# jammm/first_raytracer

Hardware: AMD Instinct MI355X
Metric: Mrays/sec + RMSE vs CPU ref, CornellBox 1080p 512spp, 1/2/4/8 MI355X (higher is better)
Workload: dtype f32

## Files before the change

### first_raytracer_amd/__init__.py

```python
import ctypes
import os

import numpy as np

HERE = os.path.dirname(os.path.abspath(__file__))
LIB_PATH = os.environ.get("FRT_LIB_PATH") or os.path.join(HERE, "libfrt.so")

FRT_WORLD_BVH, FRT_WORLD_LIST = 0, 1
FRT_MAT_LAMBERTIAN, FRT_MAT_DIFFUSE_LIGHT = 0, 1
FRT_PRIM_SPHERE = 1 << 30
ABI_VERSION = 9
FRT_MAT_LAMBERTIAN, FRT_MAT_DIFFUSE_LIGHT, FRT_MAT_MODIFIED_PHONG, FRT_MAT_METAL, FRT_MAT_DIELECTRIC = 0, 1, 2, 3, 4
FRT_MAT_ROUGH_CONDUCTOR = 5
FRT_DIST_GGX, FRT_DIST_BECKMANN = 0, 1
FRT_TEX_CONSTANT, FRT_TEX_CHECKER, FRT_TEX_IMAGE = 0, 1, 2
FRT_IMAGE_SRGB8, FRT_IMAGE_F32 = 0, 1
FRT_FLAG_NO_LDS_SCENE = 1
FRT_FLAG_WAVES5 = 2
FRT_FLAG_WAVES6 = 4
FRT_FLAG_WAVES4 = 8
FRT_FLAG_BVH2 = 16
FRT_FLAG_NO_OCT = 256
FRT_FLAG_FP64 = 512
FRT_FLAG_FP32 = 1024
FRT_FLAG_ENV_SAMPLING = 2048
FRT_FLAG_ROULETTE = 4096
FRT_FLAG_SOBOL = 8192
FRT_PRECISION_AUTO, FRT_PRECISION_FP32, FRT_PRECISION_FP64 = 0, 1, 2
FRT_GPU_BVH_PLOC = 0
FRT_GPU_BVH_LBVH = 1
FRT_GPU_BVH_SAH = 2
FRT_INTEGRATOR_PATH, FRT_INTEGRATOR_PSSMLT, FRT_INTEGRATOR_AO, FRT_INTEGRATOR_NORMALS = 0, 1, 2, 3
FRT_INTEGRATOR_ALBEDO, FRT_INTEGRATOR_DEPTH, FRT_INTEGRATOR_DENOISE = 4, 5, 6
FRT_INTEGRATOR_ERROR = 8

ERRORS = {0: "ok", -1: "invalid", -2: "hip", -3: "no scene", -4: "unsupported", -5: "io", -6: "no gfx950 device"}


class FrtError(RuntimeError):
    pass


class Material(ctypes.Structure):
    _fields_ = [("type", ctypes.c_int32), ("distribution", ctypes.c_int32),
                ("albedo", ctypes.c_double * 3), ("emit", ctypes.c_double * 3),
                ("specular", ctypes.c_double * 3), ("exponent", ctypes.c_double), ("ior", ctypes.c_double),
                ("alpha", ctypes.c_double), ("eta", ctypes.c_double * 3), ("k", ctypes.c_double * 3),
                ("texture", ctypes.c_int32), ("image", ctypes.c_int32), ("tex_odd", ctypes.c_double * 3),
                ("tex_scale", ctypes.c_double * 2)]

    @classmethod
    def from_spec(cls, m):
        r = cls()
        r.type = MAT_TYPES[m["type"]]
        r.distribution = DISTRIBUTIONS[m.get("distribution", "ggx").lower()]
        for k in ("albedo", "emit", "specular", "eta", "k"):
            getattr(r, k)[:] = [float(x) for x in m.get(k, (0.0, 0.0, 0.0))]
        r.exponent = float(m.get("exponent", 0.0))
        r.ior = float(m.get("ior", 0.0))
        r.alpha = float(m.get("alpha", 0.0))
        tex = m.get("checker")
        if tex is not None:
            r.texture = FRT_TEX_CHECKER
            r.tex_odd[:] = [float(x) for x in tex["odd"]]
            r.tex_scale[:] = [float(x) for x in tex["scale"]]
        if m.get("image") is not None:
            r.texture = FRT_TEX_IMAGE
            r.image = int(m["image"])
        return r


class Image(ctypes.Structure):
    _fields_ = [("nx", ctypes.c_int32), ("ny", ctypes.c_int32), ("format", ctypes.c_int32),
                ("reserved", ctypes.c_int32), ("data", ctypes.c_void_p)]


def image_array(img):
    a = np.asarray(img["data"])
    if a.ndim != 3 or a.shape[2] != 3:
        raise ValueError("image data must be (ny, nx, 3)")
    if a.dtype == np.uint8:
        return np.ascontiguousarray(a), FRT_IMAGE_SRGB8
    return np.ascontiguousarray(a, np.float32), FRT_IMAGE_F32


CORNELL_CAMERA = {"lookfrom": (0.0, 1.0, float(np.float32(3.9))), "lookat": (0.0, 1.0, 0.0), "vup": (0.0, 1.0, 0.0),
                  "vfov": 40.0, "aperture": 0.0, "focus": 10.0}
MAT_TYPES = {"lambertian": 0, "diffuse_light": 1, "modified_phong": 2, "metal": 3, "dielectric": 4,
             "rough_conductor": 5}
DISTRIBUTIONS = {"ggx": 0, "beckmann": 1}
SPHERE_WHERE = {"world": 1, "lights": 2, "both": 3}


class SceneView(ctypes.Structure):
    _fields_ = [
        ("world_kind", ctypes.c_int32),
        ("n_tris", ctypes.c_int32),
        ("tri_v", ctypes.c_void_p), ("tri_n", ctypes.c_void_p), ("tri_material", ctypes.c_void_p),
        ("tri_geometry_normal", ctypes.c_void_p), ("tri_inv_area", ctypes.c_void_p),
        ("n_spheres", ctypes.c_int32), ("sphere", ctypes.c_void_p), ("sphere_material", ctypes.c_void_p),
        ("n_materials", ctypes.c_int32), ("materials", ctypes.c_void_p),
        ("n_nodes", ctypes.c_int32), ("root", ctypes.c_int32),
        ("node_box", ctypes.c_void_p), ("node_child", ctypes.c_void_p),
        ("n_list", ctypes.c_int32), ("list", ctypes.c_void_p),
        ("n_lights", ctypes.c_int32), ("lights", ctypes.c_void_p),
        ("cam_origin", ctypes.c_double * 3), ("cam_lower_left", ctypes.c_double * 3),
        ("cam_horizontal", ctypes.c_double * 3), ("cam_vertical", ctypes.c_double * 3),
        ("cam_u", ctypes.c_double * 3), ("cam_v", ctypes.c_double * 3),
        ("cam_lens_radius", ctypes.c_double),
        ("env_color", ctypes.c_double * 3),
        ("cam_w", ctypes.c_double * 3),
        ("cam_half_height", ctypes.c_double),
        ("tri_uv", ctypes.c_void_p),
        ("n_images", ctypes.c_int32), ("images", ctypes.c_void_p),
    ]


class RenderParams(ctypes.Structure):
    _fields_ = [(n, ctypes.c_int32) for n in ("nx", "ny", "spp")] + [("seed", ctypes.c_uint32)] + [
        (n, ctypes.c_int32) for n in ("max_depth", "integrator", "tile_size", "shard_index", "shard_count",
                                      "samples_per_item", "flags", "mlt_chains", "mlt_bootstrap", "sample_offset")]

    @classmethod
    def make(cls, nx, ny, spp, seed=0, max_depth=33, tile_size=32, shard_index=0, shard_count=1,
             samples_per_item=0, flags=0, integrator=0, sample_offset=0):
        return cls(nx=nx, ny=ny, spp=spp, seed=seed, max_depth=max_depth, integrator=integrator, tile_size=tile_size,
                   shard_index=shard_index, shard_count=shard_count, samples_per_item=samples_per_item, flags=flags,
                   mlt_chains=0, mlt_bootstrap=0, sample_offset=sample_offset)

    @classmethod
    def pssmlt(cls, nx, ny, mutations_per_pixel, chains, seed=0, bootstrap=10000, shard_index=0, shard_count=1,
               flags=0):
        return cls(nx=nx, ny=ny, spp=mutations_per_pixel, seed=seed, max_depth=10, integrator=FRT_INTEGRATOR_PSSMLT,
                   tile_size=32, shard_index=shard_index, shard_count=shard_count, samples_per_item=0, flags=flags,
                   mlt_chains=chains, mlt_bootstrap=bootstrap)


class Stats(ctypes.Structure):
    _fields_ = [(n, ctypes.c_uint64) for n in ("camera_rays", "extension_rays", "shadow_rays", "samples",
                                               "pixels", "work_items")] + [
        ("kernel_ms", ctypes.c_double), ("total_ms", ctypes.c_double)] + [
        (n, ctypes.c_uint32) for n in ("scene_in_lds", "waves_cap", "stack_entries", "bvh_depth")] + [
        ("scene_bytes", ctypes.c_uint64), ("fp64", ctypes.c_uint32), ("reserved", ctypes.c_uint32)]

    @property
    def rays(self):
        return self.camera_rays + self.extension_rays + self.shadow_rays

    def as_dict(self):
        d = {n: getattr(self, n) for n, _ in self._fields_}
        d["rays"] = self.rays
        return d


class TreeCost(ctypes.Structure):
    _fields_ = [("v", ctypes.c_double), ("t", ctypes.c_double), ("j", ctypes.c_double), ("w", ctypes.c_double),
                ("depth", ctypes.c_int32), ("n_nodes", ctypes.c_int32), ("n_rays", ctypes.c_int32),
                ("applies", ctypes.c_int32)]

    def as_dict(self):
        return {k: getattr(self, k) for k, _ in self._fields_}


class ShadowTreeInfo(ctypes.Structure):
    _fields_ = [(n, ctypes.c_int32) for n in ("why", "kept_prims", "dropped_prims", "rule_a", "rule_b", "nodes_main",
                                              "nodes_added", "nodes_shared", "root", "empty", "n_rays",
                                              "root_stops_main", "root_stops_shadow", "n_nodes")] + [
        (n, ctypes.c_double) for n in ("v_main", "t_main", "v_shadow", "t_shadow")] + [
        ("segments", ctypes.c_int64), ("segment_hits", ctypes.c_int64)]

    def as_dict(self):
        return {k: getattr(self, k) for k, _ in self._fields_}


class ExitTreeInfo(ctypes.Structure):
    _fields_ = [(n, ctypes.c_int32) for n in ("why", "classes", "taken", "budget_refused", "nodes_off", "n_nodes",
                                              "nodes_added", "depth_off", "depth_on", "n_rays", "n_ext", "reserved")] + [
        (n, ctypes.c_int64) for n in ("lds_bytes", "lds_bytes_oct", "lds_cap", "lds_cap_oct")] + [
        (n, ctypes.c_double * 2) for n in ("v_all", "t_all", "j_all", "v_ext", "t_ext")]

    def as_dict(self):
        return {k: (list(getattr(self, k)) if t is ctypes.c_double * 2 else getattr(self, k)) for k, t in self._fields_}


class PlanQuery(ctypes.Structure):
    _fields_ = [(n, ctypes.c_int32) for n in ("kind", "integrator", "flags", "world_kind", "stack_needed", "has_bvh4",
                                              "depth4", "mats", "has_spec_mats", "env_image", "env_sampling",
                                              "has_f64", "precision")] + [
        ("scene_lds_bytes", ctypes.c_int64), ("scene_lds_bytes_oct", ctypes.c_int64)]


class PlanAnswer(ctypes.Structure):
    _fields_ = [(n, ctypes.c_int32) for n in ("rc", "stack", "waves", "lds_scene", "wide", "f64")] + [
        (n, ctypes.c_int64) for n in ("lds", "scene_lds", "lds_boot")] + [
        ("kernel", ctypes.c_uint64), ("kernel_boot", ctypes.c_uint64)]


class HostSceneInfo(ctypes.Structure):
    _fields_ = [(n, ctypes.c_int32) for n in ("n_tris", "n_spheres", "n_materials", "n_lights", "n_nodes",
                                              "world_kind", "n_list", "bvh_depth")] + [
        ("load_ms", ctypes.c_double), ("build_ms", ctypes.c_double)]


_lib = None

EXPORTS = ("frt_get_abi_version", "frt_create", "frt_destroy", "frt_last_error", "frt_set_precision", "frt_upload_scene",
           "frt_shard_slot_count", "frt_shard_slots", "frt_render", "frt_render_multi", "frt_render_device", "frt_trace_device",
           "frt_mlt_chain_state",
           "frt_scene_create", "frt_scene_new", "frt_scene_add_obj", "frt_scene_add_sphere", "frt_scene_set_camera",
           "frt_scene_set_env", "frt_scene_add_image", "frt_scene_finish", "frt_scene_build_bvh_gpu",
           "frt_scene_build_bvh_sah", "frt_scene_build_bvh_gpu_algo",
           "frt_scene_view_get", "frt_scene_info", "frt_scene_destroy", "frt_write_tessellated_obj",
           "frt_write_pfm", "frt_film_accumulate", "frt_tonemap_u8", "frt_write_image", "frt_selftest_path_host",
           "frt_selftest_mlt_paths_host",
           "frt_set_env_image", "frt_scene_set_env_image", "frt_scene_env_image", "frt_read_hdr",
           "frt_selftest_path_host_env")
EXPORTS_X = ("frtx_selftest_tree_refine", "frtx_selftest_trace_host", "frtx_selftest_chunk_variance",
             "frtx_selftest_plan", "frtx_selftest_shadow_tree", "frtx_render_pixels", "frtx_render_pixels_device",
             "frtx_selftest_exit_tree", "frtx_radiance_rays", "frtx_radiance_rays_device", "frtx_camera_rays_device",
             "frtx_selftest_radiance_host", "frtx_selftest_camera_rays_host")


def lib():
    global _lib
    if _lib is not None:
        return _lib
    if not os.path.exists(LIB_PATH):
        raise FrtError(f"{LIB_PATH} is missing: build it with `python -c 'import __graft_entry__ as g; g.build()'`")
    try:
        import torch
    except ImportError:
        pass
    L = ctypes.CDLL(LIB_PATH)
    vp = ctypes.c_void_p
    L.frt_get_abi_version.restype = ctypes.c_int
    if L.frt_get_abi_version() != ABI_VERSION:
        raise FrtError(f"{LIB_PATH}: ABI version {L.frt_get_abi_version()}, binding expects {ABI_VERSION}; rebuild")
    L.frt_create.argtypes = [ctypes.c_int, ctypes.POINTER(vp)]
    L.frt_destroy.argtypes = [vp]
    L.frt_last_error.argtypes = [vp]
    L.frt_last_error.restype = ctypes.c_char_p
    L.frt_set_precision.argtypes = [vp, ctypes.c_int]
    L.frt_upload_scene.argtypes = [vp, ctypes.POINTER(SceneView)]
    L.frt_shard_slot_count.argtypes = [ctypes.POINTER(RenderParams)]
    L.frt_shard_slot_count.restype = ctypes.c_int64
    L.frt_shard_slots.argtypes = [ctypes.POINTER(RenderParams), vp]
    L.frt_render.argtypes = [vp, ctypes.POINTER(RenderParams), vp, ctypes.POINTER(Stats)]
    L.frt_render_device.argtypes = [vp, ctypes.POINTER(RenderParams), vp, vp, ctypes.POINTER(Stats)]
    L.frt_trace_device.argtypes = [vp, vp, ctypes.c_int64, vp, ctypes.c_int, vp, ctypes.POINTER(Stats)]
    L.frt_mlt_chain_state.argtypes = [vp, ctypes.c_uint64, ctypes.c_uint64, vp, vp]
    L.frt_render_multi.argtypes = [ctypes.POINTER(vp), ctypes.c_int, ctypes.POINTER(RenderParams), vp,
                                   ctypes.POINTER(Stats)]
    L.frt_scene_create.argtypes = [ctypes.c_char_p, ctypes.c_char_p, ctypes.c_double, ctypes.POINTER(vp)]
    L.frt_scene_view_get.argtypes = [vp, ctypes.POINTER(SceneView)]
    L.frt_scene_info.argtypes = [vp, ctypes.POINTER(HostSceneInfo)]
    L.frt_scene_destroy.argtypes = [vp]
    L.frt_scene_destroy.restype = None
    dp = ctypes.POINTER(ctypes.c_double)
    L.frt_scene_new.argtypes = [ctypes.POINTER(vp)]
    L.frt_scene_add_obj.argtypes = [vp, ctypes.c_char_p, dp, ctypes.POINTER(Material), ctypes.c_int]
    L.frt_scene_add_sphere.argtypes = [vp, dp, ctypes.c_double, ctypes.POINTER(Material), ctypes.c_int]
    L.frt_scene_set_camera.argtypes = [vp, dp, dp, dp, ctypes.c_double, ctypes.c_double, ctypes.c_double,
                                       ctypes.c_double]
    L.frt_scene_set_env.argtypes = [vp, dp]
    L.frt_scene_add_image.argtypes = [vp, ctypes.POINTER(Image), ctypes.POINTER(ctypes.c_int)]
    L.frt_scene_finish.argtypes = [vp, ctypes.c_int]
    L.frt_scene_build_bvh_gpu.argtypes = [vp, vp, ctypes.POINTER(ctypes.c_double)]
    L.frt_scene_build_bvh_sah.argtypes = [vp]
    L.frt_scene_build_bvh_gpu_algo.argtypes = [vp, vp, ctypes.c_int, ctypes.POINTER(ctypes.c_double)]
    L.frt_write_tessellated_obj.argtypes = [ctypes.c_char_p, ctypes.c_int, ctypes.c_char_p]
    L.frt_write_pfm.argtypes = [ctypes.c_char_p, ctypes.c_int, ctypes.c_int, vp]
    L.frt_film_accumulate.argtypes = [vp, ctypes.c_int64, vp, ctypes.c_int64, ctypes.c_int64]
    L.frt_tonemap_u8.argtypes = [vp, ctypes.c_int, ctypes.c_int, vp]
    L.frt_write_image.argtypes = [ctypes.c_char_p, ctypes.c_int, ctypes.c_int, vp, ctypes.c_int]
    L.frt_selftest_path_host.argtypes = [ctypes.POINTER(SceneView), ctypes.POINTER(RenderParams), vp,
                                         ctypes.c_int, vp, ctypes.POINTER(Stats)]
    L.frt_selftest_mlt_paths_host.argtypes = [ctypes.POINTER(SceneView), ctypes.c_int, ctypes.c_int, ctypes.c_uint32,
                                              ctypes.c_int, vp]
    L.frt_set_env_image.argtypes = [vp, ctypes.POINTER(Image)]
    L.frt_scene_set_env_image.argtypes = [vp, ctypes.c_int]
    L.frt_scene_env_image.argtypes = [vp, ctypes.POINTER(Image)]
    L.frt_read_hdr.argtypes = [ctypes.c_char_p, ctypes.POINTER(ctypes.c_int32), ctypes.POINTER(ctypes.c_int32), vp]
    L.frt_selftest_path_host_env.argtypes = [ctypes.POINTER(SceneView), ctypes.POINTER(RenderParams), vp,
                                             ctypes.c_int, ctypes.POINTER(Image), vp, ctypes.POINTER(Stats)]
    L.frtx_selftest_tree_refine.argtypes = [ctypes.POINTER(SceneView), ctypes.POINTER(TreeCost), vp, vp, ctypes.c_int32]
    L.frtx_selftest_shadow_tree.argtypes = [ctypes.POINTER(SceneView), ctypes.POINTER(ShadowTreeInfo), vp, vp,
                                            ctypes.c_int32, ctypes.c_int64, ctypes.c_uint32]
    if hasattr(L, "frtx_selftest_exit_tree"):
        L.frtx_selftest_exit_tree.argtypes = [ctypes.POINTER(SceneView), ctypes.c_int32, ctypes.POINTER(ExitTreeInfo), vp,
                                              vp, vp, ctypes.c_int32, vp, vp, ctypes.c_int32]
    L.frtx_selftest_trace_host.argtypes = [ctypes.POINTER(SceneView), vp, ctypes.c_int64, vp]
    L.frtx_selftest_chunk_variance.argtypes = [vp, ctypes.c_int, ctypes.c_int64, ctypes.c_int, ctypes.c_int, vp]
    L.frtx_render_pixels.argtypes = [vp, ctypes.POINTER(RenderParams), vp, ctypes.c_int64, vp, vp, ctypes.POINTER(Stats)]
    L.frtx_render_pixels_device.argtypes = [vp, ctypes.POINTER(RenderParams), vp, ctypes.c_int64, vp, vp, vp,
                                            ctypes.POINTER(Stats)]
    if hasattr(L, "frtx_radiance_rays"):
        L.frtx_radiance_rays.argtypes = [vp, ctypes.POINTER(RenderParams), vp, ctypes.c_int64, vp, vp, ctypes.POINTER(Stats)]
        L.frtx_radiance_rays_device.argtypes = [vp, ctypes.POINTER(RenderParams), vp, ctypes.c_int64, vp, vp, vp,
                                                ctypes.POINTER(Stats)]
        L.frtx_camera_rays_device.argtypes = [vp, ctypes.POINTER(RenderParams), vp, ctypes.c_int64, vp, vp]
        L.frtx_selftest_radiance_host.argtypes = [ctypes.POINTER(SceneView), ctypes.POINTER(RenderParams), vp, ctypes.c_int64,
                                                  ctypes.POINTER(Image), vp, ctypes.POINTER(Stats)]
        L.frtx_selftest_camera_rays_host.argtypes = [ctypes.POINTER(SceneView), ctypes.POINTER(RenderParams), vp,
                                                     ctypes.c_int64, vp]
    _lib = L
    return L


def _check(rc, what, ctx=None):
    if rc != 0:
        msg = ""
        if ctx is not None:
            msg = lib().frt_last_error(ctx).decode(errors="replace")
        elif "_rays" in what or "radiance" in what:
            msg = lib().frt_last_error(None).decode(errors="replace")
        raise FrtError(f"{what} failed: {ERRORS.get(rc, rc)} {msg}")


class HostScene:

    def __init__(self, kind, obj_path, aspect):
        self.ptr = ctypes.c_void_p()
        _check(lib().frt_scene_create(kind.encode(), obj_path.encode(), float(aspect), ctypes.byref(self.ptr)),
               f"frt_scene_create({kind})")
        self.info = HostSceneInfo()
        lib().frt_scene_info(self.ptr, ctypes.byref(self.info))
        self.env = None

    def set_env(self, rgb):
        self.env = tuple(float(x) for x in rgb)

    def set_env_image(self, index):
        _check(lib().frt_scene_set_env_image(self.ptr, -1 if index is None else int(index)), "frt_scene_set_env_image")

    def env_image(self):
        img = Image()
        rc = lib().frt_scene_env_image(self.ptr, ctypes.byref(img))
        if rc < 0:
            _check(rc, "frt_scene_env_image")
        return img if rc == 1 else None

    @classmethod
    def from_spec(cls, spec, aspect):
        self = cls.__new__(cls)
        self.ptr = ctypes.c_void_p()
        self.env = None
        L = lib()
        _check(L.frt_scene_new(ctypes.byref(self.ptr)), "frt_scene_new")

        def dptr(x):
            a = np.ascontiguousarray(np.asarray(x, np.float64))
            return a, a.ctypes.data_as(ctypes.POINTER(ctypes.c_double))
        for img in spec.get("images", ()):
            a, fmt = image_array(img)
            desc = Image(a.shape[1], a.shape[0], fmt, 0, a.ctypes.data)
            idx = ctypes.c_int(-1)
            _check(L.frt_scene_add_image(self.ptr, ctypes.byref(desc), ctypes.byref(idx)), "frt_scene_add_image")
        for o in spec["objects"]:
            if "obj" in o:
                tw = dptr(o["to_world"]) if o.get("to_world") is not None else (None, None)
                bs = ctypes.byref(Material.from_spec(o["bsdf"])) if o.get("bsdf") is not None else None
                _check(L.frt_scene_add_obj(self.ptr, o["obj"].encode(), tw[1], bs, int(bool(o.get("geo", False)))),
                       f"frt_scene_add_obj({o['obj']})")
            else:
                c = dptr(o["sphere"])
                _check(L.frt_scene_add_sphere(self.ptr, c[1], float(o["radius"]),
                                              ctypes.byref(Material.from_spec(o["material"])),
                                              SPHERE_WHERE[o.get("where", "world")]), "frt_scene_add_sphere")
        cam = spec["camera"]
        f, a, u = dptr(cam["lookfrom"]), dptr(cam["lookat"]), dptr(cam.get("vup", (0, 1, 0)))
        _check(L.frt_scene_set_camera(self.ptr, f[1], a[1], u[1], float(cam["vfov"]), float(aspect),
                                      float(cam.get("aperture", 0.0)), float(cam.get("focus", 10.0))),
               "frt_scene_set_camera")
        if spec.get("env") is not None:
            e = dptr(spec["env"])
            _check(L.frt_scene_set_env(self.ptr, e[1]), "frt_scene_set_env")
        if spec.get("env_image") is not None:
            _check(L.frt_scene_set_env_image(self.ptr, int(spec["env_image"])), "frt_scene_set_env_image")
        _check(L.frt_scene_finish(self.ptr, {"bvh": 0, "list": 1}[spec.get("world", "bvh")]), "frt_scene_finish")
        self.info = HostSceneInfo()
        L.frt_scene_info(self.ptr, ctypes.byref(self.info))
        return self

    def view(self):
        v = SceneView()
        _check(lib().frt_scene_view_get(self.ptr, ctypes.byref(v)), "frt_scene_view_get")
        if self.env is not None:
            v.env_color[:] = self.env
        return v

    def arrays(self):
        v = self.view()

        def arr(ptr, n, dt, w=1):
            if n == 0 or not ptr:
                return np.zeros((0, w) if w > 1 else 0, dt)
            a = np.ctypeslib.as_array(ctypes.cast(ptr, ctypes.POINTER(np.ctypeslib.as_ctypes_type(dt))),
                                      shape=(n * w,)).copy()
            return a.reshape(n, w) if w > 1 else a
        return {
            "tri_v": arr(v.tri_v, v.n_tris, np.float64, 9),
            "tri_material": arr(v.tri_material, v.n_tris, np.int32),
            "sphere": arr(v.sphere, v.n_spheres, np.float64, 4),
            "node_box": arr(v.node_box, v.n_nodes, np.float64, 6),
            "node_child": arr(v.node_child, v.n_nodes, np.int32, 2),
            "root": v.root,
            "lights": arr(v.lights, v.n_lights, np.int32),
            "list": arr(v.list, v.n_list, np.int32),
        }

    def build_bvh_sah(self):
        _check(lib().frt_scene_build_bvh_sah(self.ptr), "frt_scene_build_bvh_sah")
        lib().frt_scene_info(self.ptr, ctypes.byref(self.info))
        return self.info.build_ms

    def build_bvh_gpu(self, ctx, algo="gsah"):
        ms = ctypes.c_double()
        a = {"ploc": FRT_GPU_BVH_PLOC, "lbvh": FRT_GPU_BVH_LBVH, "gsah": FRT_GPU_BVH_SAH}[algo]
        _check(lib().frt_scene_build_bvh_gpu_algo(self.ptr, ctx.ptr, a, ctypes.byref(ms)),
               "frt_scene_build_bvh_gpu_algo", ctx.ptr)
        lib().frt_scene_info(self.ptr, ctypes.byref(self.info))
        return ms.value

    def __del__(self):
        if getattr(self, "ptr", None):
            try:
                lib().frt_scene_destroy(self.ptr)
            except Exception:
                pass
            self.ptr = None


class Context:

    def __init__(self, device=0, precision=None):
        self.ptr = ctypes.c_void_p()
        self.device = int(device)
        _check(lib().frt_create(int(device), ctypes.byref(self.ptr)), f"frt_create(device={device})")
        if precision is not None:
            self.set_precision(precision)

    def set_precision(self, precision):
        if isinstance(precision, str):
            precision = {"auto": FRT_PRECISION_AUTO, "fp32": FRT_PRECISION_FP32, "fp64": FRT_PRECISION_FP64}[precision]
        _check(lib().frt_set_precision(self.ptr, int(precision)), "frt_set_precision", self.ptr)

    def upload(self, scene):
        view = scene.view() if isinstance(scene, HostScene) else scene
        _check(lib().frt_upload_scene(self.ptr, ctypes.byref(view)), "frt_upload_scene", self.ptr)
        img = scene.env_image() if isinstance(scene, HostScene) else None
        if img is not None:
            _check(lib().frt_set_env_image(self.ptr, ctypes.byref(img)), "frt_set_env_image", self.ptr)
            self._env_from_scene = True
        elif isinstance(scene, HostScene) and getattr(self, "_env_from_scene", False):
            _check(lib().frt_set_env_image(self.ptr, None), "frt_set_env_image", self.ptr)
            self._env_from_scene = False

    def set_env_image(self, image):
        self._env_from_scene = False
        if image is None:
            _check(lib().frt_set_env_image(self.ptr, None), "frt_set_env_image", self.ptr)
            return
        a, fmt = image_array({"data": image})
        desc = Image(a.shape[1], a.shape[0], fmt, 0, a.ctypes.data)
        _check(lib().frt_set_env_image(self.ptr, ctypes.byref(desc)), "frt_set_env_image", self.ptr)

    def render(self, params, film=None):
        if film is None:
            film = np.zeros((params.ny, params.nx, 3), np.float32)
        assert film.dtype == np.float32 and film.flags.c_contiguous and film.size == params.nx * params.ny * 3
        st = Stats()
        _check(lib().frt_render(self.ptr, ctypes.byref(params), film.ctypes.data, ctypes.byref(st)),
               "frt_render", self.ptr)
        return film, st

    def denoise(self, film, nx, ny, spp=16, seed=0, tile_size=32, flags=0):
        p = RenderParams.make(nx, ny, spp, seed=seed, tile_size=tile_size, flags=flags,
                              integrator=FRT_INTEGRATOR_DENOISE)
        return self.render(p, film=film)

    def render_error(self, params):
        p = RenderParams.from_buffer_copy(params)
        p.integrator = FRT_INTEGRATOR_ERROR
        return self.render(p)

    def render_pixels(self, params, pixels, variance=True):
        pixels = np.ascontiguousarray(pixels, dtype=np.int32).reshape(-1)
        rgb = np.zeros((len(pixels), 3), np.float32)
        V = np.zeros((len(pixels), 3), np.float32) if variance else None
        st = Stats()
        _check(lib().frtx_render_pixels(self.ptr, ctypes.byref(params), pixels.ctypes.data, len(pixels), rgb.ctypes.data,
                                        V.ctypes.data if variance else None, ctypes.byref(st)),
               "frtx_render_pixels", self.ptr)
        return rgb, V, st

    def radiance_rays(self, params, rays, variance=True):
        rays = np.ascontiguousarray(rays, dtype=np.float32).reshape(-1, 8)
        rgb = np.zeros((len(rays), 3), np.float32)
        V = np.zeros((len(rays), 3), np.float32) if variance else None
        st = Stats()
        _check(lib().frtx_radiance_rays(self.ptr, ctypes.byref(params), rays.ctypes.data, len(rays), rgb.ctypes.data,
                                        V.ctypes.data if variance else None, ctypes.byref(st)),
               "frtx_radiance_rays", self.ptr)
        return rgb, V, st

    def camera_rays(self, params, pixels):
        import torch
        pixels = np.ascontiguousarray(pixels, dtype=np.int32).reshape(-1)
        dev = torch.device("cuda", self.device)
        px = torch.from_numpy(pixels).to(dev)
        out = torch.zeros((len(pixels), 8), dtype=torch.float32, device=dev)
        _check(lib().frtx_camera_rays_device(self.ptr, ctypes.byref(params), px.data_ptr(), len(pixels), out.data_ptr(), None),
               "frtx_camera_rays_device", self.ptr)
        return out.cpu().numpy()

    def render_camera(self, params, make_rays, passes=1):
        acc, st = None, None
        for k in range(int(passes)):
            p = RenderParams.from_buffer_copy(params)
            p.sample_offset = params.sample_offset + k * params.spp
            jitter = None if passes == 1 else np.random.default_rng([int(params.seed), k]).random(2)
            rgb, _, st = self.radiance_rays(p, make_rays(jitter), variance=False)
            acc = rgb if acc is None else film_accumulate(acc, k * params.spp, rgb, params.spp)
        return acc, st

    def render_until(self, params, target, max_spp, first_spp=None, adaptive=False, switch=None):
        if adaptive:
            film, V, counts, e, ok, _ = render_until(lambda p: self.render(p), lambda p: self.render_error(p)[0],
                                                     params, target, max_spp, first_spp, adaptive=True,
                                                     render_pixels=lambda p, px: self.render_pixels(p, px), switch=switch)
            return film, V, counts, e, ok
        film, V, spp, e, ok, _ = render_until(lambda p: self.render(p), lambda p: self.render_error(p)[0],
                                              params, target, max_spp, first_spp)
        return film, V, spp, e, ok

    def render_device(self, params, dev_ptr, stream_ptr=None):
        st = Stats()
        _check(lib().frt_render_device(self.ptr, ctypes.byref(params), ctypes.c_void_p(dev_ptr),
                                       ctypes.c_void_p(stream_ptr) if stream_ptr else None, ctypes.byref(st)),
               "frt_render_device", self.ptr)
        return st

    def mlt_chain_state(self, first, n):
        u = np.zeros((max(n, 1), 92), np.float32)
        fp = np.zeros((max(n, 1), 2), np.uint32)
        _check(lib().frt_mlt_chain_state(self.ptr, int(first), int(n), u.ctypes.data, fp.ctypes.data),
               "frt_mlt_chain_state", self.ptr)
        return u[:n], fp[:n]

    def trace_device(self, rays_ptr, n, hits_ptr, flags=0, stream_ptr=None):
        st = Stats()
        _check(lib().frt_trace_device(self.ptr, ctypes.c_void_p(rays_ptr), int(n), ctypes.c_void_p(hits_ptr), int(flags),
                                      ctypes.c_void_p(stream_ptr) if stream_ptr else None, ctypes.byref(st)),
               "frt_trace_device", self.ptr)
        return st

    def close(self):
        if getattr(self, "ptr", None):
            lib().frt_destroy(self.ptr)
            self.ptr = None

    def __del__(self):
        try:
            self.close()
        except Exception:
            pass


def render_multi(contexts, params, film=None):
    if film is None:
        film = np.zeros((params.ny, params.nx, 3), np.float32)
    assert film.dtype == np.float32 and film.flags.c_contiguous and film.size == params.nx * params.ny * 3
    arr = (ctypes.c_void_p * len(contexts))(*[c.ptr for c in contexts])
    st = Stats()
    _check(lib().frt_render_multi(arr, len(contexts), ctypes.byref(params), film.ctypes.data, ctypes.byref(st)),
           "frt_render_multi", contexts[0].ptr)
    return film, st


def frame_error(film, V):
    f = np.asarray(film, np.float64)
    v = np.asarray(V, np.float64)
    return float(np.sqrt(v.sum() / v.size) / (f.sum() / f.size))


def combine_variance(a, Va, b, Vb):
    a, b = float(a), float(b)
    va, vb = np.asarray(Va, np.float64), np.asarray(Vb, np.float64)
    return (((a * a) * va + (b * b) * vb) / ((a + b) * (a + b))).astype(np.float32)


def replicate_variance(films):
    assert len(films) == 4
    r = [np.asarray(f, np.float64) for f in films]
    m = (((r[0] + r[1]) + r[2]) + r[3]) * 0.25
    v = ((((r[0] - m) ** 2 + (r[1] - m) ** 2) + (r[2] - m) ** 2) + (r[3] - m) ** 2) / 12.0
    mean = np.array(films[0], np.float32, copy=True)
    for k in range(1, 4):
        mean = film_accumulate(mean, k, films[k], 1)
    return mean, v.astype(np.float32)


ADAPTIVE_SWITCH = 0.5
ADAPTIVE_FIRST_SPP = 128


def frame_mean(film):
    f = np.asarray(film, np.float64).reshape(-1)
    return float(np.cumsum(f)[-1] / f.size)


def render_until(render, render_error, params, target, max_spp, first_spp=None, adaptive=False, render_pixels=None,
                 switch=None):
    if first_spp is None:
        first_spp = ADAPTIVE_FIRST_SPP if adaptive else 16
    first_spp, max_spp = int(first_spp), int(max_spp)
    if first_spp < 2 or first_spp & (first_spp - 1):
        raise FrtError("render_until: first_spp must be a power of two >= 2")
    if params.integrator not in (FRT_INTEGRATOR_PATH, FRT_INTEGRATOR_AO):
        raise FrtError("render_until: path and ao renders only (pssmlt has no error estimate, denoise is a filter)")
    if not target > 0:
        raise FrtError("render_until: target must be > 0")
    sobol = bool(params.flags & FRT_FLAG_SOBOL) and params.integrator == FRT_INTEGRATOR_PATH
    reps = 4 if sobol else 1
    if max_spp < reps * first_spp:
        raise FrtError("render_until: max_spp is below the first pass")
    slots = lib().frt_shard_slot_count(ctypes.byref(params))
    if slots < 0:
        raise FrtError("bad render params")
    if adaptive:
        if sobol:
            raise FrtError("render_until: adaptive with FRT_FLAG_SOBOL is refused -- V is an upper estimate under "
                           "Sobol' points and the replicates give no per-pixel error; render without the flag")
        if render_pixels is None:
            raise FrtError("render_until: adaptive needs a render_pixels callable")
        return _render_until_adaptive(render, render_error, render_pixels, params, float(target), max_spp, first_spp,
                                      slots, ADAPTIVE_SWITCH if switch is None else float(switch))
    films, V, total, passes = [None] * reps, None, 0, []
    halve = False
    while True:
        n = first_spp if total == 0 else total
        ms = 0.0
        for k in range(reps):
            p = RenderParams.from_buffer_copy(params)
            p.spp, p.sample_offset, p.seed = n, total, (params.seed + k) & 0xffffffff
            if halve:
                p.samples_per_item = n // 2
            film, st = render(p)
            if not sobol and st.work_items == slots:
                halve = True
                p.samples_per_item = n // 2
                film, st = render(p)
            ms += st.kernel_ms
            if not sobol:
                Vp = render_error(p)
                V = Vp if total == 0 else combine_variance(total, V, n, Vp)
            films[k] = film if total == 0 else film_accumulate(films[k], total, film, n)
        total += n
        if sobol:
            film, V = replicate_variance(films)
        else:
            film = films[0]
        e = frame_error(film, V)
        passes.append((reps * total, e, ms))
        if e <= target:
            return film, V, reps * total, e, True, passes
        if reps * 2 * total > max_spp:
            return film, V, reps * total, e, False, passes


def _render_until_adaptive(render, render_error, render_pixels, params, target, max_spp, first_spp, slots, switch):
    nx, ny = params.nx, params.ny
    npx = nx * ny
    halve = False

    def full_pass(n, offset):
        nonlocal halve
        p = RenderParams.from_buffer_copy(params)
        p.spp, p.sample_offset = n, offset
        if halve:
            p.samples_per_item = n // 2
        film, st = render(p)
        if st.work_items == slots:
            halve = True
            p.samples_per_item = n // 2
            film, st = render(p)
        return film, np.asarray(render_error(p), np.float32), st.kernel_ms

    def merge(film_px, V_px, cnt_px, rgb, Vp, n):
        for c in np.unique(cnt_px):
            g = cnt_px == c
            film_px[g] = film_accumulate(film_px[g], int(c), rgb[g], n)
            V_px[g] = combine_variance(int(c), V_px[g], n, Vp[g])

    film, V, ms = full_pass(first_spp, 0)
    film = np.array(film, np.float32).reshape(npx, 3)
    V = np.array(V, np.float32).reshape(npx, 3)
    counts = np.full(npx, first_spp, np.int64)
    offset = first_spp
    passes, sampled, sparse = [], npx, False
    while True:
        tau = target * frame_mean(film)
        v64 = V.astype(np.float64)
        active = np.flatnonzero(((v64[:, 0] + v64[:, 1]) + v64[:, 2]) / 3.0 > tau * tau)
        e = frame_error(film, V)
        passes.append((int(counts.sum()), e, ms, sampled, sparse))
        done = len(active) == 0
        n = 0 if done else int(counts[active].max())
        if done or 2 * n > max_spp:
            return (film.reshape(ny, nx, 3), V.reshape(ny, nx, 3), counts.astype(np.int32).reshape(ny, nx), e, done,
                    passes)
        sparse = len(active) < switch * npx
        if sparse:
            ms, before = 0.0, counts[active]
            for c in np.unique(before):
                idx = active[before == c]
                p = RenderParams.from_buffer_copy(params)
                p.spp, p.sample_offset, p.samples_per_item = int(c), offset, 0
                rgb, Vp, st = render_pixels(p, idx.astype(np.int32))
                ms += st.kernel_ms
                film[idx] = film_accumulate(film[idx], int(c), np.asarray(rgb, np.float32), int(c))
                V[idx] = combine_variance(int(c), V[idx], int(c), np.asarray(Vp, np.float32))
                counts[idx] += c
            sampled = len(active)
        else:
            rgb, Vp, ms = full_pass(n, offset)
            merge(film, V, counts, np.asarray(rgb, np.float32).reshape(npx, 3), Vp.reshape(npx, 3), n)
            counts += n
            sampled = npx
        offset += n


def selftest_chunk_variance(partial, spp, spi):
    partial = np.ascontiguousarray(partial, dtype=np.float32)
    k, n, three = partial.shape
    assert three == 3
    out = np.zeros((n, 3), np.float32)
    _check(lib().frtx_selftest_chunk_variance(partial.ctypes.data, k, n, int(spp), int(spi), out.ctypes.data),
           "frtx_selftest_chunk_variance")
    return out


def shard_slots(params):
    n = lib().frt_shard_slot_count(ctypes.byref(params))
    if n < 0:
        raise FrtError("bad render params")
    out = np.zeros(n, np.int32)
    _check(lib().frt_shard_slots(ctypes.byref(params), out.ctypes.data), "frt_shard_slots")
    return out


def selftest_path_host(scene, params, pixels, env_image=None):
    pixels = np.ascontiguousarray(pixels, dtype=np.int32)
    out = np.zeros((len(pixels), 3), np.float32)
    st = Stats()
    view = scene.view()
    if env_image is None:
        _check(lib().frt_selftest_path_host(ctypes.byref(view), ctypes.byref(params), pixels.ctypes.data, len(pixels),
                                            out.ctypes.data, ctypes.byref(st)), "frt_selftest_path_host")
        return out, st
    a, fmt = image_array({"data": env_image})
    desc = Image(a.shape[1], a.shape[0], fmt, 0, a.ctypes.data)
    _check(lib().frt_selftest_path_host_env(ctypes.byref(view), ctypes.byref(params), pixels.ctypes.data, len(pixels),
                                            ctypes.byref(desc), out.ctypes.data, ctypes.byref(st)),
           "frt_selftest_path_host_env")
    return out, st


def ray_records(origins, directions, t_max=None, streams=None):
    o, d = np.broadcast_arrays(np.asarray(origins, np.float32).reshape(-1, 3), np.asarray(directions, np.float32).reshape(-1, 3))
    rec = np.zeros((len(d), 8), np.float32)
    rec[:, 0:3] = o
    rec[:, 3] = np.finfo(np.float32).max if t_max is None else t_max
    rec[:, 4:7] = d
    ids = np.arange(len(d), dtype=np.uint32) if streams is None else np.asarray(streams, np.uint32).reshape(-1)
    rec.view(np.uint32)[:, 7] = ids
    return rec


def selftest_radiance_host(scene, params, rays, env_image=None):
    rays = np.ascontiguousarray(rays, dtype=np.float32).reshape(-1, 8)
    out = np.zeros((len(rays), 3), np.float32)
    st = Stats()
    view = scene.view()
    desc = None
    if env_image is not None:
        a, fmt = image_array({"data": env_image})
        desc = ctypes.byref(Image(a.shape[1], a.shape[0], fmt, 0, a.ctypes.data))
    _check(lib().frtx_selftest_radiance_host(ctypes.byref(view), ctypes.byref(params), rays.ctypes.data, len(rays), desc,
                                             out.ctypes.data, ctypes.byref(st)), "frtx_selftest_radiance_host")
    return out, st


def selftest_camera_rays_host(scene, params, pixels):
    pixels = np.ascontiguousarray(pixels, dtype=np.int32).reshape(-1)
    out = np.zeros((len(pixels), 8), np.float32)
    view = scene.view()
    _check(lib().frtx_selftest_camera_rays_host(ctypes.byref(view), ctypes.byref(params), pixels.ctypes.data, len(pixels),
                                                out.ctypes.data), "frtx_selftest_camera_rays_host")
    return out


def selftest_tree_refine(scene):
    view = scene.view()
    cap = max(1, view.n_tris + view.n_spheres)
    nodes = [np.zeros((cap, 16), np.float32) for _ in range(2)]
    out = (TreeCost * 2)()
    _check(lib().frtx_selftest_tree_refine(ctypes.byref(view), out, nodes[0].ctypes.data, nodes[1].ctypes.data, cap),
           "frtx_selftest_tree_refine")
    return tuple((out[k].as_dict(), nodes[k][:out[k].n_nodes].copy()) for k in range(2))


def selftest_shadow_tree(scene, segments=0, seed=1):
    view = scene.view()
    cap = max(2 * int(view.n_nodes), 1) + 4
    nodes = np.zeros((cap, 16), np.float32)
    dropped = np.zeros(max(int(view.n_tris), 1), np.uint8)
    out = ShadowTreeInfo()
    _check(lib().frtx_selftest_shadow_tree(ctypes.byref(view), ctypes.byref(out), dropped.ctypes.data, nodes.ctypes.data,
                                           cap, int(segments), int(seed)), "frtx_selftest_shadow_tree")
    return out.as_dict(), dropped[:int(view.n_tris)].copy(), nodes[:out.n_nodes].copy()


EXIT_WHY = ("ran", "off", "material", "not_resident", "too_large", "nothing", "budget")


def selftest_exit_tree(scene, mode=1):
    view = scene.view()
    cap = max(4 * int(view.n_nodes), 1) + 16
    nodes = np.zeros((2, cap, 16), np.float32)
    roots = np.zeros(max(int(view.n_tris), 1), np.int32)
    taken = np.zeros((64, 6), np.int32)
    view_of = np.zeros(max(int(view.n_tris), 1), np.int32)
    out = ExitTreeInfo()
    _check(lib().frtx_selftest_exit_tree(ctypes.byref(view), int(mode), ctypes.byref(out), roots.ctypes.data,
                                         view_of.ctypes.data, taken.ctypes.data, len(taken), nodes[0].ctypes.data, nodes[1].ctypes.data, cap),
           "frtx_selftest_exit_tree")
    info = out.as_dict()
    info["why_name"] = EXIT_WHY[out.why]
    info["view_of"] = view_of[:int(view.n_tris)].copy()
    return (info, roots[:int(view.n_tris)].copy(), taken[:min(out.taken, len(taken))].copy(),
            nodes[0, :out.nodes_off].copy(), nodes[1, :out.n_nodes].copy())


def selftest_trace_host(scene, rays):
    rays = np.ascontiguousarray(rays, dtype=np.float32).reshape(-1, 8)
    hits = np.zeros((len(rays), 4), np.float32)
    view = scene.view()
    _check(lib().frtx_selftest_trace_host(ctypes.byref(view), rays.ctypes.data, len(rays), hits.ctypes.data),
           "frtx_selftest_trace_host")
    return hits


_handles = None


def kernel_handles():
    global _handles
    if _handles is None:
        import re
        import subprocess
        out = subprocess.run(["nm", "--defined-only", LIB_PATH], capture_output=True, text=True, check=True).stdout
        syms = [l.split() for l in out.splitlines()]
        stub = re.compile(r"(\d+)__device_stub__")
        kernels = {stub.sub(lambda m: str(int(m.group(1)) - 15), f[2]) for f in syms if len(f) == 3 and stub.search(f[2])}
        _handles = {int(f[0], 16): f[2] for f in syms if len(f) == 3 and f[2] in kernels}
    return _handles


def selftest_plan(**query):
    f = lib().frtx_selftest_plan
    f.argtypes = [ctypes.POINTER(PlanQuery), ctypes.POINTER(PlanAnswer)]
    a = PlanAnswer()
    _check(f(ctypes.byref(PlanQuery(**query)), ctypes.byref(a)), "frtx_selftest_plan")
    d = {n: getattr(a, n) for n, _ in a._fields_}
    for k in ("kernel", "kernel_boot"):
        d[k] = kernel_handles().get(d[k]) if d[k] else None
    return d


def selftest_mlt_paths_host(scene, nx, ny, seed, n):
    out = np.zeros((n, 6), np.float32)
    view = scene.view()
    _check(lib().frt_selftest_mlt_paths_host(ctypes.byref(view), nx, ny, seed, n, out.ctypes.data),
           "frt_selftest_mlt_paths_host")
    return out


def read_hdr(path):
    nx, ny = ctypes.c_int32(0), ctypes.c_int32(0)
    _check(lib().frt_read_hdr(os.fsencode(path), ctypes.byref(nx), ctypes.byref(ny), None), f"frt_read_hdr({path})")
    out = np.zeros((ny.value, nx.value, 3), np.float32)
    _check(lib().frt_read_hdr(os.fsencode(path), ctypes.byref(nx), ctypes.byref(ny), out.ctypes.data),
           f"frt_read_hdr({path})")
    return out


def write_pfm(path, film):
    film = np.ascontiguousarray(film, dtype=np.float32)
    ny, nx = film.shape[0], film.shape[1]
    _check(lib().frt_write_pfm(path.encode(), nx, ny, film.ctypes.data), "frt_write_pfm")


def film_accumulate(acc, acc_spp, film, spp):
    acc = np.ascontiguousarray(acc, dtype=np.float32)
    film = np.ascontiguousarray(film, dtype=np.float32)
    _check(lib().frt_film_accumulate(acc.ctypes.data, int(acc_spp), film.ctypes.data, int(spp), film.size),
           "frt_film_accumulate")
    return acc


def tonemap_u8(film):
    film = np.ascontiguousarray(film, dtype=np.float32)
    ny, nx = film.shape[0], film.shape[1]
    out = np.zeros((ny, nx, 3), np.uint8)
    _check(lib().frt_tonemap_u8(film.ctypes.data, nx, ny, out.ctypes.data), "frt_tonemap_u8")
    return out


IMAGE_FORMATS = {"png": 0, "bmp": 1, "jpg": 2}


def write_image(path, rgb_u8, fmt="png"):
    rgb_u8 = np.ascontiguousarray(rgb_u8, dtype=np.uint8)
    ny, nx = rgb_u8.shape[0], rgb_u8.shape[1]
    _check(lib().frt_write_image(path.encode(), nx, ny, rgb_u8.ctypes.data, IMAGE_FORMATS[fmt]), "frt_write_image")


def work_granule(integrator, spp, n_slots, lanes, spi_req=0):
    L = lib()
    f = L.frt_internal_work_granule
    f.argtypes = [ctypes.c_int, ctypes.c_int, ctypes.c_int64, ctypes.c_int64, ctypes.c_int,
                  ctypes.POINTER(ctypes.c_int), ctypes.POINTER(ctypes.c_int)]
    spi, k = ctypes.c_int(0), ctypes.c_int(0)
    _check(f(integrator, spp, n_slots, lanes, spi_req, ctypes.byref(spi), ctypes.byref(k)), "work_granule")
    return spi.value, k.value


def write_tessellated_obj(src_obj, k, dst_obj):
    _check(lib().frt_write_tessellated_obj(src_obj.encode(), int(k), dst_obj.encode()), "frt_write_tessellated_obj")
```

### first_raytracer_amd/csrc/frt_flatten.hip

```cpp
#include "frt_flatten.hpp"

#include <algorithm>
#include <cfloat>
#include <cmath>
#include <cstdlib>
#include <functional>

#include "frt_kernels.hpp"
#include "frt_tree_passes.hpp"

using namespace frt;

static inline float round_down(double x)
{
    float f = (float)x;
    if ((double)f > x) f = std::nextafter(f, -INFINITY);
    return f;
}
static inline float round_up(double x)
{
    float f = (float)x;
    if ((double)f < x) f = std::nextafter(f, INFINITY);
    return f;
}
// ... 183 lines not shown
        out.push_back(make_float4((float)c[0], (float)c[1], (float)c[2], 0.0f));
    }
}
int env_texels_of(const frt_image *img, std::vector<float4> &out, std::string &err)
{
    if (img->nx <= 0 || img->ny <= 0) { err = "environment image: nx and ny must be positive"; return FRT_E_INVALID; }
    if (!img->data) { err = "environment image: null data"; return FRT_E_INVALID; }
    if (img->format != FRT_IMAGE_SRGB8 && img->format != FRT_IMAGE_F32) {
        err = "environment image: format must be FRT_IMAGE_SRGB8 or FRT_IMAGE_F32";
        return FRT_E_INVALID;
    }
    if ((size_t)img->nx * img->ny > (size_t)INT32_MAX) { err = "environment image larger than 2^31 texels"; return FRT_E_UNSUPPORTED; }
    out.clear();
    out.reserve((size_t)img->nx * img->ny);
    append_texels(*img, out);
    for (size_t q = 0; q < out.size(); ++q) {
        const float v[3] = {out[q].x, out[q].y, out[q].z};
        for (int ch = 0; ch < 3; ++ch)
            if (!(v[ch] >= 0.0f && v[ch] <= FLT_MAX)) {
                err = "environment image: texel (" + std::to_string(q % img->nx) + ", " + std::to_string(q / img->nx) +
                      ") is negative or not finite";
                return FRT_E_INVALID;
            }
    }
    return FRT_OK;
}

static void fill_octants(FlatScene &F)
{
    for (int o = 0; o < 8 && !F.nodes_oct.empty(); ++o)
        for (size_t i = 0; i < F.nodes.size() / 4; ++i) {
            const float4 *n = &F.nodes[4 * i];
            const float b0[6] = {n[0].x, n[0].y, n[0].z, n[0].w, n[1].x, n[1].y};
            const float b1[6] = {n[1].z, n[1].w, n[2].x, n[2].y, n[2].z, n[2].w};
            float q[12];
            for (int a = 0; a < 3; ++a) {
                const bool neg = (o >> a) & 1;
                q[a] = neg ? b0[3 + a] : b0[a];
                q[3 + a] = neg ? b0[a] : b0[3 + a];
                q[6 + a] = neg ? b1[3 + a] : b1[a];
                q[9 + a] = neg ? b1[a] : b1[3 + a];
            }
            float4 *d = &F.nodes_oct[(size_t)o * F.nodes.size() + 4 * i];
            d[0] = make_float4(q[0], q[1], q[2], q[3]);
            d[1] = make_float4(q[4], q[5], q[6], q[7]);
            d[2] = make_float4(q[8], q[9], q[10], q[11]);
            d[3] = n[3];
        }
}

int flatten_scene(const frt_scene_view *sv, FlatScene &F, std::string &err, bool f64, int refine, int shadow, int exit)
{
    auto fail = [&](int code, const std::string &m) { err = m; return code; };
    const int nt = sv->n_tris, ns = sv->n_spheres, nm = sv->n_materials;
    if (nt < 0 || ns < 0 || nm <= 0 || !sv->materials || (nt > 0 && (!sv->tri_v || !sv->tri_material || !sv->tri_inv_area)))
        return fail(FRT_E_INVALID, "scene view: missing triangle arrays or materials");
    if (ns > 0 && (!sv->sphere || !sv->sphere_material)) return fail(FRT_E_INVALID, "scene view: missing sphere arrays");
    for (int i = 0; i < nm; ++i) {
        const int t = sv->materials[i].type;
        if (t != FRT_MAT_LAMBERTIAN && t != FRT_MAT_DIFFUSE_LIGHT && t != FRT_MAT_MODIFIED_PHONG &&
            t != FRT_MAT_METAL && t != FRT_MAT_DIELECTRIC && t != FRT_MAT_ROUGH_CONDUCTOR)
            return fail(FRT_E_UNSUPPORTED, "material type " + std::to_string(t) + " is not supported");
        const int tex = sv->materials[i].texture;
        if (tex != FRT_TEX_CONSTANT && tex != FRT_TEX_CHECKER && tex != FRT_TEX_IMAGE)
            return fail(FRT_E_INVALID, "material texture must be FRT_TEX_CONSTANT, FRT_TEX_CHECKER or FRT_TEX_IMAGE");
        if (tex != FRT_TEX_CONSTANT && (t == FRT_MAT_DIFFUSE_LIGHT || t == FRT_MAT_METAL))
            return fail(FRT_E_UNSUPPORTED, "checker / image textures apply to lambertian / modified_phong / dielectric / "
                                           "rough_conductor colours");
        if (tex == FRT_TEX_IMAGE) {
            const int k = sv->materials[i].image;
            if (k < 0 || k >= sv->n_images || !sv->images)
                return fail(FRT_E_INVALID, "material image index out of range");
            const frt_image &im = sv->images[k];
            if (im.nx <= 0 || im.ny <= 0 || !im.data || (im.format != FRT_IMAGE_SRGB8 && im.format != FRT_IMAGE_F32))
                return fail(FRT_E_INVALID, "scene view: bad image");
        }
        if (t == FRT_MAT_ROUGH_CONDUCTOR &&
            (!(sv->materials[i].alpha > 0.0) || (sv->materials[i].distribution != FRT_DIST_GGX &&
                                                  sv->materials[i].distribution != FRT_DIST_BECKMANN)))
            return fail(FRT_E_INVALID, "rough_conductor needs alpha > 0 and a GGX / Beckmann distribution");
    }
    auto valid_ref = [&](int ref) {
        if (ref < 0) return false;
        if (ref & FRT_PRIM_SPHERE) return (ref & ~FRT_PRIM_SPHERE) < ns;
        return ref < nt;
    };
    auto prim_box = [&](int ref, double *lo, double *hi) {
        if (ref & FRT_PRIM_SPHERE) {
            const double *q = &sv->sphere[4 * (ref & ~FRT_PRIM_SPHERE)];
            for (int k = 0; k < 3; ++k) { lo[k] = q[k] - q[3]; hi[k] = q[k] + q[3]; }
        } else {
            const double *v = &sv->tri_v[9 * ref];
            for (int k = 0; k < 3; ++k) {
                lo[k] = std::min(std::min(v[k], v[3 + k]), v[6 + k]);
                hi[k] = std::max(std::max(v[k], v[3 + k]), v[6 + k]);
            }
        }
    };
    std::vector<int> tri_order;
    std::vector<int> tri_dev(nt, -1);
    DevScene &S = F.meta;
    S = DevScene{};
    if (sv->world_kind == FRT_WORLD_BVH) {
        const int nn = sv->n_nodes;
        if (nn < 0 || (nn > 0 && (!sv->node_box || !sv->node_child)))
            return fail(FRT_E_INVALID, "scene view: missing BVH arrays");
        if (sv->root >= nn || (sv->root >= 0 && nn == 0)) return fail(FRT_E_INVALID, "scene view: bad root");
        double rlo[3], rhi[3];
        if (sv->root < 0) {
            if (!valid_ref(~sv->root)) return fail(FRT_E_INVALID, "scene view: bad root prim");
            prim_box(~sv->root, rlo, rhi);
        } else {
            for (int k = 0; k < 3; ++k) { rlo[k] = sv->node_box[6 * sv->root + k]; rhi[k] = sv->node_box[6 * sv->root + 3 + k]; }
        }
        double scale = 1.0;
        for (int k = 0; k < 3; ++k) scale = std::max(scale, std::max(std::fabs(rlo[k]), std::fabs(rhi[k])));
        const double pad = 4e-6 * scale;
        auto padded = [&](const double *lo, const double *hi, float *flo, float *fhi) {
            for (int k = 0; k < 3; ++k) { flo[k] = round_down(lo[k] - pad); fhi[k] = round_up(hi[k] + pad); }
        };
        padded(rlo, rhi, S.root_lo, S.root_hi);
        S.ao_tmax = (float)((rhi[1] - rlo[1]) * 0.50f);
        std::vector<int> new_id(std::max(nn, 1), -1), order;
        order.reserve(nn);
        std::vector<std::pair<int, int>> st;
        st.push_back({sv->root, 1});
        while (!st.empty()) {
            const auto [x, lvl] = st.back();
            st.pop_back();
            if (x >= 0) {
                if (x >= nn || new_id[x] >= 0) return fail(FRT_E_INVALID, "scene view: BVH is not a tree");
                new_id[x] = (int)order.size();
                order.push_back(x);
                F.depth = std::max(F.depth, lvl);
                st.push_back({sv->node_child[2 * x + 1], lvl + 1});
                st.push_back({sv->node_child[2 * x], lvl + 1});
            } else {
                const int ref = ~x;
                if (!valid_ref(ref)) return fail(FRT_E_INVALID, "scene view: bad leaf prim");
                if (!(ref & FRT_PRIM_SPHERE)) {
                    if (tri_dev[ref] >= 0) return fail(FRT_E_INVALID, "scene view: triangle in two leaves");
                    tri_dev[ref] = (int)tri_order.size();
                    tri_order.push_back(ref);
                }
            }
        }
        F.nodes.resize(4 * order.size());
        for (size_t i = 0; i < order.size(); ++i) {
            const int x = order[i];
            float cb[2][6];
            int cref[2];
            for (int side = 0; side < 2; ++side) {
                const int ch = sv->node_child[2 * x + side];
                double lo[3], hi[3];
                if (ch >= 0) {
                    for (int k = 0; k < 3; ++k) { lo[k] = sv->node_box[6 * ch + k]; hi[k] = sv->node_box[6 * ch + 3 + k]; }
                    cref[side] = new_id[ch];
                } else {
                    const int ref = ~ch;
                    prim_box(ref, lo, hi);
                    cref[side] = ~((ref & FRT_PRIM_SPHERE) ? ref : tri_dev[ref]);
                }
                padded(lo, hi, &cb[side][0], &cb[side][3]);
            }
            F.nodes[4 * i + 0] = make_float4(cb[0][0], cb[0][1], cb[0][2], cb[0][3]);
            F.nodes[4 * i + 1] = make_float4(cb[0][4], cb[0][5], cb[1][0], cb[1][1]);
            F.nodes[4 * i + 2] = make_float4(cb[1][2], cb[1][3], cb[1][4], cb[1][5]);
            F.nodes[4 * i + 3] = make_float4(i2f(cref[0]), i2f(cref[1]), 0.0f, 0.0f);
        }
        if (nt >= kLeafIndexLimit) return fail(FRT_E_INVALID, "scene view: too many triangles");
        const int forced = leaf_size_override();
        if (forced) {
            collapse_leaves(F, forced);
        } else {
            const std::vector<float4> binary = F.nodes;
            const int depth = F.depth;
            collapse_leaves(F, kLeafSmallScene);
            if (!lds_planar_fits(lds_planar_bytes(F.nodes.size() / 4, 5 * (size_t)nt + 2 * (size_t)nm)) || F.depth >= kLdsMaxDepth) {
                F.nodes = binary;
                F.depth = depth;
                collapse_leaves(F, kLeafDefault);
            }
        }
        for (int i = 0; i < nt; ++i)
            if (tri_dev[i] < 0) { tri_dev[i] = (int)tri_order.size(); tri_order.push_back(i); }
    } else if (sv->world_kind == FRT_WORLD_LIST) {
        S.ao_spheres_only = 1;
        if (sv->n_list < 0 || (sv->n_list > 0 && !sv->list)) return fail(FRT_E_INVALID, "scene view: bad list");
        for (int i = 0; i < nt; ++i) { tri_dev[i] = i; tri_order.push_back(i); }
        for (int i = 0; i < sv->n_list; ++i)
            if (!valid_ref(sv->list[i])) return fail(FRT_E_INVALID, "scene view: bad list entry");
    } else {
        return fail(FRT_E_INVALID, "scene view: unknown world kind");
    }
    auto dev_ref = [&](int ref) { return (ref & FRT_PRIM_SPHERE) ? ref : tri_dev[ref]; };
    F.tri_view = tri_order;

    bool any_smooth = false;
    for (int i = 0; i < nt; ++i)
        if (sv->tri_geometry_normal && !sv->tri_geometry_normal[i]) any_smooth = true;
    if (any_smooth && !sv->tri_n) return fail(FRT_E_INVALID, "scene view: smooth triangles without normals");
    F.tris.resize(3 * (size_t)nt);
    F.tshade.resize(2 * (size_t)nt);
    if (any_smooth) F.tnorm.resize(3 * (size_t)nt);
    if (f64) {
        F.tris64.resize(3 * (size_t)nt);
        F.tshade64.resize(nt);
        if (any_smooth) F.tnorm64.resize(3 * (size_t)nt);
    }
    for (int d = 0; d < nt; ++d) {
        const int i = tri_order[d];
        const double *v = &sv->tri_v[9 * i];
        const double e1[3] = {v[3] - v[0], v[4] - v[1], v[5] - v[2]};
        const double e2[3] = {v[6] - v[0], v[7] - v[1], v[8] - v[2]};
        double ng[3] = {e1[1] * e2[2] - e1[2] * e2[1], e1[2] * e2[0] - e1[0] * e2[2], e1[0] * e2[1] - e1[1] * e2[0]};
        const double l = std::sqrt(ng[0] * ng[0] + ng[1] * ng[1] + ng[2] * ng[2]);
        for (int k = 0; k < 3; ++k) ng[k] = ng[k] / l;
        F.tris[3 * d + 0] = make_float4((float)v[0], (float)v[1], (float)v[2], 0.0f);
        F.tris[3 * d + 1] = make_float4((float)e1[0], (float)e1[1], (float)e1[2], 0.0f);
        F.tris[3 * d + 2] = make_float4((float)e2[0], (float)e2[1], (float)e2[2], 0.0f);
        const int mat = sv->tri_material[i];
        if (mat < 0 || mat >= nm) return fail(FRT_E_INVALID, "scene view: bad triangle material");
        const int geo = sv->tri_geometry_normal ? (sv->tri_geometry_normal[i] ? 1 : 0) : 1;
        F.tshade[2 * d + 0] = make_float4((float)ng[0], (float)ng[1], (float)ng[2], (float)sv->tri_inv_area[i]);
        F.tshade[2 * d + 1] = make_float4(i2f(mat), i2f(geo), 0.0f, 0.0f);
        if (any_smooth)
            for (int k = 0; k < 3; ++k)
                F.tnorm[3 * d + k] = make_float4((float)sv->tri_n[9 * i + 3 * k], (float)sv->tri_n[9 * i + 3 * k + 1],
                                                 (float)sv->tri_n[9 * i + 3 * k + 2], 0.0f);
        if (f64) {
            F.tris64[3 * d + 0] = make_double4(v[0], v[1], v[2], 0.0);
            F.tris64[3 * d + 1] = make_double4(e1[0], e1[1], e1[2], 0.0);
            F.tris64[3 * d + 2] = make_double4(e2[0], e2[1], e2[2], 0.0);
            F.tshade64[d] = make_double4(ng[0], ng[1], ng[2], sv->tri_inv_area[i]);
            if (any_smooth)
                for (int k = 0; k < 3; ++k)
                    F.tnorm64[3 * d + k] = make_double4(sv->tri_n[9 * i + 3 * k], sv->tri_n[9 * i + 3 * k + 1],
                                                        sv->tri_n[9 * i + 3 * k + 2], 0.0);
        }
    }
    bool any_tex = false;
    for (int i = 0; i < nm; ++i) any_tex |= sv->materials[i].texture != FRT_TEX_CONSTANT;
    if (any_tex) {
        F.tuv.assign(2 * (size_t)std::max(nt, 1), make_float4(0.0f, 0.0f, 0.0f, 0.0f));
        if (sv->tri_uv)
            for (int d = 0; d < nt; ++d) {
                const double *q = &sv->tri_uv[6 * tri_order[d]];
                F.tuv[2 * d] = make_float4((float)q[0], (float)q[1], (float)q[2], (float)q[3]);
                F.tuv[2 * d + 1] = make_float4((float)q[4], (float)q[5], 0.0f, 0.0f);
            }
    }
    F.spheres.resize(ns);
    F.smat.resize(ns);
    if (f64) F.spheres64.resize(ns);
    for (int k = 0; k < ns; ++k) {
        const double *q = &sv->sphere[4 * k];
        F.spheres[k] = make_float4((float)q[0], (float)q[1], (float)q[2], (float)q[3]);
        if (f64) F.spheres64[k] = make_double4(q[0], q[1], q[2], q[3]);
        F.smat[k] = sv->sphere_material[k];
        if (F.smat[k] < 0 || F.smat[k] >= nm) return fail(FRT_E_INVALID, "scene view: bad sphere material");
    }
    std::vector<int> image_off(std::max(sv->n_images, 0), -1);
    for (int i = 0; i < nm; ++i) {
        if (sv->materials[i].texture != FRT_TEX_IMAGE) continue;
        const int k = sv->materials[i].image;
        if (image_off[k] >= 0) continue;
        const frt_image &im = sv->images[k];
        const size_t n = (size_t)im.nx * im.ny;
        if (F.texels.size() + n > (size_t)INT32_MAX) return fail(FRT_E_UNSUPPORTED, "images larger than 2^31 texels");
        image_off[k] = (int)F.texels.size();
        append_texels(im, F.texels);
    }
    F.mats.assign(kMatStride * (size_t)nm, make_float4(0.0f, 0.0f, 0.0f, 0.0f));
    for (int i = 0; i < nm; ++i) {
        const frt_material &m = sv->materials[i];
        float4 *d = &F.mats[kMatStride * i];
        auto f4 = [](const double *v, float w) { return make_float4((float)v[0], (float)v[1], (float)v[2], w); };
        d[0] = f4(m.type == FRT_MAT_ROUGH_CONDUCTOR ? m.eta : m.albedo, i2f(m.type));
        if (m.type == FRT_MAT_DIFFUSE_LIGHT) d[1] = f4(m.emit, 0.0f);
        else d[1] = f4(m.specular, (float)(m.type == FRT_MAT_MODIFIED_PHONG ? m.exponent
                                           : m.type == FRT_MAT_DIELECTRIC ? m.ior : m.alpha));
        d[2] = f4(m.k, i2f(m.distribution));
        d[3] = f4(m.tex_odd, i2f(m.texture));
        d[4] = make_float4((float)m.tex_scale[0], (float)m.tex_scale[1], 0.0f, 0.0f);
        if (m.texture == FRT_TEX_IMAGE)
            d[4] = make_float4(i2f(sv->images[m.image].nx), i2f(sv->images[m.image].ny), i2f(image_off[m.image]), 0.0f);
    }
    if (sv->n_lights < 0 || (sv->n_lights > 0 && !sv->lights)) return fail(FRT_E_INVALID, "scene view: bad lights");
    F.lights.resize(sv->n_lights);
    for (int i = 0; i < sv->n_lights; ++i) {
        if (!valid_ref(sv->lights[i])) return fail(FRT_E_INVALID, "scene view: bad light");
        F.lights[i] = dev_ref(sv->lights[i]);
    }
    F.list.resize(sv->world_kind == FRT_WORLD_LIST ? sv->n_list : 0);
    for (size_t i = 0; i < F.list.size(); ++i) F.list[i] = dev_ref(sv->list[i]);

    if (sv->world_kind == FRT_WORLD_BVH && F.depth < kLdsMaxDepth &&
        lds_octant_fits(lds_octant_bytes(F.nodes.size() / 4, lds_rest(F))))
        F.nodes_oct.resize(8 * F.nodes.size());
    S.root = (sv->world_kind == FRT_WORLD_BVH) ? ((sv->root >= 0) ? 0 : ~dev_ref(~sv->root)) : 0;
    S.sroot = S.root;
    auto derive_trees = [&]() {
        fill_octants(F);
        F.has4 = sv->world_kind == FRT_WORLD_BVH && build_bvh4(F, S.root);
        if (!F.has4) F.nodes4.clear();
        S.root4 = F.has4 ? F.root4 : S.root;
        S.n_nodes4 = (int)(F.nodes4.size() / kNode4Parts);
    };
    derive_trees();
    S.n_lights = sv->n_lights;
    S.n_list = (int)F.list.size();
    S.n_nodes = (int)(F.nodes.size() / 4);
    S.n_tris = nt;
    S.n_mats = nm;
    S.n_nodes4 = (int)(F.nodes4.size() / kNode4Parts);
    S.node_es = 4; S.node_ps = 1;
    S.node4_es = kNode4Parts; S.node4_ps = 1;
    S.tri_es = 3; S.tri_ps = 1;
    S.sh_es = 2; S.sh_ps = 1;
    S.world_kind = sv->world_kind;
    auto f3d = [](const double *x) { return mk3((float)x[0], (float)x[1], (float)x[2]); };
    S.cam_o = f3d(sv->cam_origin); S.cam_llc = f3d(sv->cam_lower_left);
    S.cam_h = f3d(sv->cam_horizontal); S.cam_v = f3d(sv->cam_vertical);
    S.cam_u = f3d(sv->cam_u); S.cam_vv = f3d(sv->cam_v);
    S.lens_r = (float)sv->cam_lens_radius;
    S.cam_w = f3d(sv->cam_w);
    S.cam_half_height = (float)sv->cam_half_height;
    S.env = f3d(sv->env_color);
    auto d3d = [](const double *x) { return d3{x[0], x[1], x[2]}; };
    S.cam64_o = d3d(sv->cam_origin); S.cam64_llc = d3d(sv->cam_lower_left);
    S.cam64_h = d3d(sv->cam_horizontal); S.cam64_v = d3d(sv->cam_vertical);
    S.cam64_u = d3d(sv->cam_u); S.cam64_vv = d3d(sv->cam_v);
    S.lens_r64 = sv->cam_lens_radius;
    bool again = refine_tree(F, refine);
    again |= shadow_tree(sv, F, shadow);
    again |= exit_tree(sv, F, exit);
    if (again) derive_trees();
    S.n_nodes = (int)(F.nodes.size() / 4);
    return FRT_OK;
}

DevScene host_scene(const FlatScene &F)
{
    DevScene S = F.meta;
    S.nodes = F.nodes.data(); S.nodes4 = F.nodes4.data(); S.nodes_oct = F.nodes_oct.data();
    S.tris = F.tris.data(); S.tshade = F.tshade.data(); S.tnorm = F.tnorm.data();
    S.tuv = F.tuv.data(); S.texels = F.texels.data();
    S.spheres = F.spheres.data(); S.sphere_mat = F.smat.data(); S.mats = F.mats.data();
    S.lights = F.lights.data(); S.list = F.list.data(); S.tri_view = F.tri_view.data();
    S.tris64 = F.tris64.data(); S.tshade64 = F.tshade64.data(); S.tnorm64 = F.tnorm64.data();
    S.spheres64 = F.spheres64.data();
    return S;
}
```

### first_raytracer_amd/csrc/frt_flatten.hpp

```cpp
#pragma once
#include <string>
#include <vector>

#include "frt.h"
#include "frt_device.hpp"
#include "frt_path.hpp"

using frt::DevScene;

#pragma GCC visibility push(hidden)
struct FlatScene {
    std::vector<float4> nodes, tris, tshade, tnorm, spheres, mats, tuv;
    std::vector<float4> texels;
    std::vector<uint4> nodes4;
    std::vector<float4> nodes_oct;
    std::vector<double4> tris64, tshade64, tnorm64, spheres64;
    bool has4 = false;
    int root4 = 0, depth4 = 0;
    std::vector<int> smat, lights, list;
    std::vector<int> tri_view;
    DevScene meta{};
    int depth = 0;
    enum { kShadowRan = 0, kShadowOff, kShadowNoLights, kShadowTooLarge, kShadowMaterial, kShadowNotResident,
           kShadowNothing, kShadowBudget };
    struct {
        int why = kShadowOff;
        std::vector<uint8_t> dropped;
        int n_dropped = 0, rule_a = 0, rule_b = 0, nodes_main = 0, added = 0, shared = 0;
        bool empty = false;
    } shadow;
    enum { kExitRan = 0, kExitOff, kExitMaterial, kExitNotResident, kExitTooLarge, kExitNothing, kExitBudget };
    struct ExitClass { int sub, root, members, dropped, added, shared; double gain; };
    struct {
        int why = kExitOff;
        int classes = 0;
        std::vector<ExitClass> taken;
        std::vector<int> root;
        int nodes_before = 0, added = 0;
        bool budget_refused = false;
    } exit;
};

int flatten_scene(const frt_scene_view *sv, FlatScene &F, std::string &err, bool f64, int refine = -1, int shadow = -1,
                  int exit = -1);
int env_texels_of(const frt_image *img, std::vector<float4> &out, std::string &err);
frt::DevScene host_scene(const FlatScene &F);
#pragma GCC visibility pop
```

### first_raytracer_amd/csrc/frt_selftest.hip

```cpp
#include <algorithm>
#include <cstring>
#include <string>
#include <vector>

#include "frt_ctx.hpp"
#include "frt_flatten.hpp"
#include "frt_rays.hpp"
#include "frt_tree_passes.hpp"
#include "host/envdist.hpp"

using namespace frt;

constexpr int kSelftestStack = 8;

template <typename R, int MATS = kMatsAll>
static void selftest_pixels(const DevScene &S, const FlatScene &F, const frt_render_params *p, const int32_t *pixels,
                            int npix, bool wide, std::vector<int> &stack, float *out_rgb, uint64_t cnt[3],
                            const float *rays = nullptr)
{
    uint32_t n_ext = 0, n_sh = 0;
    for (int i = 0; i < npix; ++i) {
        const int pix = rays ? 0 : pixels[i];
        const int px = pix % p->nx, py = pix / p->nx;
        float4 ray[2];
        if (rays) memcpy(ray, rays + 8 * (size_t)i, sizeof(ray));
        V3<R> acc = zero3<R>();
        for (int smp = 0; smp < p->spp; ++smp) {
            PathState<R> P;
            if (rays) ray_begin<MATS>(P, ray[0], ray[1], p->seed, (uint32_t)(smp + p->sample_offset));
            else path_begin<MATS>(P, S, px, py, p->nx, p->ny, p->seed, (uint32_t)pix, (uint32_t)(smp + p->sample_offset));
            ++cnt[0];
            for (;;) {
                Hit<R> h;
                const bool occl = p->integrator != FRT_INTEGRATOR_AO && light_shadow_ray(P);
                const int xroot = p->integrator == FRT_INTEGRATOR_PATH && !P.shadow ? exit_root(P) : 0;
                if (S.world_kind == FRT_WORLD_LIST) {
                    h = trace<FRT_WORLD_LIST, 1>(S, P.ro, P.rd, P.rtmax, P.shadow, stack.data());
                } else if constexpr (!kIsF64<R>) {
                    h = wide ? trace<kWorldBvh4, 1, kSelftestStack>(S, P.ro, P.rd, P.rtmax, P.shadow, stack.data())
                        : xroot ? trace_bvh_from<1>(S, xroot, P.ro, P.rd, P.rtmax, stack.data())
                             : trace<FRT_WORLD_BVH, 1>(S, P.ro, P.rd, P.rtmax, P.shadow, stack.data(), occl);
                } else {
                    h = xroot ? trace_bvh_from<1>(S, xroot, P.ro, P.rd, P.rtmax, stack.data())
                              : trace<FRT_WORLD_BVH, 1>(S, P.ro, P.rd, P.rtmax, P.shadow, stack.data(), occl);
                }
                n_ext = n_sh = 0;
                const bool done = p->integrator == FRT_INTEGRATOR_AO ? ao_shade<MATS>(P, S, h, n_sh)
                                  : p->integrator == FRT_INTEGRATOR_NORMALS ? normals_shade<MATS>(P, S, h)
                                  : p->integrator == FRT_INTEGRATOR_ALBEDO ? albedo_shade(P, S, h)
                                  : p->integrator == FRT_INTEGRATOR_DEPTH ? depth_shade(P, S, h)
                                  : path_shade<MATS, true>(P, S, h, p->max_depth, n_ext, n_sh);
                cnt[1] += n_ext; cnt[2] += n_sh;
                if (done) break;
            }
            acc = acc + P.L;
        }
        if (p->integrator == FRT_INTEGRATOR_ALBEDO || p->integrator == FRT_INTEGRATOR_DEPTH) {
            const R n = (R)p->spp;
            out_rgb[3 * i] = (float)(acc.x / n); out_rgb[3 * i + 1] = (float)(acc.y / n); out_rgb[3 * i + 2] = (float)(acc.z / n);
            if (p->integrator == FRT_INTEGRATOR_DEPTH)
                out_rgb[3 * i + 1] = depth_moment_floor(out_rgb[3 * i], out_rgb[3 * i + 1], out_rgb[3 * i + 2]);
            continue;
        }
        if (rays) {
            const R n = (R)p->spp;
            out_rgb[3 * i] = (float)(acc.x / n); out_rgb[3 * i + 1] = (float)(acc.y / n); out_rgb[3 * i + 2] = (float)(acc.z / n);
            continue;
        }
        const R k = R(1) / (R)p->spp;
        out_rgb[3 * i] = (float)(acc.x * k); out_rgb[3 * i + 1] = (float)(acc.y * k); out_rgb[3 * i + 2] = (float)(acc.z * k);
    }
}

extern "C" int frt_selftest_path_host(const frt_scene_view *sv, const frt_render_params *p, const int32_t *pixels,
                                      int npix, float *out_rgb, frt_stats *st)
{
    return frt_selftest_path_host_env(sv, p, pixels, npix, nullptr, out_rgb, st);
}
static int selftest_replay(const frt_scene_view *sv, const frt_render_params *p, const int32_t *pixels, const float *rays,
                           int npix, const frt_image *env, float *out_rgb, frt_stats *st);
extern "C" int frt_selftest_path_host_env(const frt_scene_view *sv, const frt_render_params *p, const int32_t *pixels,
                                          int npix, const frt_image *env, float *out_rgb, frt_stats *st)
{
    if (!sv || !p || !pixels || !out_rgb || npix < 0 || p->spp <= 0 || p->nx <= 0 || p->ny <= 0) return FRT_E_INVALID;
    for (int i = 0; i < npix; ++i)
        if (pixels[i] < 0 || pixels[i] >= p->nx * p->ny) return FRT_E_INVALID;
    return selftest_replay(sv, p, pixels, nullptr, npix, env, out_rgb, st);
}
static int selftest_replay(const frt_scene_view *sv, const frt_render_params *p, const int32_t *pixels, const float *rays,
                           int npix, const frt_image *env, float *out_rgb, frt_stats *st)
{
    if (p->integrator == FRT_INTEGRATOR_DENOISE) return FRT_E_INVALID;
    if (p->integrator == FRT_INTEGRATOR_ERROR) return FRT_E_INVALID;
    const bool feature = p->integrator == FRT_INTEGRATOR_ALBEDO || p->integrator == FRT_INTEGRATOR_DEPTH;
    if (feature) env = nullptr;
    const bool f64 = (p->flags & FRT_FLAG_FP64) != 0 && !feature;
    FlatScene F;
    std::string err;
    const int rc = flatten_scene(sv, F, err, f64);
    if (rc != FRT_OK) return rc;
    if (p->integrator == FRT_INTEGRATOR_AO)
        for (int i = 0; i < sv->n_materials; ++i)
            if (sv->materials[i].type == FRT_MAT_METAL) return FRT_E_UNSUPPORTED;
    DevScene S = host_scene(F);
    std::vector<float4> env_tex;
    bool env_sampling = false;
    if (env) {
        const int erc = env_texels_of(env, env_tex, err);
        if (erc != FRT_OK) return erc;
        if ((p->flags & FRT_FLAG_ENV_SAMPLING) && p->integrator != FRT_INTEGRATOR_AO &&
            p->integrator != FRT_INTEGRATOR_NORMALS) {
            std::vector<float> tab;
            env_sampling = env_tables_of(&env_tex[0].x, env->nx, env->ny, tab);
            const size_t n = env_tex.size();
            env_tex.resize(n + tab.size() / 4);
            memcpy(reinterpret_cast<float *>(env_tex.data() + n), tab.data(), tab.size() * sizeof(float));
        }
        S.env_texels = env_tex.data(); S.env_nx = env->nx; S.env_ny = env->ny;
    }
    std::vector<int> stack(std::max(F.depth + 1, kSelftestStack));
    const bool wide = !f64 && S.world_kind == FRT_WORLD_BVH && F.has4 && !(p->flags & FRT_FLAG_BVH2) &&
                      bvh4_stack_fits(F.depth4, kSelftestStack);
    uint64_t cnt[3] = {0, 0, 0};
    constexpr int kEnvAll = kMatsAll | kMatsEnv;
    constexpr int kEnvNee = kEnvAll | kMatsEnvNee;
    const bool path = p->integrator == FRT_INTEGRATOR_PATH;
    const bool roulette = (p->flags & FRT_FLAG_ROULETTE) && path, sobol = (p->flags & FRT_FLAG_SOBOL) && path;
    auto run_set = [&](auto extra) {
        constexpr int X = decltype(extra)::value;
        auto run = [&](auto mats) {
            constexpr int M = decltype(mats)::value;
            if (f64) selftest_pixels<double, M | X>(S, F, p, pixels, npix, wide, stack, out_rgb, cnt, rays);
            else selftest_pixels<float, M | X>(S, F, p, pixels, npix, wide, stack, out_rgb, cnt, rays);
        };
        if (env_sampling) run(std::integral_constant<int, kEnvNee>{});
        else if (env) run(std::integral_constant<int, kEnvAll>{});
        else run(std::integral_constant<int, kMatsAll>{});
    };
    if (sobol && roulette) run_set(std::integral_constant<int, kMatsSobol | kMatsRoulette>{});
    else if (sobol) run_set(std::integral_constant<int, kMatsSobol>{});
    else if (roulette) run_set(std::integral_constant<int, kMatsRoulette>{});
    else run_set(std::integral_constant<int, 0>{});
    if (st) {
        memset(st, 0, sizeof(*st));
        st->camera_rays = cnt[0]; st->extension_rays = cnt[1]; st->shadow_rays = cnt[2];
        st->samples = cnt[0]; st->pixels = (uint64_t)npix;
        st->stack_entries = wide ? (uint32_t)kSelftestStack : (uint32_t)stack.size();
        st->bvh_depth = (uint32_t)(wide ? F.depth4 : F.depth);
        st->fp64 = f64 ? 1u : 0u;
    }
    return FRT_OK;
}

extern "C" int frtx_selftest_radiance_host(const frt_scene_view *sv, const frt_render_params *p, const float *rays, int64_t n,
                                           const frt_image *env, float *out_rgb, frt_stats *st)
{
    auto fail = [](int code, const std::string &m) { frt::null_ctx_err() = m; return code; };
    if (!sv || !p || n < 0 || n > INT32_MAX || (n > 0 && (!rays || !out_rgb))) return fail(FRT_E_INVALID, "radiance_rays: bad arguments");
    const int k = p->integrator;
    if (k == FRT_INTEGRATOR_NORMALS || k == FRT_INTEGRATOR_ALBEDO || k == FRT_INTEGRATOR_DEPTH)
        return fail(FRT_E_UNSUPPORTED, "radiance_rays: path and ao only (normals, albedo and depth have no sparse kernel)");
    if (k != FRT_INTEGRATOR_PATH && k != FRT_INTEGRATOR_AO)
        return fail(FRT_E_INVALID, "radiance_rays: path and ao only (pssmlt is no per-pixel estimator; denoise and error are "
                                   "films of a whole frame)");
    if (p->shard_count != 1) return fail(FRT_E_INVALID, "radiance_rays: shard_count must be 1 (split the list instead)");
    if (p->spp <= 0 || p->sample_offset < 0) return fail(FRT_E_INVALID, "bad render params");
    std::string why;
    if (frt::rays_first_bad(rays, n, why) >= 0) return fail(FRT_E_INVALID, "radiance_rays: " + why);
    if (st) memset(st, 0, sizeof(*st));
    if (n == 0) return FRT_OK;
    frt_render_params q = *p;
    q.nx = q.ny = 1;
    return selftest_replay(sv, &q, nullptr, rays, (int)n, env, out_rgb, st);
}

extern "C" int frtx_selftest_camera_rays_host(const frt_scene_view *sv, const frt_render_params *p, const int32_t *pixels,
                                              int64_t npix, float *rays_out)
{
    if (!sv || !p || npix < 0 || (npix > 0 && (!pixels || !rays_out)) || p->nx <= 0 || p->ny <= 0 || p->sample_offset < 0 ||
        (int64_t)p->nx * p->ny > (int64_t)INT32_MAX)
        return FRT_E_INVALID;
    for (int64_t i = 0; i < npix; ++i)
        if (pixels[i] < 0 || pixels[i] >= p->nx * p->ny) return FRT_E_INVALID;
    FlatScene F;
    std::string err;
    const int rc = flatten_scene(sv, F, err, false);
    if (rc != FRT_OK) return rc;
    const DevScene S = host_scene(F);
    for (int64_t i = 0; i < npix; ++i) {
        const int pix = pixels[i];
        PathState<float> P;
        if (p->flags & FRT_FLAG_SOBOL)
            path_begin<kMatsSobol>(P, S, pix % p->nx, pix / p->nx, p->nx, p->ny, p->seed, (uint32_t)pix, (uint32_t)p->sample_offset);
        else
            path_begin<kMatsNone>(P, S, pix % p->nx, pix / p->nx, p->nx, p->ny, p->seed, (uint32_t)pix, (uint32_t)p->sample_offset);
        const float rec[8] = {P.ro.x, P.ro.y, P.ro.z, P.rtmax, P.rd.x, P.rd.y, P.rd.z, i2f(pix)};
        memcpy(rays_out + 8 * i, rec, sizeof(rec));
    }
    return FRT_OK;
}

extern "C" int frt_selftest_mlt_paths_host(const frt_scene_view *sv, int nx, int ny, uint32_t seed, int n,
                                           float *out6)
{
    if (!sv || !out6 || n < 0 || nx <= 0 || ny <= 0) return FRT_E_INVALID;
    FlatScene F;
    std::string err;
    const int rc = flatten_scene(sv, F, err, false);
    if (rc != FRT_OK) return rc;
    const DevScene S = host_scene(F);
    std::vector<int> stack(std::max(F.depth + 1, 1));
    for (int i = 0; i < n; ++i) {
        PrndSource src{nullptr, 0, 0, rng_key(seed ^ kMltBootSalt, (uint32_t)i, 0u), 0u, true, 0.0f, 0.0f};
        MltPath M;
        mlt_begin(M, S, src, nx, ny);
        uint32_t ne = 0, ns = 0;
        for (;;) {
            if (mlt_beyond(M)) { M.P.L = M.P.L + M.P.beta * env_of<float>(S); break; }
            const Hit<float> h = (S.world_kind == FRT_WORLD_LIST)
                              ? trace<FRT_WORLD_LIST, 1>(S, M.P.ro, M.P.rd, M.P.rtmax, M.P.shadow, stack.data())
                              : trace<FRT_WORLD_BVH, 1>(S, M.P.ro, M.P.rd, M.P.rtmax, M.P.shadow, stack.data(), M.P.shadow);
            if (mlt_shade(M, S, h, src, ne, ns)) break;
        }
        const f3 L = M.P.L;
        float *o = &out6[6 * (size_t)i];
        o[0] = M.x; o[1] = M.y; o[2] = L.x; o[3] = L.y; o[4] = L.z; o[5] = fmaxf(fmaxf(L.x, L.y), L.z);
    }
    return FRT_OK;
}

extern "C" int frtx_selftest_tree_refine(const frt_scene_view *sv, frt_tree_cost out[2], float *nodes_off,
                                        float *nodes_on, int32_t max_nodes)
{
    if (!sv || !out) return FRT_E_INVALID;
    float *dst[2] = {nodes_off, nodes_on};
    for (int on = 0; on < 2; ++on) {
        FlatScene F;
        std::string err;
        const int rc = flatten_scene(sv, F, err, false, on, 0, 0);
        if (rc != FRT_OK) return rc;
        TreeCost c;
        const bool applies = tree_cost_host(F, c);
        const int nn = (int)(F.nodes.size() / 4);
        out[on] = frt_tree_cost{c.V, c.T, c.J, c.w, c.depth, nn, c.n_rays, applies ? 1 : 0};
        if (dst[on]) {
            if (nn > max_nodes) return FRT_E_INVALID;
            memcpy(dst[on], F.nodes.data(), F.nodes.size() * sizeof(float4));
        }
    }
    return FRT_OK;
}

extern "C" int frtx_selftest_shadow_tree(const frt_scene_view *sv, frt_shadow_tree_info *out, uint8_t *dropped,
                                         float *nodes, int32_t max_nodes, int64_t segments, uint32_t seed)
{
    if (!sv || !out || segments < 0) return FRT_E_INVALID;
    FlatScene F;
    std::string err;
    const int rc = flatten_scene(sv, F, err, false, -1, 1, 0);
    if (rc != FRT_OK) return rc;
    const auto &I = F.shadow;
    memset(out, 0, sizeof(*out));
    out->why = I.why;
    out->n_nodes = (int)(F.nodes.size() / 4);
    out->nodes_main = I.nodes_main;
    out->root = F.meta.sroot;
    if (nodes) {
        if (out->n_nodes > max_nodes) return FRT_E_INVALID;
        memcpy(nodes, F.nodes.data(), F.nodes.size() * sizeof(float4));
    }
    if (dropped) memset(dropped, 0, (size_t)std::max(sv->n_tris, 0));
    if (I.why != FlatScene::kShadowRan) return FRT_OK;
    out->dropped_prims = I.n_dropped;
    out->kept_prims = sv->n_tris + sv->n_spheres - I.n_dropped;
    out->rule_a = I.rule_a; out->rule_b = I.rule_b;
    out->nodes_added = I.added; out->nodes_shared = I.shared; out->empty = I.empty ? 1 : 0;
    if (dropped)
        for (int d = 0; d < sv->n_tris; ++d) dropped[F.tri_view[d]] = I.dropped[d];
    ShadowCost c;
    shadow_cost_host(F, c);
    out->n_rays = c.n_rays;
    out->v_main = c.V[0]; out->t_main = c.T[0]; out->v_shadow = c.V[1]; out->t_shadow = c.T[1];
    out->root_stops_main = c.stops[0]; out->root_stops_shadow = c.stops[1];
    if (segments > 0) {
        std::vector<float> org;
        shadow_origins_host(F, org);
        const DevScene S = host_scene(F);
        const int64_t no = (int64_t)(org.size() / 3);
        for (int64_t i = 0; i < segments && no > 0 && S.n_lights > 0; ++i) {
            const RngKey key = rng_key(seed, (uint32_t)i, (uint32_t)(i >> 32));
            const float *q = &org[3 * (size_t)(i % no)];
            const f3 o = mk3(q[0], q[1], q[2]);
            int idx = (int)(rng_u(key, 0) * (float)S.n_lights);
            if (idx == S.n_lights) idx -= 1;
            f3 ln;
            int lmat;
            const f3 d = prim_sample(S, S.lights[idx], o, rng_u(key, 1), rng_u(key, 2), ln, lmat);
            ++out->segments;
            for (int t = 0; t < S.n_tris; ++t) {
                if (!I.dropped[t]) continue;
                float u, v;
                if (prim_t(S, t, o, d, bvh_tmin(o), 1.0f - Cst<float>::shadow_eps, u, v) > 0.0f) ++out->segment_hits;
            }
        }
    }
    return FRT_OK;
}

extern "C" int frtx_selftest_exit_tree(const frt_scene_view *sv, int32_t mode, frt_exit_tree_info *out, int32_t *roots,
                                       int32_t *view_of, int32_t *taken, int32_t max_taken, float *nodes_off,
                                       float *nodes_on, int32_t max_nodes)
{
    if (!sv || !out || mode < -1 || mode > 1 || max_taken < 0) return FRT_E_INVALID;
    memset(out, 0, sizeof(*out));
    FlatScene F0, F;
    std::string err;
    int rc = flatten_scene(sv, F0, err, false, -1, -1, 0);
    if (rc == FRT_OK) rc = flatten_scene(sv, F, err, false, -1, -1, mode);
    if (rc != FRT_OK) return rc;
    const auto &I = F.exit;
    out->why = I.why;
    out->classes = I.classes;
    out->taken = (int32_t)I.taken.size();
    out->nodes_off = (int32_t)(F0.nodes.size() / 4);
    out->n_nodes = (int32_t)(F.nodes.size() / 4);
    out->nodes_added = I.added;
    out->budget_refused = I.budget_refused ? 1 : 0;
    out->depth_off = F0.depth; out->depth_on = F.depth;
    out->lds_bytes = (int64_t)lds_planar_bytes(out->n_nodes, lds_rest(F));
    out->lds_bytes_oct = F.nodes_oct.empty() ? 0 : (int64_t)lds_octant_bytes(out->n_nodes, lds_rest(F));
    out->lds_cap = (int64_t)kLdsSceneBytes; out->lds_cap_oct = (int64_t)kLdsOctBytes;
    if (out->nodes_off > max_nodes || out->n_nodes > max_nodes) return FRT_E_INVALID;
    if (nodes_off) memcpy(nodes_off, F0.nodes.data(), F0.nodes.size() * sizeof(float4));
    if (nodes_on) memcpy(nodes_on, F.nodes.data(), F.nodes.size() * sizeof(float4));
    if (roots)
        for (int d = 0; d < sv->n_tris; ++d) {
            const int r = f2i(F.tshade[2 * (size_t)d + 1].z);
            if (r != (d < (int)I.root.size() ? I.root[d] : 0)) return FRT_E_UNSUPPORTED;
            roots[F.tri_view[d]] = r;
        }
    if (view_of)
        for (int d = 0; d < sv->n_tris; ++d) view_of[d] = F.tri_view[d];
    if (taken)
        for (int k = 0; k < out->taken && k < max_taken; ++k) {
            const auto &c = I.taken[k];
            const int32_t rec[6] = {c.sub, c.root, c.members, c.dropped, c.added, c.shared};
            memcpy(taken + 6 * k, rec, sizeof(rec));
        }
    ExitCost c;
    if (exit_cost_host(F, c)) {
        out->n_rays = c.n_rays; out->n_ext = c.n_ext;
        for (int on = 0; on < 2; ++on) {
            out->v_all[on] = c.V_all[on]; out->t_all[on] = c.T_all[on]; out->j_all[on] = c.J_all[on];
            out->v_ext[on] = c.V_ext[on]; out->t_ext[on] = c.T_ext[on];
        }
    }
    return FRT_OK;
}

extern "C" int frtx_selftest_trace_host(const frt_scene_view *sv, const float *rays, int64_t n, float *hits)
{
    if (!sv || n < 0 || (n > 0 && (!rays || !hits))) return FRT_E_INVALID;
    FlatScene F;
    std::string err;
    const int rc = flatten_scene(sv, F, err, false);
    if (rc != FRT_OK) return rc;
    const DevScene S = host_scene(F);
    std::vector<int> stack(std::max(F.depth + 1, 1));
    for (int64_t i = 0; i < n; ++i) {
        const float *q = rays + 8 * i;
        const f3 o = mk3(q[0], q[1], q[2]), d = mk3(q[4], q[5], q[6]);
        const bool anyhit = (f2i(q[7]) & 1) != 0;
        const Hit<float> h = S.world_kind == FRT_WORLD_LIST ? trace<FRT_WORLD_LIST, 1>(S, o, d, q[3], anyhit, stack.data())
                                                            : trace<FRT_WORLD_BVH, 1>(S, o, d, q[3], anyhit, stack.data());
        const int ref = (h.prim < 0 || (h.prim & FRT_PRIM_SPHERE)) ? h.prim : F.tri_view[h.prim];
        float *r = hits + 4 * i;
        r[0] = h.t; r[1] = h.u; r[2] = h.v;
        const float refbits = i2f(ref);
        memcpy(&r[3], &refbits, sizeof(float));
    }
    return FRT_OK;
}
```

### first_raytracer_amd/csrc/frt_tree_passes.hip

```cpp
#include "frt_tree_passes.hpp"

#include <algorithm>
#include <cstdlib>
#include <cstring>
#include <functional>
#include <unordered_map>

#include "frt_kernels.hpp"
#include "host/exit_tree.hpp"
#include "host/shadow_tree.hpp"
#include "host/tree_refine.hpp"

using namespace frt;

static bool knob(const char *name)
{
    const char *e = std::getenv(name);
    return !(e && std::atoi(e) == 0);
}
static bool pass_on(int mode, const char *name) { return mode < 0 ? knob(name) : mode != 0; }

static bool lambertian_only(const frt_scene_view *sv)
{
    for (int i = 0; i < sv->n_materials; ++i)
        if (sv->materials[i].type != FRT_MAT_LAMBERTIAN && sv->materials[i].type != FRT_MAT_DIFFUSE_LIGHT) return false;
    return true;
}

static bool tree_in_lds(const FlatScene &F)
{
    if (F.meta.world_kind != FRT_WORLD_BVH || F.meta.root < 0 || F.depth >= kLdsMaxDepth) return false;
    return lds_planar_fits(lds_planar_bytes(F.nodes.size() / 4, lds_rest(F))) || !F.nodes_oct.empty();
}

constexpr size_t kLdsGranule = 1280, kLdsCuBytes = 160 * 1024;
static int lds_blocks_per_cu(const FlatScene &F, size_t scene_bytes)
{
    const size_t block = lds_block_bytes(F.depth < 8 ? 8 : 16, scene_bytes);
    return (int)(kLdsCuBytes / ((block + kLdsGranule - 1) / kLdsGranule * kLdsGranule));
}
static bool keeps_plan(const FlatScene &F, int nn0, int nn1, bool same_blocks)
{
    const size_t rest = lds_rest(F);
    const size_t p0 = lds_planar_bytes(nn0, rest), p1 = lds_planar_bytes(nn1, rest);
    const size_t o0 = lds_octant_bytes(nn0, rest), o1 = lds_octant_bytes(nn1, rest);
    const bool lds0 = lds_planar_fits(p0), oct0 = !F.nodes_oct.empty();
    if (lds0 != lds_planar_fits(p1) || oct0 != lds_octant_fits(o1)) return false;
    if (!same_blocks) return true;
    if (lds0 && lds_blocks_per_cu(F, p1) != lds_blocks_per_cu(F, p0)) return false;
    return !oct0 || lds_blocks_per_cu(F, o1) == lds_blocks_per_cu(F, o0);
}

static std::vector<float> node_floats(const std::vector<float4> &nodes)
{
    std::vector<float> v(4 * nodes.size());
    memcpy(v.data(), nodes.data(), sizeof(float4) * nodes.size());
    return v;
}
static std::vector<float4> node_records(const std::vector<float> &v)
{
    std::vector<float4> nodes(v.size() / 4);
    memcpy(nodes.data(), v.data(), sizeof(float) * v.size());
    return nodes;
}
static void adopt_nodes(FlatScene &F, const std::vector<float> &v)
{
    F.nodes = node_records(v);
    if (!F.nodes_oct.empty()) F.nodes_oct.resize(8 * F.nodes.size());
}

struct RefineLeaf { float box[6]; int ref; };

struct TreeView {
    frt_refine::Topology t;
    std::vector<RefineLeaf> leaves;
    std::unordered_map<int, int> leaf_of;

    explicit TreeView(const std::vector<float4> &nodes)
    {
        const int nn = (int)(nodes.size() / 4);
        t.child.assign(2 * (size_t)nn, 0);
        for (int i = 0; i < nn; ++i) {
            const float4 *n = &nodes[4 * i];
            const float b[2][6] = {{n[0].x, n[0].y, n[0].z, n[0].w, n[1].x, n[1].y}, {n[1].z, n[1].w, n[2].x, n[2].y, n[2].z, n[2].w}};
            for (int side = 0; side < 2; ++side) {
                const int c = f2i(side ? n[3].y : n[3].x);
                if (c >= 0) { t.child[2 * i + side] = ~c; continue; }
                const auto [it, fresh] = leaf_of.emplace(c, (int)leaves.size());
                if (fresh) {
                    RefineLeaf l;
                    for (int k = 0; k < 6; ++k) l.box[k] = b[side][k];
                    l.ref = c;
                    leaves.push_back(l);
                }
                t.child[2 * i + side] = it->second;
            }
        }
        t.n_leaves = (int)leaves.size();
        t.root = t.n_leaves;
        for (int &c : t.child)
            if (c < 0) c = t.n_leaves + ~c;
    }
    int slot(int ref) const { return ref >= 0 ? t.n_leaves + ref : leaf_of.at(ref); }
    std::vector<int> leaves_under(int s) const
    {
        std::vector<int> under, st{s};
        while (!st.empty()) {
            const int x = st.back();
            st.pop_back();
            if (x < t.n_leaves) { under.push_back(x); continue; }
            st.push_back(t.child[2 * (x - t.n_leaves)]);
            st.push_back(t.child[2 * (x - t.n_leaves) + 1]);
        }
        return under;
    }
    bool same_leaves(const TreeView &o) const
    {
        return leaves.size() == o.leaves.size() &&
               std::equal(leaves.begin(), leaves.end(), o.leaves.begin(),
                          [](const RefineLeaf &a, const RefineLeaf &b) { return a.ref == b.ref; });
    }
};

constexpr double kRefineW = 1.8;
constexpr int kRefineFitFrame = 24, kRefineValFrame = 40;
constexpr uint32_t kRefineFitSeed = 0x7ee5eed1u, kRefineValSeed = 0x7ee5eed2u;
constexpr int kRefineMaxDepth = 33;
constexpr int kRefineMaxEvals = 700;

struct Replay {
    frt_refine::RaySet R;
    std::vector<uint8_t> occl;
    std::vector<int> from;
    std::vector<float> origins;
};
static Replay sample_rays(const FlatScene &F, const std::vector<RefineLeaf> &leaves, int frame, uint32_t seed)
{
    const DevScene S = host_scene(F);
    struct Ray { f3 o, d; float tmax; bool shadow, occl; int from; };
    std::vector<Ray> rays;
    std::vector<int> stack(std::max(F.depth + 1, 1));
    for (int pix = 0; pix < frame * frame; ++pix) {
        PathState<float> P;
        path_begin<kMatsAll>(P, S, pix % frame, pix / frame, frame, frame, seed, (uint32_t)pix, 0u);
        int last = -1;
        for (;;) {
            rays.push_back(Ray{P.ro, P.rd, P.rtmax, P.shadow, light_shadow_ray(P),
                               (P.shadow || last < 0 || (last & FRT_PRIM_SPHERE)) ? -1 : last});
            const Hit<float> h = trace<FRT_WORLD_BVH, 1>(S, P.ro, P.rd, P.rtmax, P.shadow, stack.data(), light_shadow_ray(P));
            if (!P.shadow) last = h.prim;
            uint32_t n_ext = 0, n_sh = 0;
            if (path_shade<kMatsAll>(P, S, h, kRefineMaxDepth, n_ext, n_sh)) break;
        }
    }
    const int n = (int)rays.size(), nl = (int)leaves.size();
    Replay out;
    frt_refine::RaySet &R = out.R;
    R.n = n;
    R.n_leaves = nl;
    R.prim_first.assign(nl + 1, 0);
    for (int l = 0; l < nl; ++l) {
        const int lref = ~leaves[l].ref;
        const bool sph = (lref & FRT_PRIM_SPHERE) != 0;
        const int first = sph ? lref : (lref & kLeafIndexMask), count = sph ? 1 : (lref >> kLeafCountShift) + 1;
        for (int k = 0; k < count; ++k) R.prim_ref.push_back(first + k);
        R.prim_first[l + 1] = (int)R.prim_ref.size();
    }
    R.n_prims = (int)R.prim_ref.size();
    R.tmin.resize(n); R.tmax.resize(n); R.anyhit.resize(n); R.live.resize(n);
    out.occl.assign(n, 0);
    out.from.assign(n, -1);
    R.slab.resize((size_t)nl * n * 6);
    R.prim_t.resize((size_t)n * R.n_prims);
    int stride = (int)(0.618 * n) | 1;
    auto gcd = [](int a, int b) { while (b) { const int c = a % b; a = b; b = c; } return a; };
    while (n > 1 && gcd(stride, n) != 1) stride += 2;
    for (int i = 0; i < n; ++i) {
        const Ray &q = rays[(int)(((int64_t)i * stride) % std::max(n, 1))];
        Trav<float> T;
        R.live[i] = trav_begin(T, S, S.root, q.o, q.d, q.tmax) ? 1 : 0;
        R.tmin[i] = T.tmin;
        R.tmax[i] = q.tmax;
        R.anyhit[i] = q.shadow ? 1 : 0;
        out.occl[i] = q.occl ? 1 : 0;
        out.from[i] = q.from;
        if (q.occl) out.origins.insert(out.origins.end(), {q.o.x, q.o.y, q.o.z});
        const float inv[3] = {T.sr.invd.x, T.sr.invd.y, T.sr.invd.z}, oi[3] = {T.sr.oinv.x, T.sr.oinv.y, T.sr.oinv.z};
        for (int l = 0; l < nl; ++l) {
            float *s = &R.slab[((size_t)i * nl + l) * 6];
            for (int a = 0; a < 3; ++a) {
                const bool neg = inv[a] < 0.0f;
                s[a] = vfma(leaves[l].box[neg ? 3 + a : a], inv[a], oi[a]);
                s[3 + a] = -vfma(leaves[l].box[neg ? a : 3 + a], inv[a], oi[a]);
            }
        }
        for (int k = 0; k < R.n_prims; ++k) {
            float u, v;
            R.prim_t[(size_t)i * R.n_prims + k] = prim_t(S, R.prim_ref[k], q.o, q.d, T.tmin, q.tmax, u, v);
        }
    }
    return out;
}


static void write_topology(FlatScene &F, const frt_refine::Topology &t, const std::vector<RefineLeaf> &leaves)
{
    const int L = t.n_leaves, nn = L - 1;
    std::vector<float> box(6 * (size_t)(L + nn));
    std::function<void(int)> bound = [&](int s) {
        float *b = &box[6 * (size_t)s];
        if (s < L) { for (int k = 0; k < 6; ++k) b[k] = leaves[s].box[k]; return; }
        const int c0 = t.child[2 * (s - L)], c1 = t.child[2 * (s - L) + 1];
        bound(c0);
        bound(c1);
        for (int k = 0; k < 3; ++k) {
            b[k] = std::min(box[6 * (size_t)c0 + k], box[6 * (size_t)c1 + k]);
            b[3 + k] = std::max(box[6 * (size_t)c0 + 3 + k], box[6 * (size_t)c1 + 3 + k]);
        }
    };
    bound(t.root);
    std::vector<float4> out(4 * (size_t)nn);
    int next = 0;
    std::function<int(int)> emit = [&](int s) {
        if (s < L) return leaves[s].ref;
        const int me = next++;
        const int c[2] = {t.child[2 * (s - L)], t.child[2 * (s - L) + 1]};
        const float *a = &box[6 * (size_t)c[0]], *b = &box[6 * (size_t)c[1]];
        out[4 * me + 0] = make_float4(a[0], a[1], a[2], a[3]);
        out[4 * me + 1] = make_float4(a[4], a[5], b[0], b[1]);
        out[4 * me + 2] = make_float4(b[2], b[3], b[4], b[5]);
        const int r0 = emit(c[0]), r1 = emit(c[1]);
        out[4 * me + 3] = make_float4(i2f(r0), i2f(r1), 0.0f, 0.0f);
        return me;
    };
    emit(t.root);
    F.nodes.swap(out);
}

bool tree_cost_host(const FlatScene &F, TreeCost &out)
{
    out = TreeCost{};
    out.w = kRefineW;
    if (!tree_in_lds(F) || F.nodes.empty()) return false;
    const TreeView v(F.nodes);
    const Replay val = sample_rays(F, v.leaves, kRefineValFrame, kRefineValSeed);
    const frt_refine::Cost c = frt_refine::tree_cost(v.t, val.R);
    out.V = c.V; out.T = c.T; out.J = frt_refine::cost_j(c, kRefineW);
    out.depth = v.t.depth();
    out.n_rays = val.R.n;
    return true;
}

bool refine_tree(FlatScene &F, int mode)
{
    const int nn = (int)(F.nodes.size() / 4);
    if (!pass_on(mode, "FRT_TREE_REFINE") || !tree_in_lds(F) || nn < 3) return false;
    const TreeView v(F.nodes);
    if (v.t.n_leaves != nn + 1) return false;
    frt_refine::Topology t = v.t;
    const Replay fit = sample_rays(F, v.leaves, kRefineFitFrame, kRefineFitSeed);
    if (frt_refine::refine(t, fit.R, kRefineW, v.t.depth(), kRefineMaxEvals) == 0) return false;
    const Replay val = sample_rays(F, v.leaves, kRefineValFrame, kRefineValSeed);
    const double j0 = frt_refine::cost_j(frt_refine::tree_cost(v.t, val.R), kRefineW);
    const double j1 = frt_refine::cost_j(frt_refine::tree_cost(t, val.R), kRefineW);
    if (!(j1 < j0)) return false;
    write_topology(F, t, v.leaves);
    return true;
}


struct ProofGeometry {
    std::vector<double> tv, tn;
    std::vector<uint8_t> smooth;
    frt_shadow::Geometry g;
};
static void proof_geometry(const frt_scene_view *sv, const FlatScene &F, ProofGeometry &pg)
{
    const int nt = sv->n_tris;
    pg.tv.resize(9 * (size_t)nt);
    pg.smooth.assign(nt, 0);
    bool any_smooth = false;
    for (int d = 0; d < nt; ++d) {
        const int i = F.tri_view[d];
        std::copy(&sv->tri_v[9 * (size_t)i], &sv->tri_v[9 * (size_t)i] + 9, &pg.tv[9 * (size_t)d]);
        pg.smooth[d] = sv->tri_geometry_normal && !sv->tri_geometry_normal[i];
        any_smooth |= pg.smooth[d] != 0;
    }
    if (any_smooth) {
        pg.tn.resize(9 * (size_t)nt);
        for (int d = 0; d < nt; ++d)
            std::copy(&sv->tri_n[9 * (size_t)F.tri_view[d]], &sv->tri_n[9 * (size_t)F.tri_view[d]] + 9, &pg.tn[9 * (size_t)d]);
    }
    frt_shadow::Geometry &g = pg.g;
    g.n_tris = nt; g.n_spheres = sv->n_spheres;
    g.tri_v = pg.tv.data(); g.tri_n = any_smooth ? pg.tn.data() : nullptr; g.tri_smooth = pg.smooth.data();
    g.sphere = sv->sphere;
    g.lights = F.lights.data(); g.n_lights = (int)F.lights.size(); g.sphere_bit = FRT_PRIM_SPHERE;
    for (int k = 0; k < 3; ++k) { g.cam_o[k] = sv->cam_origin[k]; g.cam_u[k] = sv->cam_u[k]; g.cam_v[k] = sv->cam_v[k]; }
    g.lens_r = sv->cam_lens_radius;
    g.eps = (double)Cst<float>::eps;
}

bool shadow_tree(const frt_scene_view *sv, FlatScene &F, int mode)
{
    if (!pass_on(mode, "FRT_SHADOW_TREE")) return false;
    auto &I = F.shadow;
    DevScene &S = F.meta;
    auto why = [&](int w) { I.why = w; return w == FlatScene::kShadowRan; };
    I.nodes_main = (int)(F.nodes.size() / 4);
    if (sv->n_lights <= 0) return why(FlatScene::kShadowNoLights);
    if (!lambertian_only(sv)) return why(FlatScene::kShadowMaterial);
    if (!tree_in_lds(F) || F.nodes.empty()) return why(FlatScene::kShadowNotResident);
    ProofGeometry pg;
    proof_geometry(sv, F, pg);
    frt_shadow::Classified c;
    frt_shadow::classify(pg.g, c);
    if (c.why != frt_shadow::kRan)
        return why(c.why == frt_shadow::kNoLights ? FlatScene::kShadowNoLights : FlatScene::kShadowTooLarge);
    int n_dropped = 0;
    for (int d = 0; d < sv->n_tris; ++d) n_dropped += c.dropped[d];
    if (n_dropped == 0) return why(FlatScene::kShadowNothing);
    std::vector<float> nodes = node_floats(F.nodes);
    frt_shadow::Tree t;
    frt_shadow::build(nodes, S.root, c.dropped, FRT_PRIM_SPHERE, kLeafCountShift, t);
    if (t.dropped_leaves == 0) return why(FlatScene::kShadowNothing);
    if (!keeps_plan(F, I.nodes_main, (int)(nodes.size() / 16), false)) return why(FlatScene::kShadowBudget);
    adopt_nodes(F, nodes);
    S.sroot = t.empty ? kSentinel : t.root;
    I.dropped = c.dropped;
    I.n_dropped = n_dropped; I.rule_a = c.n_rule_a; I.rule_b = c.n_rule_b;
    I.added = t.added; I.shared = t.shared; I.empty = t.empty;
    return why(FlatScene::kShadowRan);
}

bool shadow_cost_host(const FlatScene &F, ShadowCost &out)
{
    out = ShadowCost{};
    if (F.shadow.why != FlatScene::kShadowRan) return false;
    const TreeView v(F.nodes);
    Replay val = sample_rays(F, v.leaves, kRefineValFrame, kRefineValSeed);
    frt_refine::RaySet &R = val.R;
    const std::vector<uint8_t> &occl = val.occl;
    int n_occl = 0;
    for (int i = 0; i < R.n; ++i) n_occl += occl[i];
    out.n_rays = n_occl;
    if (n_occl == 0) return true;
    auto price = [&](int which) {
        const frt_refine::Cost c = frt_refine::tree_cost(v.t, R);
        out.V[which] = c.V * R.n / n_occl;
        out.T[which] = c.T * R.n / n_occl;
    };
    for (int i = 0; i < R.n; ++i) {
        R.live[i] = R.live[i] && occl[i];
        if (occl[i] && !R.live[i]) ++out.stops[0];
    }
    price(0);
    if (F.shadow.empty) {
        out.stops[1] = n_occl;
        return true;
    }
    const int sroot = v.slot(F.meta.sroot);
    const std::vector<int> under = v.leaves_under(sroot);
    auto misses_box = [&](int i) {
        float u[6];
        for (int k = 0; k < 6; ++k) u[k] = __builtin_inff();
        for (int l : under)
            for (int k = 0; k < 6; ++k) u[k] = std::min(u[k], R.slab[((size_t)i * R.n_leaves + l) * 6 + k]);
        const float tn = std::max(std::max(u[0], u[1]), std::max(u[2], Cst<float>::eps));
        const float tf = std::min(std::min(-u[3], -u[4]), std::min(-u[5], R.tmax[i]));
        return !(tn <= tf);
    };
    R.root.assign(R.n, sroot);
    for (int i = 0; i < R.n; ++i) {
        R.live[i] = occl[i];
        if (occl[i] && misses_box(i)) ++out.stops[1];
    }
    price(1);
    return true;
}

void shadow_origins_host(const FlatScene &F, std::vector<float> &origins)
{
    origins.clear();
    if (F.meta.world_kind != FRT_WORLD_BVH || F.nodes.empty()) return;
    origins = sample_rays(F, TreeView(F.nodes).leaves, kRefineValFrame, kRefineValSeed).origins;
}

constexpr int kExitMaxRoot = 1 << 10;

bool exit_tree(const frt_scene_view *sv, FlatScene &F, int mode)
{
    if (!pass_on(mode, "FRT_EXIT_TREE")) return false;
    auto &I = F.exit;
    DevScene &S = F.meta;
    auto why = [&](int w) { I.why = w; return w == FlatScene::kExitRan; };
    I.nodes_before = (int)(F.nodes.size() / 4);
    I.root.assign((size_t)std::max(sv->n_tris, 0), 0);
    if (!lambertian_only(sv)) return why(FlatScene::kExitMaterial);
    if (!tree_in_lds(F) || F.nodes.empty() || S.root != 0) return why(FlatScene::kExitNotResident);
    ProofGeometry pg;
    proof_geometry(sv, F, pg);
    frt_exit::Hidden hid;
    frt_exit::classify(pg.g, hid);
    if (hid.why != frt_exit::kRan) return why(FlatScene::kExitTooLarge);
    std::vector<float> nodes = node_floats(F.nodes);
    std::vector<frt_exit::Class> cls;
    frt_exit::classes(nodes, S.root, FRT_PRIM_SPHERE, kLeafCountShift, hid, cls);
    I.classes = (int)cls.size();
    if (cls.empty()) return why(FlatScene::kExitNothing);

    const TreeView v0(F.nodes);
    Replay fit = sample_rays(F, v0.leaves, kRefineFitFrame, kRefineFitSeed);
    frt_refine::RaySet &R = fit.R;
    const std::vector<uint8_t> live0 = R.live;

    struct Cand { int cls, added; double gain; };
    std::vector<Cand> cand;
    for (int c = 0; c < (int)cls.size(); ++c) {
        std::vector<float> trial = nodes;
        frt_shadow::Tree t;
        frt_shadow::build(trial, S.root, cls[c].dropped, FRT_PRIM_SPHERE, kLeafCountShift, t);
        if (t.empty || t.root <= 0 || t.root >= kExitMaxRoot || t.dropped_leaves == 0) continue;
        const TreeView v(node_records(trial));
        if (!v.same_leaves(v0)) continue;
        bool any = false;
        for (int i = 0; i < R.n; ++i) {
            const int from = fit.from[i];
            const bool mine = from >= 0 && std::binary_search(cls[c].members.begin(), cls[c].members.end(), from);
            R.live[i] = live0[i] && mine;
            any |= R.live[i] != 0;
        }
        if (!any) continue;
        R.root.clear();
        const double j0 = frt_refine::cost_j(frt_refine::tree_cost(v.t, R), kRefineW);
        R.root.assign(R.n, v.slot(t.root));
        const double j1 = frt_refine::cost_j(frt_refine::tree_cost(v.t, R), kRefineW);
        if (j1 < j0) cand.push_back(Cand{c, t.added, j0 - j1});
    }
    if (cand.empty()) return why(FlatScene::kExitNothing);
    std::stable_sort(cand.begin(), cand.end(), [](const Cand &a, const Cand &b) {
        if ((a.added == 0) != (b.added == 0)) return a.added == 0;
        const double ra = a.gain / std::max(a.added, 1), rb = b.gain / std::max(b.added, 1);
        if (ra != rb) return ra > rb;
        return a.gain > b.gain;
    });
    bool refused = false;
    for (const Cand &k : cand) {
        const frt_exit::Class &c = cls[k.cls];
        std::vector<float> next = nodes;
        frt_shadow::Tree t;
        frt_shadow::build(next, S.root, c.dropped, FRT_PRIM_SPHERE, kLeafCountShift, t);
        if (!keeps_plan(F, I.nodes_before, (int)(next.size() / 16), true) || t.root >= kExitMaxRoot) { refused = true; continue; }
        nodes.swap(next);
        for (int d : c.members) I.root[d] = t.root;
        I.taken.push_back({c.sub, t.root, (int)c.members.size(), c.n_dropped, t.added, t.shared, k.gain});
        I.added += t.added;
    }
    if (I.taken.empty()) return why(refused ? FlatScene::kExitBudget : FlatScene::kExitNothing);
    I.budget_refused = refused;
    adopt_nodes(F, nodes);
    for (size_t d = 0; d < I.root.size(); ++d)
        if (I.root[d]) F.tshade[2 * d + 1].z = i2f(I.root[d]);
    return why(FlatScene::kExitRan);
}

bool exit_cost_host(const FlatScene &F, ExitCost &out)
{
    out = ExitCost{};
    if (!tree_in_lds(F) || F.nodes.empty()) return false;
    const TreeView v(F.nodes);
    Replay val = sample_rays(F, v.leaves, kRefineValFrame, kRefineValSeed);
    frt_refine::RaySet &R = val.R;
    const std::vector<uint8_t> &occl = val.occl;
    const std::vector<int> &from = val.from;
    const DevScene &S = F.meta;
    const std::vector<uint8_t> live0 = R.live;
    out.n_rays = R.n;
    for (int i = 0; i < R.n; ++i) out.n_ext += from[i] >= 0;
    for (int on = 0; on < 2; ++on) {
        R.root.assign(R.n, v.t.root);
        R.live = live0;
        for (int i = 0; i < R.n; ++i) {
            if (occl[i] && S.sroot != S.root) {
                if (S.sroot == kSentinel) R.live[i] = 0;
                else { R.root[i] = v.slot(S.sroot); R.live[i] = 1; }
            } else if (on && from[i] >= 0 && from[i] < (int)F.exit.root.size() && F.exit.root[from[i]]) {
                R.root[i] = v.slot(F.exit.root[from[i]]);
            }
        }
        const frt_refine::Cost all = frt_refine::tree_cost(v.t, R);
        out.V_all[on] = all.V; out.T_all[on] = all.T; out.J_all[on] = frt_refine::cost_j(all, kRefineW);
        for (int i = 0; i < R.n; ++i) R.live[i] = R.live[i] && from[i] >= 0;
        const frt_refine::Cost ext = frt_refine::tree_cost(v.t, R);
        if (out.n_ext > 0) { out.V_ext[on] = ext.V * R.n / out.n_ext; out.T_ext[on] = ext.T * R.n / out.n_ext; }
    }
    return true;
}
```

### first_raytracer_amd/csrc/frt_tree_passes.hpp

```cpp
#pragma once
#include "frt_flatten.hpp"

#pragma GCC visibility push(hidden)
bool refine_tree(FlatScene &F, int mode);
bool shadow_tree(const frt_scene_view *sv, FlatScene &F, int mode);
bool exit_tree(const frt_scene_view *sv, FlatScene &F, int mode);

struct ExitCost {
    double V_all[2] = {0, 0}, T_all[2] = {0, 0}, J_all[2] = {0, 0}, V_ext[2] = {0, 0}, T_ext[2] = {0, 0};
    int n_rays = 0, n_ext = 0;
};
bool exit_cost_host(const FlatScene &F, ExitCost &out);
struct ShadowCost { double V[2] = {0, 0}, T[2] = {0, 0}; int n_rays = 0, stops[2] = {0, 0}; };
bool shadow_cost_host(const FlatScene &F, ShadowCost &out);
void shadow_origins_host(const FlatScene &F, std::vector<float> &origins);
struct TreeCost { double V = 0.0, T = 0.0, J = 0.0, w = 0.0; int depth = 0, n_rays = 0; };
bool tree_cost_host(const FlatScene &F, TreeCost &out);
#pragma GCC visibility pop
```

### first_raytracer_amd/csrc/host/shadow_tree.cpp

```cpp
#include "shadow_tree.hpp"

#include <algorithm>
#include <cmath>

namespace frt_shadow {
namespace {

constexpr double kU = 1.0 / 16777216.0;
constexpr double kNoise = 32.0, kOnPlane = 8.0, kMaxAspect = 8.0;

struct V { double x, y, z; };
inline V sub(V a, V b) { return V{a.x - b.x, a.y - b.y, a.z - b.z}; }
inline double dot(V a, V b) { return a.x * b.x + a.y * b.y + a.z * b.z; }
inline V cross(V a, V b) { return V{a.y * b.z - a.z * b.y, a.z * b.x - a.x * b.z, a.x * b.y - a.y * b.x}; }
inline double len(V a) { return std::sqrt(dot(a, a)); }
inline V at(const double *p) { return V{p[0], p[1], p[2]}; }

}

void classify(const Geometry &g, Classified &out)
{
    out = Classified{};
    out.dropped.assign((size_t)std::max(g.n_tris, 0), 0);
    if (g.n_lights <= 0) { out.why = kNoLights; return; }
    double lo[3] = {1e300, 1e300, 1e300}, hi[3] = {-1e300, -1e300, -1e300};
    auto grow = [&](const double *p, double r) {
        for (int k = 0; k < 3; ++k) { lo[k] = std::min(lo[k], p[k] - r); hi[k] = std::max(hi[k], p[k] + r); }
    };
    for (int i = 0; i < 3 * g.n_tris; ++i) grow(&g.tri_v[3 * i], 0.0);
    for (int i = 0; i < g.n_spheres; ++i) grow(&g.sphere[4 * i], g.sphere[4 * i + 3]);
    grow(g.cam_o, std::fabs(g.lens_r));
    double M = 0.0, Dm = 0.0;
    for (int k = 0; k < 3; ++k) {
        M = std::max(M, std::max(std::fabs(lo[k]), std::fabs(hi[k])));
        Dm += (hi[k] - lo[k]) * (hi[k] - lo[k]);
    }
    Dm = std::sqrt(Dm);
    if (!(kNoise * kU * Dm <= 0.25 * g.eps) || !(M < 1e30)) { out.why = kTooLarge; return; }
    const double tol = kOnPlane * kU * M;
    const double lens = std::fabs(g.lens_r);

    std::vector<V> ng((size_t)g.n_tris);
    std::vector<uint8_t> flat((size_t)g.n_tris, 0);
    for (int i = 0; i < g.n_tris; ++i) {
        const double *v = &g.tri_v[9 * i];
        const V c = cross(sub(at(v + 3), at(v)), sub(at(v + 6), at(v)));
        const double l = len(c);
        if (l > 0.0) ng[i] = V{c.x / l, c.y / l, c.z / l};
        else { ng[i] = V{0, 0, 0}; flat[i] = 1; }
    }
    auto smooth = [&](int i) { return g.tri_smooth && g.tri_smooth[i]; };
    auto light_is_sphere = [&](int ref) { return (ref & g.sphere_bit) != 0; };

    for (int p = 0; p < g.n_tris; ++p) {
        if (flat[p]) continue;
        const double *pv = &g.tri_v[9 * p];
        const V v0 = at(pv), e1 = sub(at(pv + 3), v0), e2 = sub(at(pv + 6), v0), m = ng[p];
        const double rho = len(e1) * len(e2) / len(cross(e1, e2));
        if (!(rho <= kMaxAspect)) continue;
        const double E = kNoise * kU * rho * Dm, D = 4.0 * E / g.eps;
        auto s = [&](const double *x) { return dot(m, sub(at(x), v0)); };

        bool rule_b = false;
        for (int k = 0; k < 3 && !rule_b; ++k) {
            const double c = pv[k];
            bool ok = pv[3 + k] == c && pv[6 + k] == c;
            for (int l = 0; l < g.n_lights && ok; ++l) {
                const int ref = g.lights[l];
                if (light_is_sphere(ref)) { ok = false; break; }
                const double *lv = &g.tri_v[9 * ref];
                ok = lv[k] == c && lv[3 + k] == c && lv[6 + k] == c;
            }
            rule_b = ok;
        }
        if (rule_b) { out.dropped[p] = 1; ++out.n_rule_b; continue; }

        for (int side = 1; side >= -1 && !out.dropped[p]; side -= 2) {
            const double sg = (double)side;
            bool ok = true;
            for (int i = 0; i < 3 * g.n_tris && ok; ++i) ok = sg * s(&g.tri_v[3 * i]) >= -tol;
            for (int i = 0; i < g.n_spheres && ok; ++i) ok = sg * s(&g.sphere[4 * i]) - g.sphere[4 * i + 3] >= -tol;
            if (ok) {
                const double a = dot(m, at(g.cam_u)), b = dot(m, at(g.cam_v));
                ok = sg * s(g.cam_o) - lens * std::sqrt(a * a + b * b) >= -tol;
            }
            for (int q = 0; q < g.n_tris && ok; ++q) {
                const double *qv = &g.tri_v[9 * q];
                bool leans;
                if (smooth(q)) {
                    leans = false;
                    for (int j = 0; j < 3; ++j) leans |= !(sg * dot(m, at(&g.tri_n[9 * q + 3 * j])) >= 0.0);
                } else {
                    leans = flat[q] || !(-sg * dot(m, ng[q]) * g.eps <= E);
                }
                if (leans) ok = std::min(std::min(sg * s(qv), sg * s(qv + 3)), sg * s(qv + 6)) >= 2.0 * g.eps;
            }
            for (int i = 0; i < g.n_spheres && ok; ++i)
                ok = sg * s(&g.sphere[4 * i]) - g.sphere[4 * i + 3] >= 2.0 * g.eps;
            for (int l = 0; l < g.n_lights && ok; ++l) {
                const int ref = g.lights[l];
                if (light_is_sphere(ref)) {
                    const double *q = &g.sphere[4 * (ref & ~g.sphere_bit)];
                    ok = sg * s(q) - q[3] >= D;
                } else {
                    const double *lv = &g.tri_v[9 * ref];
                    ok = std::min(std::min(sg * s(lv), sg * s(lv + 3)), sg * s(lv + 6)) >= D;
                }
            }
            if (ok) { out.dropped[p] = 1; ++out.n_rule_a; }
        }
    }
}

void build(std::vector<float> &nodes, int main_root, const std::vector<uint8_t> &dropped, int sphere_bit,
           int count_shift, Tree &out)
{
    out = Tree{};
    auto ref_of = [&](int i, int side) {
        int r;
        const float f = nodes[16 * (size_t)i + 12 + side];
        static_assert(sizeof(r) == sizeof(f), "refs are stored as int bits");
        std::copy(reinterpret_cast<const char *>(&f), reinterpret_cast<const char *>(&f) + sizeof(f), reinterpret_cast<char *>(&r));
        return r;
    };
    auto leaf_kept = [&](int lref) {
        if (lref & sphere_bit) return true;
        const int first = lref & ((1 << count_shift) - 1), count = (lref >> count_shift) + 1;
        for (int k = 0; k < count; ++k)
            if (first + k >= (int)dropped.size() || !dropped[first + k]) return true;
        return false;
    };
    struct Sub { bool empty, same; int ref; float box[6]; int n_nodes; };
    struct Rec {
        std::vector<float> &nodes;
        decltype(ref_of) &ref;
        decltype(leaf_kept) &kept;
        Tree &out;
        Sub visit(int r, const float *box)
        {
            Sub s{};
            for (int k = 0; k < 6; ++k) s.box[k] = box[k];
            s.ref = r;
            if (r < 0) {
                s.same = true;
                s.empty = !kept(~r);
                ++(s.empty ? out.dropped_leaves : out.kept_leaves);
                return s;
            }
            float b0[6], b1[6];
            for (int k = 0; k < 6; ++k) { b0[k] = nodes[16 * (size_t)r + k]; b1[k] = nodes[16 * (size_t)r + 6 + k]; }
            const Sub a = visit(ref(r, 0), b0), b = visit(ref(r, 1), b1);
            if (a.empty && b.empty) { s.empty = true; return s; }
            if (a.empty || b.empty) { Sub c = a.empty ? b : a; c.same = false; return c; }
            if (a.same && b.same) { s.same = true; s.n_nodes = 1 + a.n_nodes + b.n_nodes; return s; }
            out.shared += a.n_nodes + b.n_nodes;
            s.ref = (int)(nodes.size() / 16);
            float rec[16] = {0};
            for (int k = 0; k < 6; ++k) { rec[k] = a.box[k]; rec[6 + k] = b.box[k]; }
            const int refs[2] = {a.ref, b.ref};
            std::copy(reinterpret_cast<const char *>(refs), reinterpret_cast<const char *>(refs) + sizeof(refs),
                      reinterpret_cast<char *>(&rec[12]));
            nodes.insert(nodes.end(), rec, rec + 16);
            ++out.added;
            for (int k = 0; k < 3; ++k) { s.box[k] = std::min(a.box[k], b.box[k]); s.box[3 + k] = std::max(a.box[3 + k], b.box[3 + k]); }
            return s;
        }
    } rec{nodes, ref_of, leaf_kept, out};
    const float no_box[6] = {0, 0, 0, 0, 0, 0};
    const Sub r = rec.visit(main_root, no_box);
    out.shared += r.n_nodes;
    out.empty = r.empty;
    out.root = r.empty ? main_root : r.ref;
}

}
```

### first_raytracer_amd/csrc/host/shadow_tree.hpp

```cpp
#pragma once
#include <cstdint>
#include <vector>

namespace frt_shadow {

struct Geometry {
    int n_tris = 0, n_spheres = 0;
    const double *tri_v = nullptr;
    const double *tri_n = nullptr;
    const uint8_t *tri_smooth = nullptr;
    const double *sphere = nullptr;
    const int *lights = nullptr;
    int n_lights = 0, sphere_bit = 0;
    double cam_o[3] = {0, 0, 0}, cam_u[3] = {0, 0, 0}, cam_v[3] = {0, 0, 0}, lens_r = 0.0;
    double eps = 0.0;
};

enum Why { kRan = 0, kNoLights, kTooLarge };
struct Classified {
    int why = kRan;
    std::vector<uint8_t> dropped;
    int n_rule_a = 0, n_rule_b = 0;
};
void classify(const Geometry &g, Classified &out);

struct Tree {
    int root = 0;
    bool empty = false;
    int added = 0, shared = 0;
    int kept_leaves = 0, dropped_leaves = 0;
};
void build(std::vector<float> &nodes, int main_root, const std::vector<uint8_t> &dropped, int sphere_bit,
           int count_shift, Tree &out);

}
```

### first_raytracer_amd/csrc/host/tree_refine.cpp

```cpp
#include "tree_refine.hpp"

#include <algorithm>
#include <cstddef>
#include <cstring>
#include <utility>
#include <vector>

#include "frt.h"

namespace frt_refine {
namespace {

constexpr int kMaxLevels = 64;
constexpr int kChunks = 16;
constexpr double kSlack = 0.002;

struct Tables {
    int n_slots = 0;
    std::vector<float> tab;
};

inline void unite(const float *a, const float *b, float *out)
{
    for (int k = 0; k < 6; ++k) out[k] = std::min(a[k], b[k]);
}

void count_rays(const Topology &t, const RaySet &R, const Tables &tb, const int *dirty, int n_dirty, const int *local_of,
                int r0, int r1, uint64_t &V, uint64_t &T)
{
    const int L = t.n_leaves;
    const int *child = t.child.data();
    float loc[2 * kMaxLevels][6];
    for (int r = r0; r < r1; ++r) {
        if (!R.live[r]) continue;
        const float *base = &tb.tab[(size_t)r * tb.n_slots * 6];
        auto rec = [&](int s) { return n_dirty > 0 && local_of[s] >= 0 ? loc[local_of[s]] : base + 6 * s; };
        for (int k = 0; k < n_dirty; ++k) {
            const int j = dirty[k] - L;
            unite(rec(child[2 * j]), rec(child[2 * j + 1]), loc[k]);
        }
        const float tmin = R.tmin[r];
        const bool any = R.anyhit[r] != 0;
        const float *pt = &R.prim_t[(size_t)r * R.n_prims];
        float tb_ = R.tmax[r];
        int hp = -1, sp = 0, node = R.root.empty() ? t.root : R.root[r];
        int stk[kMaxLevels];
        for (;;) {
            while (node >= L) {
                ++V;
                const int c0 = child[2 * (node - L)], c1 = child[2 * (node - L) + 1];
                const float *a = rec(c0), *b = rec(c1);
                const float t0 = std::max(std::max(a[0], a[1]), std::max(a[2], tmin));
                const float f0 = std::min(std::min(-a[3], -a[4]), std::min(-a[5], tb_));
                const float t1 = std::max(std::max(b[0], b[1]), std::max(b[2], tmin));
                const float f1 = std::min(std::min(-b[3], -b[4]), std::min(-b[5], tb_));
                const bool h0 = t0 <= f0, h1 = t1 <= f1;
                if (h0 && h1) {
                    const bool first0 = t0 <= t1;
                    stk[sp++] = first0 ? c1 : c0;
                    node = first0 ? c0 : c1;
                } else if (h0) {
                    node = c0;
                } else if (h1) {
                    node = c1;
                } else {
                    node = sp > 0 ? stk[--sp] : -1;
                }
            }
            if (node < 0) break;
            bool done = false;
            for (int k = R.prim_first[node]; k < R.prim_first[node + 1]; ++k) {
                ++T;
                const float th = pt[k];
                const int ref = R.prim_ref[k];
                const bool sph = (ref & FRT_PRIM_SPHERE) != 0;
                if (th > 0.0f && th <= tb_ && (th < tb_ || (sph ? hp >= 0 : ref < hp))) {
                    tb_ = th;
                    hp = ref;
                    if (any) { done = true; break; }
                }
            }
            if (done || sp == 0) break;
            node = stk[--sp];
        }
    }
}

void build_tables(const Topology &t, const RaySet &R, Tables &tb)
{
    const int L = t.n_leaves, nI = (int)(t.child.size() / 2);
    tb.n_slots = L + nI;
    tb.tab.resize((size_t)R.n * tb.n_slots * 6);
    std::vector<int> order, roots{t.root};
    roots.insert(roots.end(), R.root.begin(), R.root.end());
    std::sort(roots.begin(), roots.end());
    roots.erase(std::unique(roots.begin(), roots.end()), roots.end());
    std::vector<char> seen(tb.n_slots, 0);
    std::vector<std::pair<int, bool>> st;
    for (int root : roots) st.push_back({root, false});
    while (!st.empty()) {
        const auto [s, done] = st.back();
        st.pop_back();
        if (s < L) continue;
        if (done) { order.push_back(s); continue; }
        if (seen[s]) continue;
        seen[s] = 1;
        st.push_back({s, true});
        st.push_back({t.child[2 * (s - L)], false});
        st.push_back({t.child[2 * (s - L) + 1], false});
    }
    for (int r = 0; r < R.n; ++r) {
        float *base = &tb.tab[(size_t)r * tb.n_slots * 6];
        memcpy(base, &R.slab[(size_t)r * L * 6], sizeof(float) * 6 * L);
        for (size_t k = 0; k < order.size(); ++k) {
            const int s = order[k], j = s - L;
            unite(base + 6 * t.child[2 * j], base + 6 * t.child[2 * j + 1], base + 6 * s);
        }
    }
}

}

int Topology::depth() const
{
    int d = 0, sp = 0;
    int st[2 * kMaxLevels][2];
    st[sp][0] = root; st[sp++][1] = 1;
    while (sp > 0) {
        const int s = st[--sp][0], lvl = st[sp][1];
        if (s < n_leaves) continue;
        d = std::max(d, lvl);
        if (lvl >= kMaxLevels) return lvl;
        st[sp][0] = child[2 * (s - n_leaves)]; st[sp++][1] = lvl + 1;
        st[sp][0] = child[2 * (s - n_leaves) + 1]; st[sp++][1] = lvl + 1;
    }
    return d;
}

Cost tree_cost(const Topology &t, const RaySet &R)
{
    Tables tb;
    build_tables(t, R, tb);
    uint64_t V = 0, T = 0;
    count_rays(t, R, tb, nullptr, 0, nullptr, 0, R.n, V, T);
    Cost c;
    if (R.n > 0) { c.V = (double)V / R.n; c.T = (double)T / R.n; }
    return c;
}

int refine(Topology &t, const RaySet &R, double w, int max_depth, int max_evals)
{
    const int L = t.n_leaves, nI = L - 1, nS = L + nI;
    if (nI < 2 || R.n <= 0 || max_depth >= kMaxLevels) return 0;
    Tables tb;
    std::vector<int> parent(nS, -1), local_of(nS, -1);
    int bound[kChunks + 1];
    for (int c = 0; c <= kChunks; ++c) bound[c] = (int)((int64_t)R.n * c / kChunks);
    double prefix[kChunks + 1] = {0.0};
    auto keep_tree = [&]() {
        std::fill(parent.begin(), parent.end(), -1);
        for (int j = 0; j < nI; ++j) { parent[t.child[2 * j]] = L + j; parent[t.child[2 * j + 1]] = L + j; }
        build_tables(t, R, tb);
        uint64_t V = 0, T = 0;
        for (int c = 0; c < kChunks; ++c) {
            count_rays(t, R, tb, nullptr, 0, nullptr, bound[c], bound[c + 1], V, T);
            prefix[c + 1] = (double)V + w * (double)T;
        }
    };
    keep_tree();
    auto in_subtree = [&](int x, int s) {
        for (; x >= 0; x = parent[x]) if (x == s) return true;
        return false;
    };
    auto side_of = [&](int par, int c) { return 2 * (par - L) + (t.child[2 * (par - L)] == c ? 0 : 1); };
    auto move = [&](int s, int x) {
        const int p = parent[s];
        const int q = t.child[side_of(p, s) ^ 1];
        const int g = parent[p];
        if (g < 0) t.root = q;
        else t.child[side_of(g, p)] = q;
        parent[q] = g;
        const int xp = parent[x];
        if (xp < 0) t.root = p;
        else t.child[side_of(xp, x)] = p;
        parent[p] = xp;
        t.child[2 * (p - L)] = x;
        t.child[2 * (p - L) + 1] = s;
        parent[x] = p;
        parent[s] = p;
        return g;
    };
    int evals = 0, kept = 0;
    bool improved = true;
    while (improved && evals < max_evals) {
        improved = false;
        for (int s = 0; s < nS && evals < max_evals; ++s) {
            if (parent[s] < 0) continue;
            int best_x = -1;
            double best_j = prefix[kChunks];
            const Topology keep = t;
            const std::vector<int> keep_parent = parent;
            const int p = parent[s], q = t.child[side_of(p, s) ^ 1];
            for (int x = 0; x < nS && evals < max_evals; ++x) {
                if (x == p || x == q || in_subtree(x, s)) continue;
                const int g = move(s, x);
                if (t.depth() <= max_depth) {
                    ++evals;
                    std::pair<int, int> dl[2 * kMaxLevels];
                    int nd = 0;
                    for (int start : {p, g})
                        for (int y = start; y >= 0; y = parent[y]) {
                            int lvl = 0;
                            for (int z = y; z >= 0; z = parent[z]) ++lvl;
                            dl[nd++] = {-lvl, y};
                        }
                    std::sort(dl, dl + nd);
                    nd = (int)(std::unique(dl, dl + nd) - dl);
                    int dirty[2 * kMaxLevels];
                    for (int k = 0; k < nd; ++k) { dirty[k] = dl[k].second; local_of[dirty[k]] = k; }
                    uint64_t V = 0, T = 0;
                    const double slack = kSlack * prefix[kChunks];
                    double j = 0.0;
                    bool ok = true;
                    for (int c = 0; c < kChunks && ok; ++c) {
                        count_rays(t, R, tb, dirty, nd, local_of.data(), bound[c], bound[c + 1], V, T);
                        j = (double)V + w * (double)T;
                        ok = j <= prefix[c + 1] + slack;
                    }
                    for (int k = 0; k < nd; ++k) local_of[dirty[k]] = -1;
                    if (ok && j < best_j) { best_j = j; best_x = x; }
                }
                t = keep;
                parent = keep_parent;
            }
            if (best_x < 0) continue;
            move(s, best_x);
            keep_tree();
            ++kept;
            improved = true;
        }
    }
    return kept;
}

}
```

### first_raytracer_amd/csrc/host/tree_refine.hpp

```cpp
#pragma once
#include <cstdint>
#include <vector>

namespace frt_refine {

struct RaySet {
    int n = 0, n_leaves = 0, n_prims = 0;
    std::vector<float> tmin, tmax;
    std::vector<uint8_t> anyhit, live;
    std::vector<float> slab;
    std::vector<int> prim_first;
    std::vector<int> prim_ref;
    std::vector<float> prim_t;
    std::vector<int> root;
};

struct Topology {
    int n_leaves = 0, root = 0;
    std::vector<int> child;
    int depth() const;
};

struct Cost { double V = 0.0, T = 0.0; };
inline double cost_j(const Cost &c, double w) { return c.V + w * c.T; }

Cost tree_cost(const Topology &t, const RaySet &rays);

int refine(Topology &t, const RaySet &fit, double w, int max_depth, int max_evals);

}
```

### include/frt.h

```cpp
#ifndef FRT_H
#define FRT_H

#include <stdint.h>

#ifdef __cplusplus
extern "C" {
#endif

#define FRT_ABI_VERSION 9

enum {
    FRT_OK = 0,
    FRT_E_INVALID = -1,
    FRT_E_HIP = -2,
    FRT_E_NO_SCENE = -3,
    FRT_E_UNSUPPORTED = -4,
    FRT_E_IO = -5,
    FRT_E_NO_DEVICE = -6
};

enum { FRT_WORLD_BVH = 0, FRT_WORLD_LIST = 1 };
enum { FRT_MAT_LAMBERTIAN = 0,
       FRT_MAT_DIFFUSE_LIGHT = 1,
       FRT_MAT_MODIFIED_PHONG = 2,
       FRT_MAT_METAL = 3,
       FRT_MAT_DIELECTRIC = 4,
       FRT_MAT_ROUGH_CONDUCTOR = 5 };
enum { FRT_DIST_GGX = 0, FRT_DIST_BECKMANN = 1 };
enum { FRT_INTEGRATOR_PATH = 0,
       FRT_INTEGRATOR_PSSMLT = 1,
       FRT_INTEGRATOR_AO = 2,
       FRT_INTEGRATOR_NORMALS = 3,
       FRT_INTEGRATOR_ALBEDO = 4,
       FRT_INTEGRATOR_DEPTH = 5,
       FRT_INTEGRATOR_DENOISE = 6,
       FRT_INTEGRATOR_ERROR = 8      };
enum { FRT_FLAG_NO_LDS_SCENE = 1,
       FRT_FLAG_WAVES5 = 2,
       FRT_FLAG_WAVES6 = 4,
       FRT_FLAG_WAVES4 = 8,
       FRT_FLAG_BVH2 = 16,
       FRT_FLAG_NO_OCT = 256,
       FRT_FLAG_FP64 = 512,
       FRT_FLAG_FP32 = 1024,
       FRT_FLAG_ENV_SAMPLING = 2048,
       FRT_FLAG_ROULETTE = 4096,
       FRT_FLAG_SOBOL = 8192 };




enum { FRT_PRECISION_AUTO = 0, FRT_PRECISION_FP32 = 1, FRT_PRECISION_FP64 = 2 };

#define FRT_PRIM_SPHERE (1 << 30)

typedef struct frt_material {
    int32_t type;
    int32_t distribution;
    double albedo[3];
    double emit[3];
    double specular[3];
    double exponent;
    double ior;
    double alpha;
    double eta[3], k[3];
    int32_t texture;
    int32_t image;
    double tex_odd[3];
    double tex_scale[2];
} frt_material;
enum { FRT_TEX_CONSTANT = 0, FRT_TEX_CHECKER = 1, FRT_TEX_IMAGE = 2 };

enum { FRT_IMAGE_SRGB8 = 0, FRT_IMAGE_F32 = 1 };
typedef struct frt_image {
    int32_t nx, ny;
    int32_t format;
    int32_t reserved;
    const void *data;
} frt_image;

typedef struct frt_scene_view {
    int32_t world_kind;
    int32_t n_tris;
    const double *tri_v;
    const double *tri_n;
    const int32_t *tri_material;
    const uint8_t *tri_geometry_normal;
    const double *tri_inv_area;
    int32_t n_spheres;
    const double *sphere;
    const int32_t *sphere_material;
    int32_t n_materials;
    const frt_material *materials;
    int32_t n_nodes;
    int32_t root;
    const double *node_box;
    const int32_t *node_child;
    int32_t n_list;
    const int32_t *list;
    int32_t n_lights;
    const int32_t *lights;
    double cam_origin[3], cam_lower_left[3], cam_horizontal[3], cam_vertical[3];
    double cam_u[3], cam_v[3];
    double cam_lens_radius;
    double env_color[3];
    double cam_w[3];
    double cam_half_height;
    const double *tri_uv;
    int32_t n_images;
    const frt_image *images;
} frt_scene_view;

typedef struct frt_render_params {
    int32_t nx, ny;
    int32_t spp;
    uint32_t seed;
    int32_t max_depth;
    int32_t integrator;
    int32_t tile_size;
    int32_t shard_index;
    int32_t shard_count;
    int32_t samples_per_item;
    int32_t flags;
    int32_t mlt_chains;
    int32_t mlt_bootstrap;
    int32_t sample_offset;
} frt_render_params;

typedef struct frt_stats {
    uint64_t camera_rays;
    uint64_t extension_rays;
    uint64_t shadow_rays;
    uint64_t samples;
    uint64_t pixels;
    uint64_t work_items;
    double kernel_ms;
    double total_ms;
    uint32_t scene_in_lds;
    uint32_t waves_cap;
    uint32_t stack_entries;
    uint32_t bvh_depth;
    uint64_t scene_bytes;
    uint32_t fp64;
    uint32_t reserved;
} frt_stats;

int frt_get_abi_version(void);

typedef struct frt_ctx frt_ctx;
int frt_create(int hip_device, frt_ctx **out);
int frt_destroy(frt_ctx *ctx);
const char *frt_last_error(const frt_ctx *ctx);
int frt_set_precision(frt_ctx *ctx, int precision);

int frt_set_env_image(frt_ctx *ctx, const frt_image *img);

int frt_upload_scene(frt_ctx *ctx, const frt_scene_view *scene);

int64_t frt_shard_slot_count(const frt_render_params *p);
int frt_shard_slots(const frt_render_params *p, int32_t *slot_pixel);

int frt_render(frt_ctx *ctx, const frt_render_params *p, float *film_rgb, frt_stats *st);

int frt_render_multi(frt_ctx **ctxs, int n, const frt_render_params *p, float *film_rgb, frt_stats *st);

int frt_render_device(frt_ctx *ctx, const frt_render_params *p, float *slots_rgb, void *hip_stream,
                      frt_stats *st);

int frt_mlt_chain_state(frt_ctx *ctx, uint64_t first, uint64_t n, float *u_out, uint32_t *fp_out);

int frt_trace_device(frt_ctx *ctx, const float *rays, int64_t n, float *hits, int flags, void *hip_stream,
                     frt_stats *st);

typedef struct frt_host_scene frt_host_scene;
typedef struct frt_host_scene_info {
    int32_t n_tris, n_spheres, n_materials, n_lights, n_nodes, world_kind, n_list, bvh_depth;
    double load_ms, build_ms;
} frt_host_scene_info;
int frt_scene_create(const char *kind, const char *obj_path, double aspect, frt_host_scene **out);
int frt_scene_view_get(const frt_host_scene *s, frt_scene_view *view);

enum { FRT_SPHERE_WORLD = 1, FRT_SPHERE_LIGHTS = 2, FRT_SPHERE_BOTH = 3 };
int frt_scene_new(frt_host_scene **out);
int frt_scene_add_obj(frt_host_scene *s, const char *obj_path, const double *to_world16, const frt_material *bsdf,
                      int use_geometry_normals);
int frt_scene_add_sphere(frt_host_scene *s, const double *center, double radius, const frt_material *m, int where);
int frt_scene_set_camera(frt_host_scene *s, const double *lookfrom, const double *lookat, const double *vup,
                         double vfov, double aspect, double aperture, double focus_dist);
int frt_scene_set_env(frt_host_scene *s, const double *rgb);
int frt_scene_add_image(frt_host_scene *s, const frt_image *img, int *index);
int frt_scene_set_env_image(frt_host_scene *s, int index);
int frt_scene_env_image(const frt_host_scene *s, frt_image *out);
int frt_scene_finish(frt_host_scene *s, int world_kind);
enum { FRT_GPU_BVH_PLOC = 0, FRT_GPU_BVH_LBVH = 1, FRT_GPU_BVH_SAH = 2 };
int frt_scene_build_bvh_gpu(frt_host_scene *s, frt_ctx *ctx, double *device_ms);
int frt_scene_build_bvh_gpu_algo(frt_host_scene *s, frt_ctx *ctx, int algo, double *device_ms);
int frt_scene_build_bvh_sah(frt_host_scene *s);
int frt_scene_info(const frt_host_scene *s, frt_host_scene_info *info);
void frt_scene_destroy(frt_host_scene *s);

int frt_write_tessellated_obj(const char *src_obj, int k, const char *dst_obj);

int frt_read_hdr(const char *path, int32_t *nx, int32_t *ny, float *rgb);

int frt_write_pfm(const char *path, int nx, int ny, const float *rgb);

int frt_film_accumulate(float *acc, int64_t acc_spp, const float *pass, int64_t pass_spp, int64_t n);
int frt_tonemap_u8(const float *rgb, int nx, int ny, uint8_t *out_u8);
enum { FRT_IMAGE_PNG = 0, FRT_IMAGE_BMP = 1, FRT_IMAGE_JPG = 2 };
int frt_write_image(const char *path, int nx, int ny, const uint8_t *rgb_u8, int format);

int frt_selftest_path_host(const frt_scene_view *scene, const frt_render_params *p, const int32_t *pixels,
                           int npix, float *out_rgb, frt_stats *st);
int frt_selftest_path_host_env(const frt_scene_view *scene, const frt_render_params *p, const int32_t *pixels,
                               int npix, const frt_image *env, float *out_rgb, frt_stats *st);
int frt_selftest_mlt_paths_host(const frt_scene_view *scene, int nx, int ny, uint32_t seed, int n, float *out6);
typedef struct frt_tree_cost {
    double v, t, j, w;
    int32_t depth, n_nodes, n_rays, applies;
} frt_tree_cost;
int frtx_selftest_tree_refine(const frt_scene_view *scene, frt_tree_cost out[2], float *nodes_off, float *nodes_on,
                             int32_t max_nodes);
typedef struct frt_shadow_tree_info {
    int32_t why, kept_prims, dropped_prims, rule_a, rule_b;
    int32_t nodes_main, nodes_added, nodes_shared, root, empty;
    int32_t n_rays, root_stops_main, root_stops_shadow, n_nodes;
    double v_main, t_main, v_shadow, t_shadow;
    int64_t segments, segment_hits;
} frt_shadow_tree_info;
int frtx_selftest_shadow_tree(const frt_scene_view *scene, frt_shadow_tree_info *out, uint8_t *dropped, float *nodes,
                              int32_t max_nodes, int64_t segments, uint32_t seed);
typedef struct frt_exit_tree_info {
    int32_t why, classes, taken, budget_refused;
    int32_t nodes_off, n_nodes, nodes_added, depth_off, depth_on, n_rays, n_ext, reserved;
    int64_t lds_bytes, lds_bytes_oct, lds_cap, lds_cap_oct;
    double v_all[2], t_all[2], j_all[2], v_ext[2], t_ext[2];
} frt_exit_tree_info;
int frtx_selftest_exit_tree(const frt_scene_view *scene, int32_t mode, frt_exit_tree_info *out, int32_t *roots,
                            int32_t *view_of, int32_t *taken, int32_t max_taken, float *nodes_off, float *nodes_on,
                            int32_t max_nodes);
int frtx_selftest_trace_host(const frt_scene_view *scene, const float *rays, int64_t n, float *hits);
int frtx_selftest_chunk_variance(const float *partial, int n_chunks, int64_t n_slots, int spp, int spi, float *out);
typedef struct frt_plan_query {
    int32_t kind, integrator, flags;
    int32_t world_kind, stack_needed, has_bvh4, depth4;
    int32_t mats, has_spec_mats, env_image, env_sampling, has_f64, precision;
    int64_t scene_lds_bytes, scene_lds_bytes_oct;
} frt_plan_query;
typedef struct frt_plan_answer {
    int32_t rc, stack, waves, lds_scene, wide, f64;
    int64_t lds, scene_lds;
    int64_t lds_boot;
    uint64_t kernel, kernel_boot;
} frt_plan_answer;
int frtx_selftest_plan(const frt_plan_query *q, frt_plan_answer *a);
int frtx_render_pixels(frt_ctx *ctx, const frt_render_params *p, const int32_t *pixels, int64_t npix,
                       float *out_rgb, float *out_var, frt_stats *st);
int frtx_render_pixels_device(frt_ctx *ctx, const frt_render_params *p, const int32_t *pixels, int64_t npix,
                              float *out_rgb, float *out_var, void *hip_stream, frt_stats *st);
int frtx_radiance_rays(frt_ctx *ctx, const frt_render_params *p, const float *rays, int64_t n,
                       float *out_rgb, float *out_var, frt_stats *st);
int frtx_radiance_rays_device(frt_ctx *ctx, const frt_render_params *p, const float *rays, int64_t n,
                              float *out_rgb, float *out_var, void *hip_stream, frt_stats *st);
int frtx_camera_rays_device(frt_ctx *ctx, const frt_render_params *p, const int32_t *pixels, int64_t npix,
                            float *rays_out, void *hip_stream);
int frtx_selftest_radiance_host(const frt_scene_view *scene, const frt_render_params *p, const float *rays, int64_t n,
                                const frt_image *env, float *out_rgb, frt_stats *st);
int frtx_selftest_camera_rays_host(const frt_scene_view *scene, const frt_render_params *p, const int32_t *pixels,
                                   int64_t npix, float *rays_out);

#ifdef __cplusplus
}
#endif
#endif
```

Before: 41010.

## Jointly plan main, shadow and exit BVH trees with a priced host search

Replaces the standalone tree-refine pass with a joint tree planner that prices the main, shadow and exit trees together using replayed sample paths, and adds a wave-level SIMD traversal simulator to estimate divergent per-wave cost. The main-tree topology used for BVH4 derivation can now differ from the binary tree that carries the appended subtrees. The aim is to pick tree shapes that cut traversal node and leaf visits per wave in the LDS-resident scene. It adds host preprocessing time and more complex tree-construction logic, and the planner is on by default unless FRT_TREE_PLAN=0.

```diff
diff --git a/first_raytracer_amd/__init__.py b/first_raytracer_amd/__init__.py
--- a/first_raytracer_amd/__init__.py
+++ b/first_raytracer_amd/__init__.py
@@ -183,6 +183,19 @@
         return {k: (list(getattr(self, k)) if t is ctypes.c_double * 2 else getattr(self, k)) for k, t in self._fields_}
 
 
+class TreePlanInfo(ctypes.Structure):
+    _fields_ = [(n, ctypes.c_int32) for n in ("mode", "priced", "searched", "accepted", "evals", "kept", "priced_sroot",
+                                              "built_sroot", "priced_appended", "built_appended", "priced_served",
+                                              "built_served", "shadow_added", "nodes_main", "n_nodes", "depth_in",
+                                              "depth")] + [("n_kind", ctypes.c_int32 * 4), ("reserved", ctypes.c_int32)] + [
+        (n, ctypes.c_double) for n in ("j_parent", "j_plan", "j_main_in", "j_main")] + [
+        (n, ctypes.c_double * 4) for n in ("v", "t", "j")] + [("pass_seconds", ctypes.c_double)]
+
+    def as_dict(self):
+        return {k: (getattr(self, k) if isinstance(getattr(self, k), (int, float)) else list(getattr(self, k)))
+                for k, _ in self._fields_}
+
+
 class PlanQuery(ctypes.Structure):
     _fields_ = [(n, ctypes.c_int32) for n in ("kind", "integrator", "flags", "world_kind", "stack_needed", "has_bvh4",
                                               "depth4", "mats", "has_spec_mats", "env_image", "env_sampling",
@@ -218,7 +231,7 @@
 EXPORTS_X = ("frtx_selftest_tree_refine", "frtx_selftest_trace_host", "frtx_selftest_chunk_variance",
              "frtx_selftest_plan", "frtx_selftest_shadow_tree", "frtx_render_pixels", "frtx_render_pixels_device",
              "frtx_selftest_exit_tree", "frtx_radiance_rays", "frtx_radiance_rays_device", "frtx_camera_rays_device",
-             "frtx_selftest_radiance_host", "frtx_selftest_camera_rays_host")
+             "frtx_selftest_radiance_host", "frtx_selftest_camera_rays_host", "frtx_selftest_tree_plan", "frtx_selftest_wave_model")
 
 
 def lib():
@@ -303,6 +316,10 @@
                                                   ctypes.POINTER(Image), vp, ctypes.POINTER(Stats)]
         L.frtx_selftest_camera_rays_host.argtypes = [ctypes.POINTER(SceneView), ctypes.POINTER(RenderParams), vp,
                                                      ctypes.c_int64, vp]
+    if hasattr(L, "frtx_selftest_wave_model"):
+        L.frtx_selftest_wave_model.argtypes = [ctypes.POINTER(SceneView), ctypes.POINTER(ctypes.c_double)]
+    if hasattr(L, "frtx_selftest_tree_plan"):
+        L.frtx_selftest_tree_plan.argtypes = [ctypes.POINTER(SceneView), ctypes.POINTER(TreePlanInfo), vp, vp, vp, ctypes.c_int32]
     _lib = L
     return L
 
@@ -843,6 +860,28 @@
             nodes[0, :out.nodes_off].copy(), nodes[1, :out.n_nodes].copy())
 
 
+def selftest_tree_plan(scene):
+    view = scene.view()
+    cap = max(4 * int(view.n_nodes), 1) + 16
+    nodes = np.zeros((cap, 16), np.float32)
+    roots = np.zeros((2, max(int(view.n_tris), 1)), np.int32)
+    out = TreePlanInfo()
+    _check(lib().frtx_selftest_tree_plan(ctypes.byref(view), ctypes.byref(out), roots[0].ctypes.data, roots[1].ctypes.data,
+                                         nodes.ctypes.data, cap), "frtx_selftest_tree_plan")
+    n = int(view.n_tris)
+    return out.as_dict(), roots[0, :n].copy(), roots[1, :n].copy(), nodes[:out.n_nodes].copy()
+
+
+WAVE_MODEL_FIELDS = ("node_trips", "leaf_trips", "step_trips", "shade_trips", "node_util", "leaf_util", "step_util", "cost", "rays")
+
+
+def selftest_wave_model(scene):
+    out = (ctypes.c_double * 9)()
+    view = scene.view()
+    _check(lib().frtx_selftest_wave_model(ctypes.byref(view), out), "frtx_selftest_wave_model")
+    return dict(zip(WAVE_MODEL_FIELDS, out))
+
+
 def selftest_trace_host(scene, rays):
     rays = np.ascontiguousarray(rays, dtype=np.float32).reshape(-1, 8)
     hits = np.zeros((len(rays), 4), np.float32)
diff --git a/first_raytracer_amd/csrc/frt_flatten.hip b/first_raytracer_amd/csrc/frt_flatten.hip
--- a/first_raytracer_amd/csrc/frt_flatten.hip
+++ b/first_raytracer_amd/csrc/frt_flatten.hip
@@ -509,7 +509,9 @@
     S.sroot = S.root;
     auto derive_trees = [&]() {
         fill_octants(F);
+        if (!F.plan.main_root_nodes.empty()) F.nodes.swap(F.plan.main_root_nodes);
         F.has4 = sv->world_kind == FRT_WORLD_BVH && build_bvh4(F, S.root);
+        if (!F.plan.main_root_nodes.empty()) F.nodes.swap(F.plan.main_root_nodes);
         if (!F.has4) F.nodes4.clear();
         S.root4 = F.has4 ? F.root4 : S.root;
         S.n_nodes4 = (int)(F.nodes4.size() / kNode4Parts);
@@ -539,7 +541,7 @@
     S.cam64_h = d3d(sv->cam_horizontal); S.cam64_v = d3d(sv->cam_vertical);
     S.cam64_u = d3d(sv->cam_u); S.cam64_vv = d3d(sv->cam_v);
     S.lens_r64 = sv->cam_lens_radius;
-    bool again = refine_tree(F, refine);
+    bool again = refine_tree(sv, F, refine);
     again |= shadow_tree(sv, F, shadow);
     again |= exit_tree(sv, F, exit);
     if (again) derive_trees();
diff --git a/first_raytracer_amd/csrc/frt_flatten.hpp b/first_raytracer_amd/csrc/frt_flatten.hpp
--- a/first_raytracer_amd/csrc/frt_flatten.hpp
+++ b/first_raytracer_amd/csrc/frt_flatten.hpp
@@ -39,6 +39,16 @@
         int nodes_before = 0, added = 0;
         bool budget_refused = false;
     } exit;
+    struct {
+        int mode = 0;
+        bool priced = false, searched = false, accepted = false;
+        int evals = 0, kept = 0;
+        double j_parent = 0.0, j_plan = 0.0;
+        double j_main_in = 0.0, j_main = 0.0;
+        int sroot = 0, appended = 0, served = 0;
+        std::vector<int> exit_root;
+        std::vector<float4> main_root_nodes;
+    } plan;
 };
 
 int flatten_scene(const frt_scene_view *sv, FlatScene &F, std::string &err, bool f64, int refine = -1, int shadow = -1,
diff --git a/first_raytracer_amd/csrc/frt_selftest.hip b/first_raytracer_amd/csrc/frt_selftest.hip
--- a/first_raytracer_amd/csrc/frt_selftest.hip
+++ b/first_raytracer_amd/csrc/frt_selftest.hip
@@ -1,4 +1,5 @@
 #include <algorithm>
+#include <chrono>
 #include <cstring>
 #include <string>
 #include <vector>
@@ -358,6 +359,64 @@
     return FRT_OK;
 }
 
+extern "C" int frtx_selftest_tree_plan(const frt_scene_view *sv, frt_tree_plan_info *out, int32_t *roots_priced,
+                                       int32_t *roots_built, float *nodes, int32_t max_nodes)
+{
+    if (!sv || !out) return FRT_E_INVALID;
+    memset(out, 0, sizeof(*out));
+    using clk = std::chrono::steady_clock;
+    FlatScene F0, F;
+    std::string err;
+    const auto t0 = clk::now();
+    int rc = flatten_scene(sv, F0, err, false, 0, 0, 0);
+    const auto t1 = clk::now();
+    if (rc == FRT_OK) rc = flatten_scene(sv, F, err, false);
+    const auto t2 = clk::now();
+    if (rc != FRT_OK) return rc;
+    out->pass_seconds = std::chrono::duration<double>(t2 - t1).count() - std::chrono::duration<double>(t1 - t0).count();
+    const auto &I = F.plan;
+    out->mode = I.mode; out->priced = I.priced; out->searched = I.searched; out->accepted = I.accepted;
+    out->evals = I.evals; out->kept = I.kept;
+    out->j_parent = I.j_parent; out->j_plan = I.j_plan; out->j_main_in = I.j_main_in; out->j_main = I.j_main;
+    out->n_nodes = (int32_t)(F.nodes.size() / 4);
+    out->nodes_main = (int32_t)(F0.nodes.size() / 4);
+    out->priced_sroot = I.sroot; out->built_sroot = F.meta.sroot;
+    out->priced_appended = I.appended; out->built_appended = out->n_nodes - out->nodes_main;
+    out->priced_served = I.served;
+    out->shadow_added = F.shadow.why == FlatScene::kShadowRan ? F.shadow.added : 0;
+    out->depth_in = F0.depth;
+    for (int d = 0; d < sv->n_tris; ++d) {
+        const int b = d < (int)F.exit.root.size() ? F.exit.root[d] : 0, p = d < (int)I.exit_root.size() ? I.exit_root[d] : 0;
+        out->built_served += b != 0;
+        if (roots_built) roots_built[F.tri_view[d]] = b;
+        if (roots_priced) roots_priced[F.tri_view[d]] = p;
+    }
+    if (nodes) {
+        if (out->n_nodes > max_nodes) return FRT_E_INVALID;
+        memcpy(nodes, F.nodes.data(), F.nodes.size() * sizeof(float4));
+    }
+    PlanCost c;
+    if (plan_cost_host(F, c)) {
+        out->depth = c.depth;
+        for (int k = 0; k < 4; ++k) { out->v[k] = c.V[k]; out->t[k] = c.T[k]; out->j[k] = c.J[k]; out->n_kind[k] = c.n[k]; }
+    }
+    return FRT_OK;
+}
+
+extern "C" int frtx_selftest_wave_model(const frt_scene_view *sv, double *out)
+{
+    if (!sv || !out) return FRT_E_INVALID;
+    FlatScene F;
+    std::string err;
+    const int rc = flatten_scene(sv, F, err, false);
+    if (rc != FRT_OK) return rc;
+    WaveCost c;
+    if (!wave_cost_host(F, c)) return FRT_E_UNSUPPORTED;
+    const double v[9] = {c.node_trips, c.leaf_trips, c.step_trips, c.shade_trips, c.node_util, c.leaf_util, c.step_util, c.cost, c.rays};
+    memcpy(out, v, sizeof(v));
+    return FRT_OK;
+}
+
 extern "C" int frtx_selftest_trace_host(const frt_scene_view *sv, const float *rays, int64_t n, float *hits)
 {
     if (!sv || n < 0 || (n > 0 && (!rays || !hits))) return FRT_E_INVALID;
diff --git a/first_raytracer_amd/csrc/frt_tree_passes.hip b/first_raytracer_amd/csrc/frt_tree_passes.hip
--- a/first_raytracer_amd/csrc/frt_tree_passes.hip
+++ b/first_raytracer_amd/csrc/frt_tree_passes.hip
@@ -4,12 +4,15 @@
 #include <cstdlib>
 #include <cstring>
 #include <functional>
+#include <limits>
 #include <unordered_map>
 
 #include "frt_kernels.hpp"
 #include "host/exit_tree.hpp"
 #include "host/shadow_tree.hpp"
+#include "host/tree_plan.hpp"
 #include "host/tree_refine.hpp"
+#include "host/wave_model.hpp"
 
 using namespace frt;
 
@@ -19,6 +22,11 @@
     return !(e && std::atoi(e) == 0);
 }
 static bool pass_on(int mode, const char *name) { return mode < 0 ? knob(name) : mode != 0; }
+static int plan_mode()
+{
+    const char *e = std::getenv("FRT_TREE_PLAN");
+    return (e && std::atoi(e) == 0) ? 0 : 1;
+}
 
 static bool lambertian_only(const frt_scene_view *sv)
 {
@@ -75,9 +83,14 @@
     frt_refine::Topology t;
     std::vector<RefineLeaf> leaves;
     std::unordered_map<int, int> leaf_of;
-
-    explicit TreeView(const std::vector<float4> &nodes)
+    bool foreign = false;
+
+    explicit TreeView(const std::vector<float4> &nodes, const std::vector<RefineLeaf> *numbering = nullptr)
     {
+        if (numbering) {
+            leaves = *numbering;
+            for (size_t l = 0; l < leaves.size(); ++l) leaf_of.emplace(leaves[l].ref, (int)l);
+        }
         const int nn = (int)(nodes.size() / 4);
         t.child.assign(2 * (size_t)nn, 0);
         for (int i = 0; i < nn; ++i) {
@@ -88,6 +101,7 @@
                 if (c >= 0) { t.child[2 * i + side] = ~c; continue; }
                 const auto [it, fresh] = leaf_of.emplace(c, (int)leaves.size());
                 if (fresh) {
+                    foreign |= numbering != nullptr;
                     RefineLeaf l;
                     for (int k = 0; k < 6; ++k) l.box[k] = b[side][k];
                     l.ref = c;
@@ -133,16 +147,21 @@
     std::vector<uint8_t> occl;
     std::vector<int> from;
     std::vector<float> origins;
+    std::vector<int> path_first;
+    std::vector<int> path_ray;
 };
-static Replay sample_rays(const FlatScene &F, const std::vector<RefineLeaf> &leaves, int frame, uint32_t seed)
+static Replay sample_rays(const FlatScene &F, const std::vector<RefineLeaf> &leaves, int frame, uint32_t seed, int spp = 1)
 {
     const DevScene S = host_scene(F);
     struct Ray { f3 o, d; float tmax; bool shadow, occl; int from; };
     std::vector<Ray> rays;
     std::vector<int> stack(std::max(F.depth + 1, 1));
-    for (int pix = 0; pix < frame * frame; ++pix) {
+    std::vector<int> path_first;
+    for (int path = 0; path < frame * frame * spp; ++path) {
+        const int pix = path / spp;
+        path_first.push_back((int)rays.size());
         PathState<float> P;
-        path_begin<kMatsAll>(P, S, pix % frame, pix / frame, frame, frame, seed, (uint32_t)pix, 0u);
+        path_begin<kMatsAll>(P, S, pix % frame, pix / frame, frame, frame, seed, (uint32_t)pix, (uint32_t)(path % spp));
         int last = -1;
         for (;;) {
             rays.push_back(Ray{P.ro, P.rd, P.rtmax, P.shadow, light_shadow_ray(P),
@@ -153,8 +172,11 @@
             if (path_shade<kMatsAll>(P, S, h, kRefineMaxDepth, n_ext, n_sh)) break;
         }
     }
+    path_first.push_back((int)rays.size());
     const int n = (int)rays.size(), nl = (int)leaves.size();
     Replay out;
+    out.path_first.swap(path_first);
+    out.path_ray.assign(n, 0);
     frt_refine::RaySet &R = out.R;
     R.n = n;
     R.n_leaves = nl;
@@ -177,6 +199,7 @@
     while (n > 1 && gcd(stride, n) != 1) stride += 2;
     for (int i = 0; i < n; ++i) {
         const Ray &q = rays[(int)(((int64_t)i * stride) % std::max(n, 1))];
+        out.path_ray[(int)(((int64_t)i * stride) % std::max(n, 1))] = i;
         Trav<float> T;
         R.live[i] = trav_begin(T, S, S.root, q.o, q.d, q.tmax) ? 1 : 0;
         R.tmin[i] = T.tmin;
@@ -203,7 +226,7 @@
 }
 
 
-static void write_topology(FlatScene &F, const frt_refine::Topology &t, const std::vector<RefineLeaf> &leaves)
+static std::vector<float4> topology_nodes(const frt_refine::Topology &t, const std::vector<RefineLeaf> &leaves)
 {
     const int L = t.n_leaves, nn = L - 1;
     std::vector<float> box(6 * (size_t)(L + nn));
@@ -234,7 +257,7 @@
         return me;
     };
     emit(t.root);
-    F.nodes.swap(out);
+    return out;
 }
 
 bool tree_cost_host(const FlatScene &F, TreeCost &out)
@@ -251,23 +274,6 @@
     return true;
 }
 
-bool refine_tree(FlatScene &F, int mode)
-{
-    const int nn = (int)(F.nodes.size() / 4);
-    if (!pass_on(mode, "FRT_TREE_REFINE") || !tree_in_lds(F) || nn < 3) return false;
-    const TreeView v(F.nodes);
-    if (v.t.n_leaves != nn + 1) return false;
-    frt_refine::Topology t = v.t;
-    const Replay fit = sample_rays(F, v.leaves, kRefineFitFrame, kRefineFitSeed);
-    if (frt_refine::refine(t, fit.R, kRefineW, v.t.depth(), kRefineMaxEvals) == 0) return false;
-    const Replay val = sample_rays(F, v.leaves, kRefineValFrame, kRefineValSeed);
-    const double j0 = frt_refine::cost_j(frt_refine::tree_cost(v.t, val.R), kRefineW);
-    const double j1 = frt_refine::cost_j(frt_refine::tree_cost(t, val.R), kRefineW);
-    if (!(j1 < j0)) return false;
-    write_topology(F, t, v.leaves);
-    return true;
-}
-
 
 struct ProofGeometry {
     std::vector<double> tv, tn;
@@ -301,36 +307,58 @@
     g.eps = (double)Cst<float>::eps;
 }
 
+struct ShadowProof {
+    int why = FlatScene::kShadowOff;
+    frt_shadow::Classified c;
+    int n_dropped = 0;
+};
+static void shadow_proof(const frt_scene_view *sv, const FlatScene &F, int mode, ShadowProof &P)
+{
+    P = ShadowProof{};
+    if (!pass_on(mode, "FRT_SHADOW_TREE")) return;
+    if (sv->n_lights <= 0) { P.why = FlatScene::kShadowNoLights; return; }
+    if (!lambertian_only(sv)) { P.why = FlatScene::kShadowMaterial; return; }
+    if (!tree_in_lds(F) || F.nodes.empty()) { P.why = FlatScene::kShadowNotResident; return; }
+    ProofGeometry pg;
+    proof_geometry(sv, F, pg);
+    frt_shadow::classify(pg.g, P.c);
+    if (P.c.why != frt_shadow::kRan) {
+        P.why = P.c.why == frt_shadow::kNoLights ? FlatScene::kShadowNoLights : FlatScene::kShadowTooLarge;
+        return;
+    }
+    for (int d = 0; d < sv->n_tris; ++d) P.n_dropped += P.c.dropped[d];
+    P.why = P.n_dropped == 0 ? FlatScene::kShadowNothing : FlatScene::kShadowRan;
+}
+static int shadow_derive(const FlatScene &F, std::vector<float> &nodes, const ShadowProof &P, frt_shadow::Tree &t)
+{
+    if (P.why != FlatScene::kShadowRan) return P.why;
+    const int nn_main = (int)(nodes.size() / 16);
+    std::vector<float> next = nodes;
+    frt_shadow::build(next, F.meta.root, P.c.dropped, FRT_PRIM_SPHERE, kLeafCountShift, t);
+    if (t.dropped_leaves == 0) return FlatScene::kShadowNothing;
+    if (!keeps_plan(F, nn_main, (int)(next.size() / 16), false)) return FlatScene::kShadowBudget;
+    nodes.swap(next);
+    return FlatScene::kShadowRan;
+}
+
 bool shadow_tree(const frt_scene_view *sv, FlatScene &F, int mode)
 {
-    if (!pass_on(mode, "FRT_SHADOW_TREE")) return false;
     auto &I = F.shadow;
     DevScene &S = F.meta;
-    auto why = [&](int w) { I.why = w; return w == FlatScene::kShadowRan; };
+    ShadowProof P;
+    shadow_proof(sv, F, mode, P);
+    if (P.why == FlatScene::kShadowOff) return false;
     I.nodes_main = (int)(F.nodes.size() / 4);
-    if (sv->n_lights <= 0) return why(FlatScene::kShadowNoLights);
-    if (!lambertian_only(sv)) return why(FlatScene::kShadowMaterial);
-    if (!tree_in_lds(F) || F.nodes.empty()) return why(FlatScene::kShadowNotResident);
-    ProofGeometry pg;
-    proof_geometry(sv, F, pg);
-    frt_shadow::Classified c;
-    frt_shadow::classify(pg.g, c);
-    if (c.why != frt_shadow::kRan)
-        return why(c.why == frt_shadow::kNoLights ? FlatScene::kShadowNoLights : FlatScene::kShadowTooLarge);
-    int n_dropped = 0;
-    for (int d = 0; d < sv->n_tris; ++d) n_dropped += c.dropped[d];
-    if (n_dropped == 0) return why(FlatScene::kShadowNothing);
     std::vector<float> nodes = node_floats(F.nodes);
     frt_shadow::Tree t;
-    frt_shadow::build(nodes, S.root, c.dropped, FRT_PRIM_SPHERE, kLeafCountShift, t);
-    if (t.dropped_leaves == 0) return why(FlatScene::kShadowNothing);
-    if (!keeps_plan(F, I.nodes_main, (int)(nodes.size() / 16), false)) return why(FlatScene::kShadowBudget);
+    I.why = shadow_derive(F, nodes, P, t);
+    if (I.why != FlatScene::kShadowRan) return false;
     adopt_nodes(F, nodes);
     S.sroot = t.empty ? kSentinel : t.root;
-    I.dropped = c.dropped;
-    I.n_dropped = n_dropped; I.rule_a = c.n_rule_a; I.rule_b = c.n_rule_b;
+    I.dropped = P.c.dropped;
+    I.n_dropped = P.n_dropped; I.rule_a = P.c.n_rule_a; I.rule_b = P.c.n_rule_b;
     I.added = t.added; I.shared = t.shared; I.empty = t.empty;
-    return why(FlatScene::kShadowRan);
+    return true;
 }
 
 bool shadow_cost_host(const FlatScene &F, ShadowCost &out)
@@ -388,80 +416,134 @@
 
 constexpr int kExitMaxRoot = 1 << 10;
 
-bool exit_tree(const frt_scene_view *sv, FlatScene &F, int mode)
-{
-    if (!pass_on(mode, "FRT_EXIT_TREE")) return false;
-    auto &I = F.exit;
-    DevScene &S = F.meta;
-    auto why = [&](int w) { I.why = w; return w == FlatScene::kExitRan; };
-    I.nodes_before = (int)(F.nodes.size() / 4);
-    I.root.assign((size_t)std::max(sv->n_tris, 0), 0);
-    if (!lambertian_only(sv)) return why(FlatScene::kExitMaterial);
-    if (!tree_in_lds(F) || F.nodes.empty() || S.root != 0) return why(FlatScene::kExitNotResident);
+struct ExitProof {
+    int why = FlatScene::kExitOff;
+    frt_exit::Hidden hid;
+};
+static void exit_proof(const frt_scene_view *sv, const FlatScene &F, int mode, ExitProof &P)
+{
+    P = ExitProof{};
+    if (!pass_on(mode, "FRT_EXIT_TREE")) return;
+    if (!lambertian_only(sv)) { P.why = FlatScene::kExitMaterial; return; }
+    if (!tree_in_lds(F) || F.nodes.empty() || F.meta.root != 0) { P.why = FlatScene::kExitNotResident; return; }
     ProofGeometry pg;
     proof_geometry(sv, F, pg);
-    frt_exit::Hidden hid;
-    frt_exit::classify(pg.g, hid);
-    if (hid.why != frt_exit::kRan) return why(FlatScene::kExitTooLarge);
-    std::vector<float> nodes = node_floats(F.nodes);
+    frt_exit::classify(pg.g, P.hid);
+    P.why = P.hid.why != frt_exit::kRan ? FlatScene::kExitTooLarge : FlatScene::kExitRan;
+}
+
+struct ExitChoice {
+    int classes = 0, added = 0;
+    bool refused = false;
+    std::vector<FlatScene::ExitClass> taken;
+    std::vector<int> root;
+};
+static int exit_derive(const FlatScene &F, std::vector<float> &nodes, const ExitProof &P, const std::vector<RefineLeaf> &leaves,
+                       Replay &fit, int share_from, bool share, ExitChoice &out)
+{
+    out = ExitChoice{};
+    out.root.assign((size_t)P.hid.n, 0);
+    if (P.why != FlatScene::kExitRan) return P.why;
+    const int root = F.meta.root, nodes_before = (int)(nodes.size() / 16), from_node = share ? share_from : -1;
     std::vector<frt_exit::Class> cls;
-    frt_exit::classes(nodes, S.root, FRT_PRIM_SPHERE, kLeafCountShift, hid, cls);
-    I.classes = (int)cls.size();
-    if (cls.empty()) return why(FlatScene::kExitNothing);
-
-    const TreeView v0(F.nodes);
-    Replay fit = sample_rays(F, v0.leaves, kRefineFitFrame, kRefineFitSeed);
+    frt_exit::classes(nodes, root, FRT_PRIM_SPHERE, kLeafCountShift, P.hid, cls);
+    out.classes = (int)cls.size();
+    if (cls.empty()) return FlatScene::kExitNothing;
+
     frt_refine::RaySet &R = fit.R;
     const std::vector<uint8_t> live0 = R.live;
-
+    const std::vector<int> root0 = R.root;
+    std::vector<int> class_of((size_t)P.hid.n, -1);
+    for (int c = 0; c < (int)cls.size(); ++c)
+        for (int d : cls[c].members) class_of[d] = c;
+    std::vector<std::vector<int>> rays_of(cls.size());
+    for (int i = 0; i < R.n; ++i) {
+        const int from = fit.from[i];
+        if (live0[i] && from >= 0 && from < P.hid.n && class_of[from] >= 0) rays_of[class_of[from]].push_back(i);
+    }
     struct Cand { int cls, added; double gain; };
     std::vector<Cand> cand;
     for (int c = 0; c < (int)cls.size(); ++c) {
+        if (rays_of[c].empty()) continue;
         std::vector<float> trial = nodes;
         frt_shadow::Tree t;
-        frt_shadow::build(trial, S.root, cls[c].dropped, FRT_PRIM_SPHERE, kLeafCountShift, t);
+        frt_shadow::build(trial, root, cls[c].dropped, FRT_PRIM_SPHERE, kLeafCountShift, t, from_node);
         if (t.empty || t.root <= 0 || t.root >= kExitMaxRoot || t.dropped_leaves == 0) continue;
-        const TreeView v(node_records(trial));
-        if (!v.same_leaves(v0)) continue;
-        bool any = false;
-        for (int i = 0; i < R.n; ++i) {
-            const int from = fit.from[i];
-            const bool mine = from >= 0 && std::binary_search(cls[c].members.begin(), cls[c].members.end(), from);
-            R.live[i] = live0[i] && mine;
-            any |= R.live[i] != 0;
-        }
-        if (!any) continue;
+        const TreeView v(node_records(trial), &leaves);
+        if (v.foreign) continue;
+        std::fill(R.live.begin(), R.live.end(), 0);
+        for (int i : rays_of[c]) R.live[i] = 1;
         R.root.clear();
         const double j0 = frt_refine::cost_j(frt_refine::tree_cost(v.t, R), kRefineW);
         R.root.assign(R.n, v.slot(t.root));
         const double j1 = frt_refine::cost_j(frt_refine::tree_cost(v.t, R), kRefineW);
         if (j1 < j0) cand.push_back(Cand{c, t.added, j0 - j1});
     }
-    if (cand.empty()) return why(FlatScene::kExitNothing);
+    R.live = live0;
+    R.root = root0;
+    if (cand.empty()) return FlatScene::kExitNothing;
     std::stable_sort(cand.begin(), cand.end(), [](const Cand &a, const Cand &b) {
         if ((a.added == 0) != (b.added == 0)) return a.added == 0;
         const double ra = a.gain / std::max(a.added, 1), rb = b.gain / std::max(b.added, 1);
         if (ra != rb) return ra > rb;
         return a.gain > b.gain;
     });
-    bool refused = false;
     for (const Cand &k : cand) {
         const frt_exit::Class &c = cls[k.cls];
         std::vector<float> next = nodes;
         frt_shadow::Tree t;
-        frt_shadow::build(next, S.root, c.dropped, FRT_PRIM_SPHERE, kLeafCountShift, t);
-        if (!keeps_plan(F, I.nodes_before, (int)(next.size() / 16), true) || t.root >= kExitMaxRoot) { refused = true; continue; }
+        frt_shadow::build(next, root, c.dropped, FRT_PRIM_SPHERE, kLeafCountShift, t, from_node);
+        if (!keeps_plan(F, nodes_before, (int)(next.size() / 16), true) || t.root >= kExitMaxRoot) { out.refused = true; continue; }
         nodes.swap(next);
-        for (int d : c.members) I.root[d] = t.root;
-        I.taken.push_back({c.sub, t.root, (int)c.members.size(), c.n_dropped, t.added, t.shared, k.gain});
-        I.added += t.added;
-    }
-    if (I.taken.empty()) return why(refused ? FlatScene::kExitBudget : FlatScene::kExitNothing);
-    I.budget_refused = refused;
+        for (int d : c.members) out.root[d] = t.root;
+        out.taken.push_back({c.sub, t.root, (int)c.members.size(), c.n_dropped, t.added, t.shared, k.gain});
+        out.added += t.added;
+    }
+    if (out.taken.empty()) return out.refused ? FlatScene::kExitBudget : FlatScene::kExitNothing;
+    return FlatScene::kExitRan;
+}
+
+bool exit_tree(const frt_scene_view *sv, FlatScene &F, int mode)
+{
+    auto &I = F.exit;
+    ExitProof P;
+    exit_proof(sv, F, mode, P);
+    if (P.why == FlatScene::kExitOff) return false;
+    I.nodes_before = (int)(F.nodes.size() / 4);
+    I.root.assign((size_t)std::max(sv->n_tris, 0), 0);
+    I.why = P.why;
+    if (P.why != FlatScene::kExitRan) return false;
+    const TreeView v0(F.nodes);
+    Replay fit = sample_rays(F, v0.leaves, kRefineFitFrame, kRefineFitSeed);
+    std::vector<float> nodes = node_floats(F.nodes);
+    ExitChoice c;
+    const int first_appended = F.shadow.why == FlatScene::kShadowRan ? F.shadow.nodes_main : I.nodes_before;
+    I.why = exit_derive(F, nodes, P, v0.leaves, fit, first_appended, plan_mode() != 0, c);
+    I.classes = c.classes;
+    if (I.why != FlatScene::kExitRan) return false;
+    I.taken = c.taken; I.added = c.added; I.budget_refused = c.refused;
+    for (size_t d = 0; d < I.root.size() && d < c.root.size(); ++d) I.root[d] = c.root[d];
     adopt_nodes(F, nodes);
     for (size_t d = 0; d < I.root.size(); ++d)
         if (I.root[d]) F.tshade[2 * d + 1].z = i2f(I.root[d]);
-    return why(FlatScene::kExitRan);
+    return true;
+}
+
+static void start_rays(const TreeView &v, Replay &rp, const std::vector<uint8_t> &live0, int main_root, int sroot,
+                       const std::vector<int> *exit_root)
+{
+    frt_refine::RaySet &R = rp.R;
+    R.root.assign(R.n, v.t.root);
+    R.live = live0;
+    for (int i = 0; i < R.n; ++i) {
+        const int from = rp.from[i];
+        if (rp.occl[i] && sroot != main_root) {
+            if (sroot == kSentinel) R.live[i] = 0;
+            else { R.root[i] = v.slot(sroot); R.live[i] = 1; }
+        } else if (exit_root && from >= 0 && from < (int)exit_root->size() && (*exit_root)[from]) {
+            R.root[i] = v.slot((*exit_root)[from]);
+        }
+    }
 }
 
 bool exit_cost_host(const FlatScene &F, ExitCost &out)
@@ -471,23 +553,13 @@
     const TreeView v(F.nodes);
     Replay val = sample_rays(F, v.leaves, kRefineValFrame, kRefineValSeed);
     frt_refine::RaySet &R = val.R;
-    const std::vector<uint8_t> &occl = val.occl;
     const std::vector<int> &from = val.from;
     const DevScene &S = F.meta;
     const std::vector<uint8_t> live0 = R.live;
     out.n_rays = R.n;
     for (int i = 0; i < R.n; ++i) out.n_ext += from[i] >= 0;
     for (int on = 0; on < 2; ++on) {
-        R.root.assign(R.n, v.t.root);
-        R.live = live0;
-        for (int i = 0; i < R.n; ++i) {
-            if (occl[i] && S.sroot != S.root) {
-                if (S.sroot == kSentinel) R.live[i] = 0;
-                else { R.root[i] = v.slot(S.sroot); R.live[i] = 1; }
-            } else if (on && from[i] >= 0 && from[i] < (int)F.exit.root.size() && F.exit.root[from[i]]) {
-                R.root[i] = v.slot(F.exit.root[from[i]]);
-            }
-        }
+        start_rays(v, val, live0, S.root, S.sroot, on ? &F.exit.root : nullptr);
         const frt_refine::Cost all = frt_refine::tree_cost(v.t, R);
         out.V_all[on] = all.V; out.T_all[on] = all.T; out.J_all[on] = frt_refine::cost_j(all, kRefineW);
         for (int i = 0; i < R.n; ++i) R.live[i] = R.live[i] && from[i] >= 0;
@@ -496,3 +568,198 @@
     }
     return true;
 }
+
+bool plan_cost_host(const FlatScene &F, PlanCost &out)
+{
+    out = PlanCost{};
+    if (!tree_in_lds(F) || F.nodes.empty()) return false;
+    const TreeView v(F.nodes);
+    Replay val = sample_rays(F, v.leaves, kRefineValFrame, kRefineValSeed);
+    frt_refine::RaySet &R = val.R;
+    const DevScene &S = F.meta;
+    const std::vector<uint8_t> live0 = R.live;
+    start_rays(v, val, live0, S.root, S.sroot, &F.exit.root);
+    const std::vector<uint8_t> live = R.live;
+    const bool shadow_root = S.sroot != S.root;
+    for (int k = 0; k < 4; ++k) {
+        for (int i = 0; i < R.n; ++i) {
+            const int kind = (val.occl[i] && shadow_root) ? 2 : val.from[i] >= 0 ? 3 : 1;
+            const bool mine = k == 0 || kind == k;
+            out.n[k] += mine;
+            R.live[i] = live[i] && mine;
+        }
+        const frt_refine::Cost c = frt_refine::tree_cost(v.t, R);
+        const double per = out.n[k] > 0 ? (double)R.n / out.n[k] : 0.0;
+        out.V[k] = c.V * per; out.T[k] = c.T * per; out.J[k] = frt_refine::cost_j(c, kRefineW) * per;
+    }
+    const int nn_main = F.shadow.why == FlatScene::kShadowRan ? F.shadow.nodes_main
+                      : F.exit.why == FlatScene::kExitRan ? F.exit.nodes_before : (int)(F.nodes.size() / 4);
+    out.depth = TreeView(std::vector<float4>(F.nodes.begin(), F.nodes.begin() + 4 * (size_t)nn_main)).t.depth();
+    return true;
+}
+
+constexpr int kWaveSpp = 4;
+bool wave_cost_host(const FlatScene &F, WaveCost &out)
+{
+    out = WaveCost{};
+    if (!tree_in_lds(F) || F.nodes.empty()) return false;
+    const TreeView v(F.nodes);
+    Replay rp = sample_rays(F, v.leaves, kRefineValFrame, kRefineValSeed, kWaveSpp);
+    const std::vector<uint8_t> live0 = rp.R.live;
+    start_rays(v, rp, live0, F.meta.root, F.meta.sroot, &F.exit.root);
+    frt_wave::Steps st;
+    frt_refine::ray_steps(v.t, rp.R, st.first, st.nodes, st.prims);
+    st.shadow = rp.R.anyhit;
+    frt_wave::Paths paths;
+    paths.frame = kRefineValFrame; paths.spp = kWaveSpp;
+    paths.first = rp.path_first; paths.ray = rp.path_ray;
+    const frt_wave::Trips t = frt_wave::simulate(paths, st, kTravMinLdsPath);
+    out.rays = (double)t.rays;
+    if (t.rays == 0) return true;
+    out.node_trips = (double)t.node_wave / t.rays; out.leaf_trips = (double)t.leaf_wave / t.rays;
+    out.step_trips = (double)t.step_wave / t.rays; out.shade_trips = (double)t.shade_wave / t.rays;
+    out.node_util = t.node_wave ? (double)t.node_lane / (64.0 * t.node_wave) : 0.0;
+    out.leaf_util = t.leaf_wave ? (double)t.leaf_lane / (64.0 * t.leaf_wave) : 0.0;
+    out.step_util = t.step_wave ? (double)t.step_lane / (64.0 * t.step_wave) : 0.0;
+    out.cost = t.cost() / t.rays;
+    return true;
+}
+
+
+constexpr int kPlanMaxEvals = 900;
+constexpr int kPlanStages = 3;
+constexpr int kPlanPrefix[kPlanStages - 1] = {16, 4};
+constexpr double kPlanSlack[kPlanStages - 1] = {0.04, 0.01};
+
+static Replay replay_prefix(const Replay &a, int part)
+{
+    Replay b = a;
+    frt_refine::RaySet &R = b.R;
+    const int m = std::max(a.R.n / part, std::min(a.R.n, 1));
+    R.n = m;
+    R.tmin.resize(m); R.tmax.resize(m); R.anyhit.resize(m); R.live.resize(m);
+    R.slab.resize((size_t)m * R.n_leaves * 6);
+    R.prim_t.resize((size_t)m * R.n_prims);
+    R.root.clear();
+    b.occl.resize(m); b.from.resize(m);
+    b.origins.clear();
+    return b;
+}
+
+struct PlanCtx {
+    const FlatScene &F;
+    std::vector<RefineLeaf> leaves;
+    ShadowProof shadow;
+    ExitProof exit;
+    Replay rp[kPlanStages + 1];
+    std::vector<uint8_t> live[kPlanStages + 1];
+};
+struct PlanPrice {
+    double J = 0.0, V = 0.0, T = 0.0;
+    int sroot = 0, appended = 0, shadow_added = 0, served = 0;
+    bool shadow_ran = false, exit_ran = false;
+    std::vector<int> exit_root;
+};
+static PlanPrice price_plan(PlanCtx &C, const frt_refine::Topology &t, int on, bool as_stored = false)
+{
+    PlanPrice out;
+    const FlatScene &F = C.F;
+    std::vector<float> nodes = node_floats(as_stored ? F.nodes : topology_nodes(t, C.leaves));
+    const int nn_main = (int)(nodes.size() / 16);
+    out.sroot = F.meta.root;
+    frt_shadow::Tree st;
+    if (shadow_derive(F, nodes, C.shadow, st) == FlatScene::kShadowRan) {
+        out.shadow_ran = true;
+        out.sroot = st.empty ? kSentinel : st.root;
+        out.shadow_added = st.added;
+    }
+    ExitChoice ec;
+    const int choose = std::min(on, kPlanStages - 1);
+    C.rp[choose].R.live = C.live[choose];
+    C.rp[choose].R.root.clear();
+    out.exit_ran = exit_derive(F, nodes, C.exit, C.leaves, C.rp[choose], nn_main, true, ec) == FlatScene::kExitRan;
+    out.exit_root = ec.root;
+    if (!out.exit_ran) std::fill(out.exit_root.begin(), out.exit_root.end(), 0);
+    for (int r : out.exit_root) out.served += r != 0;
+    out.appended = (int)(nodes.size() / 16) - nn_main;
+    const TreeView v(node_records(nodes), &C.leaves);
+    start_rays(v, C.rp[on], C.live[on], F.meta.root, out.sroot, out.exit_ran ? &out.exit_root : nullptr);
+    const frt_refine::Cost c = frt_refine::tree_cost(v.t, C.rp[on].R);
+    out.V = c.V; out.T = c.T; out.J = frt_refine::cost_j(c, kRefineW);
+    return out;
+}
+
+bool refine_tree(const frt_scene_view *sv, FlatScene &F, int mode)
+{
+    F.plan = {};
+    const int nn = (int)(F.nodes.size() / 4);
+    if (!pass_on(mode, "FRT_TREE_REFINE") || !tree_in_lds(F) || nn < 3) return false;
+    const TreeView v(F.nodes);
+    if (v.t.n_leaves != nn + 1) return false;
+    frt_refine::Topology t = v.t;
+    PlanCtx C{F, v.leaves, {}, {}, {}, {}};
+    Replay &fit = C.rp[kPlanStages - 1], &val = C.rp[kPlanStages];
+    fit = sample_rays(F, v.leaves, kRefineFitFrame, kRefineFitSeed);
+    const int kept = frt_refine::refine(t, fit.R, kRefineW, v.t.depth(), kRefineMaxEvals);
+    const int plan = plan_mode();
+    if (!kept && !plan) return false;
+    val = sample_rays(F, v.leaves, kRefineValFrame, kRefineValSeed);
+    const double j0 = frt_refine::cost_j(frt_refine::tree_cost(v.t, val.R), kRefineW);
+    const double j1 = kept ? frt_refine::cost_j(frt_refine::tree_cost(t, val.R), kRefineW) : j0;
+    const bool refined = kept && j1 < j0;
+    if (!refined) t = v.t;
+    auto &I = F.plan;
+    I.mode = plan;
+    I.j_main_in = j0; I.j_main = j1;
+    if (I.mode != 0 && F.meta.root == 0) {
+        shadow_proof(sv, F, 1, C.shadow);
+        exit_proof(sv, F, 1, C.exit);
+    }
+    if (C.shadow.why == FlatScene::kShadowRan || C.exit.why == FlatScene::kExitRan) {
+        for (int k = 0; k < kPlanStages - 1; ++k) C.rp[k] = replay_prefix(fit, kPlanPrefix[k]);
+        for (int k = 0; k <= kPlanStages; ++k) C.live[k] = C.rp[k].R.live;
+        double best[kPlanStages];
+        int served = 0, appended = 0;
+        for (int k = 0; k < kPlanStages; ++k) {
+            const PlanPrice p = price_plan(C, t, k, !refined);
+            best[k] = p.J;
+            served = p.served;
+            appended = p.appended;
+        }
+        auto keeps_blocks = [&](const PlanPrice &p) { return p.appended <= appended || keeps_plan(F, nn + appended, nn + p.appended, true); };
+        frt_refine::Topology u = t;
+        const frt_plan::Result r = frt_plan::search(u, v.t.depth(), kPlanMaxEvals, [&](const frt_refine::Topology &x) {
+            const double inf = std::numeric_limits<double>::infinity();
+            double j[kPlanStages];
+            for (int k = 0; k < kPlanStages; ++k) {
+                const PlanPrice p = price_plan(C, x, k);
+                j[k] = p.J;
+                if (k < kPlanStages - 1 ? !(j[k] <= best[k] * (1.0 + kPlanSlack[k])) : (p.served < served || !keeps_blocks(p) || !(j[k] < best[k]))) return inf;
+            }
+            std::copy(j, j + kPlanStages, best);
+            return j[kPlanStages - 1];
+        });
+        PlanPrice chosen = price_plan(C, t, kPlanStages, !refined);
+        I.searched = true; I.evals = r.evals; I.kept = r.kept;
+        I.j_parent = I.j_plan = chosen.J;
+        if (r.kept > 0) {
+            const PlanPrice p = price_plan(C, u, kPlanStages);
+            val.R.live = C.live[kPlanStages];
+            val.R.root.clear();
+            const double ju = frt_refine::cost_j(frt_refine::tree_cost(u, val.R), kRefineW);
+            if (p.J < chosen.J && ju < j0 && p.served >= chosen.served && keeps_blocks(p)) {
+                I.accepted = true;
+                I.j_plan = p.J; I.j_main = ju;
+                chosen = p;
+                I.main_root_nodes = refined ? topology_nodes(t, v.leaves) : F.nodes;
+                t = u;
+            }
+        }
+        I.sroot = chosen.sroot; I.appended = chosen.appended; I.served = chosen.served;
+        I.exit_root = chosen.exit_root;
+        I.priced = true;
+    }
+    if (!refined && !I.accepted) return false;
+    F.nodes = topology_nodes(t, v.leaves);
+    return true;
+}
diff --git a/first_raytracer_amd/csrc/frt_tree_passes.hpp b/first_raytracer_amd/csrc/frt_tree_passes.hpp
--- a/first_raytracer_amd/csrc/frt_tree_passes.hpp
+++ b/first_raytracer_amd/csrc/frt_tree_passes.hpp
@@ -2,7 +2,7 @@
 #include "frt_flatten.hpp"
 
 #pragma GCC visibility push(hidden)
-bool refine_tree(FlatScene &F, int mode);
+bool refine_tree(const frt_scene_view *sv, FlatScene &F, int mode);
 bool shadow_tree(const frt_scene_view *sv, FlatScene &F, int mode);
 bool exit_tree(const frt_scene_view *sv, FlatScene &F, int mode);
 
@@ -11,6 +11,10 @@
     int n_rays = 0, n_ext = 0;
 };
 bool exit_cost_host(const FlatScene &F, ExitCost &out);
+struct PlanCost { double V[4] = {0, 0, 0, 0}, T[4] = {0, 0, 0, 0}, J[4] = {0, 0, 0, 0}; int n[4] = {0, 0, 0, 0}, depth = 0; };
+bool plan_cost_host(const FlatScene &F, PlanCost &out);
+struct WaveCost { double node_trips = 0, leaf_trips = 0, step_trips = 0, shade_trips = 0, node_util = 0, leaf_util = 0, step_util = 0, cost = 0, rays = 0; };
+bool wave_cost_host(const FlatScene &F, WaveCost &out);
 struct ShadowCost { double V[2] = {0, 0}, T[2] = {0, 0}; int n_rays = 0, stops[2] = {0, 0}; };
 bool shadow_cost_host(const FlatScene &F, ShadowCost &out);
 void shadow_origins_host(const FlatScene &F, std::vector<float> &origins);
diff --git a/first_raytracer_amd/csrc/host/shadow_tree.cpp b/first_raytracer_amd/csrc/host/shadow_tree.cpp
--- a/first_raytracer_amd/csrc/host/shadow_tree.cpp
+++ b/first_raytracer_amd/csrc/host/shadow_tree.cpp
@@ -113,7 +113,7 @@
 }
 
 void build(std::vector<float> &nodes, int main_root, const std::vector<uint8_t> &dropped, int sphere_bit,
-           int count_shift, Tree &out)
+           int count_shift, Tree &out, int share_from)
 {
     out = Tree{};
     auto ref_of = [&](int i, int side) {
@@ -136,6 +136,7 @@
         decltype(ref_of) &ref;
         decltype(leaf_kept) &kept;
         Tree &out;
+        int share_from;
         Sub visit(int r, const float *box)
         {
             Sub s{};
@@ -154,7 +155,11 @@
             if (a.empty || b.empty) { Sub c = a.empty ? b : a; c.same = false; return c; }
             if (a.same && b.same) { s.same = true; s.n_nodes = 1 + a.n_nodes + b.n_nodes; return s; }
             out.shared += a.n_nodes + b.n_nodes;
-            s.ref = (int)(nodes.size() / 16);
+            for (int k = 0; k < 3; ++k) { s.box[k] = std::min(a.box[k], b.box[k]); s.box[3 + k] = std::max(a.box[3 + k], b.box[3 + k]); }
+            const int n_stored = (int)(nodes.size() / 16);
+            for (int i = share_from; i >= 0 && i < n_stored; ++i)
+                if (ref(i, 0) == a.ref && ref(i, 1) == b.ref) { s.ref = i; ++out.reused; return s; }
+            s.ref = n_stored;
             float rec[16] = {0};
             for (int k = 0; k < 6; ++k) { rec[k] = a.box[k]; rec[6 + k] = b.box[k]; }
             const int refs[2] = {a.ref, b.ref};
@@ -162,10 +167,9 @@
                       reinterpret_cast<char *>(&rec[12]));
             nodes.insert(nodes.end(), rec, rec + 16);
             ++out.added;
-            for (int k = 0; k < 3; ++k) { s.box[k] = std::min(a.box[k], b.box[k]); s.box[3 + k] = std::max(a.box[3 + k], b.box[3 + k]); }
             return s;
         }
-    } rec{nodes, ref_of, leaf_kept, out};
+    } rec{nodes, ref_of, leaf_kept, out, share_from};
     const float no_box[6] = {0, 0, 0, 0, 0, 0};
     const Sub r = rec.visit(main_root, no_box);
     out.shared += r.n_nodes;
diff --git a/first_raytracer_amd/csrc/host/shadow_tree.hpp b/first_raytracer_amd/csrc/host/shadow_tree.hpp
--- a/first_raytracer_amd/csrc/host/shadow_tree.hpp
+++ b/first_raytracer_amd/csrc/host/shadow_tree.hpp
@@ -28,9 +28,10 @@
     int root = 0;
     bool empty = false;
     int added = 0, shared = 0;
+    int reused = 0;
     int kept_leaves = 0, dropped_leaves = 0;
 };
 void build(std::vector<float> &nodes, int main_root, const std::vector<uint8_t> &dropped, int sphere_bit,
-           int count_shift, Tree &out);
+           int count_shift, Tree &out, int share_from = -1);
 
 }
diff --git a/first_raytracer_amd/csrc/host/tree_plan.cpp b/first_raytracer_amd/csrc/host/tree_plan.cpp
--- /dev/null
+++ b/first_raytracer_amd/csrc/host/tree_plan.cpp
@@ -0,0 +1,66 @@
+#include "tree_plan.hpp"
+
+#include <algorithm>
+#include <vector>
+
+namespace frt_plan {
+
+Result search(frt_refine::Topology &t, int max_depth, int max_evals, const Score &score)
+{
+    using frt_refine::Topology;
+    Result out;
+    const int L = t.n_leaves, nI = (int)(t.child.size() / 2), nS = L + nI;
+    out.start = out.best = score(t);
+    if (nI != L - 1 || nI < 2 || max_evals <= 0) return out;
+    std::vector<int> parent(nS, -1);
+    auto set_parents = [&](const Topology &u) {
+        std::fill(parent.begin(), parent.end(), -1);
+        for (int j = 0; j < nI; ++j) { parent[u.child[2 * j]] = L + j; parent[u.child[2 * j + 1]] = L + j; }
+    };
+    set_parents(t);
+    auto in_subtree = [&](int x, int s) {
+        for (; x >= 0; x = parent[x]) if (x == s) return true;
+        return false;
+    };
+    auto moved = [&](int s, int x) {
+        Topology u = t;
+        auto side_of = [&](int par, int c) { return 2 * (par - L) + (u.child[2 * (par - L)] == c ? 0 : 1); };
+        const int p = parent[s], q = u.child[side_of(p, s) ^ 1], g = parent[p];
+        if (g < 0) u.root = q;
+        else u.child[side_of(g, p)] = q;
+        const int xp = (x == q) ? g : parent[x];
+        if (xp < 0) u.root = p;
+        else u.child[side_of(xp, x)] = p;
+        u.child[2 * (p - L)] = x;
+        u.child[2 * (p - L) + 1] = s;
+        return u;
+    };
+    bool improved = true;
+    while (improved && out.evals < max_evals) {
+        improved = false;
+        for (int s = 0; s < nS && out.evals < max_evals; ++s) {
+            if (parent[s] < 0) continue;
+            const int p = parent[s], q = t.child[2 * (p - L)] == s ? t.child[2 * (p - L) + 1] : t.child[2 * (p - L)];
+            Topology best_t;
+            double best = out.best;
+            bool found = false;
+            for (int x = 0; x < nS && out.evals < max_evals; ++x) {
+                if (x == p || x == q || in_subtree(x, s)) continue;
+                Topology u = moved(s, x);
+                if (u.depth() > max_depth) continue;
+                ++out.evals;
+                const double j = score(u);
+                if (j < best) { best = j; best_t.n_leaves = u.n_leaves; best_t.root = u.root; best_t.child.swap(u.child); found = true; }
+            }
+            if (!found) continue;
+            t = best_t;
+            set_parents(t);
+            out.best = best;
+            ++out.kept;
+            improved = true;
+        }
+    }
+    return out;
+}
+
+}
diff --git a/first_raytracer_amd/csrc/host/tree_plan.hpp b/first_raytracer_amd/csrc/host/tree_plan.hpp
--- /dev/null
+++ b/first_raytracer_amd/csrc/host/tree_plan.hpp
@@ -0,0 +1,17 @@
+#pragma once
+#include <functional>
+
+#include "tree_refine.hpp"
+
+namespace frt_plan {
+
+using Score = std::function<double(const frt_refine::Topology &)>;
+
+struct Result {
+    int evals = 0, kept = 0;
+    double start = 0.0, best = 0.0;
+};
+
+Result search(frt_refine::Topology &t, int max_depth, int max_evals, const Score &score);
+
+}
diff --git a/first_raytracer_amd/csrc/host/tree_refine.cpp b/first_raytracer_amd/csrc/host/tree_refine.cpp
--- a/first_raytracer_amd/csrc/host/tree_refine.cpp
+++ b/first_raytracer_amd/csrc/host/tree_refine.cpp
@@ -17,6 +17,7 @@
 
 struct Tables {
     int n_slots = 0;
+    int first = 0;
     std::vector<float> tab;
 };
 
@@ -25,15 +26,16 @@
     for (int k = 0; k < 6; ++k) out[k] = std::min(a[k], b[k]);
 }
 
+struct StepSink { std::vector<uint16_t> *nodes, *prims; };
 void count_rays(const Topology &t, const RaySet &R, const Tables &tb, const int *dirty, int n_dirty, const int *local_of,
-                int r0, int r1, uint64_t &V, uint64_t &T)
+                int r0, int r1, uint64_t &V, uint64_t &T, const StepSink *steps = nullptr)
 {
     const int L = t.n_leaves;
     const int *child = t.child.data();
     float loc[2 * kMaxLevels][6];
     for (int r = r0; r < r1; ++r) {
         if (!R.live[r]) continue;
-        const float *base = &tb.tab[(size_t)r * tb.n_slots * 6];
+        const float *base = &tb.tab[(size_t)(r - tb.first) * tb.n_slots * 6];
         auto rec = [&](int s) { return n_dirty > 0 && local_of[s] >= 0 ? loc[local_of[s]] : base + 6 * s; };
         for (int k = 0; k < n_dirty; ++k) {
             const int j = dirty[k] - L;
@@ -46,6 +48,10 @@
         int hp = -1, sp = 0, node = R.root.empty() ? t.root : R.root[r];
         int stk[kMaxLevels];
         for (;;) {
+            const uint64_t v0 = V, t0_ = T;
+            auto step_ends = [&]() {
+                if (steps) { steps->nodes->push_back((uint16_t)(V - v0)); steps->prims->push_back((uint16_t)(T - t0_)); }
+            };
             while (node >= L) {
                 ++V;
                 const int c0 = child[2 * (node - L)], c1 = child[2 * (node - L) + 1];
@@ -67,7 +73,7 @@
                     node = sp > 0 ? stk[--sp] : -1;
                 }
             }
-            if (node < 0) break;
+            if (node < 0) { step_ends(); break; }
             bool done = false;
             for (int k = R.prim_first[node]; k < R.prim_first[node + 1]; ++k) {
                 ++T;
@@ -80,22 +86,21 @@
                     if (any) { done = true; break; }
                 }
             }
+            step_ends();
             if (done || sp == 0) break;
             node = stk[--sp];
         }
     }
 }
 
-void build_tables(const Topology &t, const RaySet &R, Tables &tb)
-{
-    const int L = t.n_leaves, nI = (int)(t.child.size() / 2);
-    tb.n_slots = L + nI;
-    tb.tab.resize((size_t)R.n * tb.n_slots * 6);
+std::vector<int> bottom_up(const Topology &t, const RaySet &R)
+{
+    const int L = t.n_leaves, n_slots = L + (int)(t.child.size() / 2);
     std::vector<int> order, roots{t.root};
     roots.insert(roots.end(), R.root.begin(), R.root.end());
     std::sort(roots.begin(), roots.end());
     roots.erase(std::unique(roots.begin(), roots.end()), roots.end());
-    std::vector<char> seen(tb.n_slots, 0);
+    std::vector<char> seen(n_slots, 0);
     std::vector<std::pair<int, bool>> st;
     for (int root : roots) st.push_back({root, false});
     while (!st.empty()) {
@@ -109,14 +114,27 @@
         st.push_back({t.child[2 * (s - L)], false});
         st.push_back({t.child[2 * (s - L) + 1], false});
     }
-    for (int r = 0; r < R.n; ++r) {
-        float *base = &tb.tab[(size_t)r * tb.n_slots * 6];
-        memcpy(base, &R.slab[(size_t)r * L * 6], sizeof(float) * 6 * L);
-        for (size_t k = 0; k < order.size(); ++k) {
-            const int s = order[k], j = s - L;
-            unite(base + 6 * t.child[2 * j], base + 6 * t.child[2 * j + 1], base + 6 * s);
-        }
-    }
+    return order;
+}
+
+inline void fill_records(const Topology &t, const RaySet &R, const std::vector<int> &order, int r, float *base)
+{
+    const int L = t.n_leaves;
+    memcpy(base, &R.slab[(size_t)r * L * 6], sizeof(float) * 6 * L);
+    for (size_t k = 0; k < order.size(); ++k) {
+        const int s = order[k], j = s - L;
+        unite(base + 6 * t.child[2 * j], base + 6 * t.child[2 * j + 1], base + 6 * s);
+    }
+}
+
+void build_tables(const Topology &t, const RaySet &R, Tables &tb)
+{
+    tb.n_slots = t.n_leaves + (int)(t.child.size() / 2);
+    tb.first = 0;
+    tb.tab.resize((size_t)R.n * tb.n_slots * 6);
+    const std::vector<int> order = bottom_up(t, R);
+    for (int r = 0; r < R.n; ++r)
+        if (R.live[r]) fill_records(t, R, order, r, &tb.tab[(size_t)r * tb.n_slots * 6]);
 }
 
 }
@@ -140,12 +158,41 @@
 Cost tree_cost(const Topology &t, const RaySet &R)
 {
     Tables tb;
-    build_tables(t, R, tb);
+    tb.n_slots = t.n_leaves + (int)(t.child.size() / 2);
+    tb.tab.resize((size_t)tb.n_slots * 6);
+    const std::vector<int> order = bottom_up(t, R);
     uint64_t V = 0, T = 0;
-    count_rays(t, R, tb, nullptr, 0, nullptr, 0, R.n, V, T);
+    for (int r = 0; r < R.n; ++r) {
+        if (!R.live[r]) continue;
+        tb.first = r;
+        fill_records(t, R, order, r, tb.tab.data());
+        count_rays(t, R, tb, nullptr, 0, nullptr, r, r + 1, V, T);
+    }
     Cost c;
     if (R.n > 0) { c.V = (double)V / R.n; c.T = (double)T / R.n; }
     return c;
+}
+
+void ray_steps(const Topology &t, const RaySet &R, std::vector<int> &first, std::vector<uint16_t> &nodes,
+               std::vector<uint16_t> &prims)
+{
+    Tables tb;
+    tb.n_slots = t.n_leaves + (int)(t.child.size() / 2);
+    tb.tab.resize((size_t)tb.n_slots * 6);
+    const std::vector<int> order = bottom_up(t, R);
+    first.assign((size_t)R.n + 1, 0);
+    nodes.clear();
+    prims.clear();
+    const StepSink sink{&nodes, &prims};
+    uint64_t V = 0, T = 0;
+    for (int r = 0; r < R.n; ++r) {
+        first[r] = (int)nodes.size();
+        if (!R.live[r]) continue;
+        tb.first = r;
+        fill_records(t, R, order, r, tb.tab.data());
+        count_rays(t, R, tb, nullptr, 0, nullptr, r, r + 1, V, T, &sink);
+    }
+    first[R.n] = (int)nodes.size();
 }
 
 int refine(Topology &t, const RaySet &R, double w, int max_depth, int max_evals)
diff --git a/first_raytracer_amd/csrc/host/tree_refine.hpp b/first_raytracer_amd/csrc/host/tree_refine.hpp
--- a/first_raytracer_amd/csrc/host/tree_refine.hpp
+++ b/first_raytracer_amd/csrc/host/tree_refine.hpp
@@ -26,6 +26,9 @@
 
 Cost tree_cost(const Topology &t, const RaySet &rays);
 
+void ray_steps(const Topology &t, const RaySet &rays, std::vector<int> &first, std::vector<uint16_t> &nodes,
+               std::vector<uint16_t> &prims);
+
 int refine(Topology &t, const RaySet &fit, double w, int max_depth, int max_evals);
 
 }
diff --git a/first_raytracer_amd/csrc/host/wave_model.cpp b/first_raytracer_amd/csrc/host/wave_model.cpp
--- /dev/null
+++ b/first_raytracer_amd/csrc/host/wave_model.cpp
@@ -0,0 +1,74 @@
+#include "wave_model.hpp"
+
+#include <algorithm>
+
+namespace frt_wave {
+
+Trips simulate(const Paths &p, const Steps &s, int trav_min)
+{
+    Trips out;
+    if (p.frame <= 0 || p.frame % 8 != 0 || p.spp <= 0) return out;
+    const int blocks = p.frame / 8;
+    struct Lane { int path, path_end, k, k_end, step, step_end; bool tracing, pending, active; };
+    for (int b = 0; b < blocks * blocks; ++b) {
+        Lane L[64];
+        for (int l = 0; l < 64; ++l) {
+            const int x = (b % blocks) * 8 + l % 8, y = (b / blocks) * 8 + l / 8, pix = y * p.frame + x;
+            L[l] = Lane{pix * p.spp, (pix + 1) * p.spp, 0, 0, 0, 0, false, false, false};
+        }
+        auto begin_ray = [&](Lane &a) {
+            const int r = p.ray[a.k];
+            ++out.rays;
+            a.step = s.first[r];
+            a.step_end = s.first[r + 1];
+            a.tracing = a.step < a.step_end;
+            a.pending = !a.tracing;
+        };
+        for (;;) {
+            for (;;) {
+                int n_max = 0, p_max = 0, tracing = 0;
+                for (Lane &a : L) {
+                    if (!a.tracing) continue;
+                    ++tracing;
+                    const int n = s.nodes[a.step], q = s.prims[a.step];
+                    n_max = std::max(n_max, n);
+                    p_max = std::max(p_max, q);
+                    out.node_lane += n;
+                    out.leaf_lane += q;
+                    if (++a.step < a.step_end) continue;
+                    const int r = p.ray[a.k];
+                    if (s.shadow[r] && a.k + 1 < a.k_end) { ++a.k; begin_ray(a); }
+                    else { a.tracing = false; a.pending = true; }
+                }
+                if (tracing) { ++out.step_wave; out.step_lane += tracing; out.node_wave += n_max; out.leaf_wave += p_max; }
+                int still = 0;
+                for (const Lane &a : L) still += a.tracing;
+                if (still <= trav_min) break;
+            }
+            bool shaded = false, any = false;
+            for (Lane &a : L) {
+                bool next = false;
+                if (a.pending) {
+                    a.pending = false;
+                    shaded = true;
+                    a.active = ++a.k < a.k_end;
+                    next = a.active;
+                }
+                if (!a.active && a.path < a.path_end) {
+                    a.k = p.first[a.path];
+                    a.k_end = p.first[a.path + 1];
+                    ++a.path;
+                    a.active = a.k < a.k_end;
+                    next = a.active;
+                }
+                if (next) begin_ray(a);
+                any |= a.tracing || a.pending;
+            }
+            out.shade_wave += shaded;
+            if (!any) break;
+        }
+    }
+    return out;
+}
+
+}
diff --git a/first_raytracer_amd/csrc/host/wave_model.hpp b/first_raytracer_amd/csrc/host/wave_model.hpp
--- /dev/null
+++ b/first_raytracer_amd/csrc/host/wave_model.hpp
@@ -0,0 +1,23 @@
+#pragma once
+#include <cstdint>
+#include <vector>
+
+namespace frt_wave {
+
+struct Paths {
+    int frame = 0, spp = 0;
+    std::vector<int> first;
+    std::vector<int> ray;
+};
+struct Steps {
+    std::vector<int> first;
+    std::vector<uint16_t> nodes, prims;
+    std::vector<uint8_t> shadow;
+};
+struct Trips {
+    uint64_t node_wave = 0, node_lane = 0, leaf_wave = 0, leaf_lane = 0, step_wave = 0, step_lane = 0, shade_wave = 0, rays = 0;
+    double cost() const { return 31.0 * (double)node_wave + 56.0 * (double)leaf_wave; }
+};
+Trips simulate(const Paths &p, const Steps &s, int trav_min);
+
+}
diff --git a/include/frt.h b/include/frt.h
--- a/include/frt.h
+++ b/include/frt.h
@@ -239,6 +239,18 @@
 int frtx_selftest_exit_tree(const frt_scene_view *scene, int32_t mode, frt_exit_tree_info *out, int32_t *roots,
                             int32_t *view_of, int32_t *taken, int32_t max_taken, float *nodes_off, float *nodes_on,
                             int32_t max_nodes);
+typedef struct frt_tree_plan_info {
+    int32_t mode, priced, searched, accepted, evals, kept;
+    int32_t priced_sroot, built_sroot, priced_appended, built_appended, priced_served, built_served;
+    int32_t shadow_added, nodes_main, n_nodes, depth_in, depth, n_kind[4];
+    int32_t reserved;
+    double j_parent, j_plan, j_main_in, j_main;
+    double v[4], t[4], j[4];
+    double pass_seconds;
+} frt_tree_plan_info;
+int frtx_selftest_tree_plan(const frt_scene_view *scene, frt_tree_plan_info *out, int32_t *roots_priced,
+                            int32_t *roots_built, float *nodes, int32_t max_nodes);
+int frtx_selftest_wave_model(const frt_scene_view *scene, double *out);
 int frtx_selftest_trace_host(const frt_scene_view *scene, const float *rays, int64_t n, float *hits);
 int frtx_selftest_chunk_variance(const float *partial, int n_chunks, int64_t n_slots, int spp, int spi, float *out);
 typedef struct frt_plan_query {
```

Result: faster. 42530 (median of 6 runs) (+3.7%).
